# ilpoviertola/V-AURA

Measured on AMD Instinct MI355X. Metric: audio codec tokens/sec (whole node), 2.56 s clips, higher is better.
Workload: dtype f16x2-split(22b)/f32-acc

## Files before the change

include/vaura_hip.h:

```cpp
#ifndef VAURA_HIP_H
#define VAURA_HIP_H

#include <stddef.h>
#include <stdint.h>

#ifdef __cplusplus
extern "C" {
#endif

typedef void* vaura_stream_t;

typedef enum vaura_status {
  VAURA_OK = 0,
  VAURA_ERR_ARG = -1,
  VAURA_ERR_SHAPE = -2,
  VAURA_ERR_DTYPE = -3,
  VAURA_ERR_STATE = -4
} vaura_status;

typedef enum vaura_wdtype { VAURA_W_F32 = 0, VAURA_W_BF16 = 1, VAURA_W_FP8 = 2, VAURA_W_H1 = 3, VAURA_W_H2 = 4, VAURA_W_FP8H = 5 } vaura_wdtype;

typedef struct vaura_dims {
  int32_t n_layer;
  int32_t d_model;
// ... 135 lines not shown

int vaura_pattern_build(const int32_t* codes, int32_t* seq, int B, int K, int T, int special, vaura_stream_t s);
int vaura_pattern_revert(const int32_t* seq, int32_t* codes, int B, int K, int T, int S, int fill, vaura_stream_t s);
int vaura_pattern_build_delays(const int32_t* codes, int32_t* seq, int B, int K, int T, int S, int special,
                               const int32_t* delays_host, vaura_stream_t s);
int vaura_pattern_revert_delays(const int32_t* seq, int32_t* codes, int B, int K, int T, int S, int fill,
                                const int32_t* delays_host, vaura_stream_t s);

int vaura_sample(const float* logits, int B, int K, int vocab, const vaura_sampling* sp, const float* noise,
                 int64_t step, int32_t* tokens_out, vaura_stream_t s);

int vaura_sample_clips(const float* logits, int B, int K, int vocab, const vaura_sampling* sp, const vaura_clip_sampling* clips,
                       const float* noise, int64_t step, int32_t* tokens_out, int32_t* seq, int T, int S, int32_t* state,
                       vaura_stream_t s);

int vaura_sample_logprobs(const float* logits, int B, int K, int vocab, const vaura_sampling* sp, const vaura_clip_sampling* clips,
                          const float* noise, int64_t step, int32_t* tokens_out, int32_t* seq, int T, int S, int32_t* state,
                          float* logprobs_out, vaura_stream_t s);
int vaura_sample_relevance(const float* logits, int B, int K, int vocab, const vaura_sampling* sp, const vaura_clip_sampling* clips,
                           const float* noise, int64_t step, int32_t* tokens_out, int32_t* seq, int T, int S, int32_t* state,
                           float* logprobs_out, float* cond_out, float* null_out, vaura_stream_t s);
int vaura_pattern_revert_delays_f32(const float* seq, float* out, int B, int K, int T, int S, float fill, const int32_t* delays_host,
                                    vaura_stream_t s);
int vaura_sequence_logprob(const float* logprobs, int seq_len, const int32_t* delays_host, int B, int K, int T, int t0,
                           float* per_codebook, float* per_clip, vaura_stream_t s);
int vaura_select_candidates(const float* scores, const int32_t* codes, int B, int N, int K, int T, int32_t* codes_out, int32_t* winner,
                            vaura_stream_t s);

int vaura_pattern_build_clips(const int32_t* codes, int32_t* seq, int B, int K, int T, int S, int special, const int32_t* delays_host,
                              const int32_t* clip_timesteps, vaura_stream_t s);
int vaura_pattern_revert_clips(const int32_t* seq, int32_t* codes, int B, int K, int T, int S, int fill, int pad,
                               const int32_t* delays_host, const int32_t* clip_timesteps, vaura_stream_t s);
int vaura_pattern_revert_clips_f32(const float* seq, float* out, int B, int K, int T, int S, float fill, float pad,
                                   const int32_t* delays_host, const int32_t* clip_timesteps, vaura_stream_t s);
int vaura_sequence_logprob_clips(const float* logprobs, int seq_len, const int32_t* delays_host, int B, int K, int T, int t0,
                                 const int32_t* clip_timesteps, float* per_codebook, float* per_clip, vaura_stream_t s);
int vaura_sample_seq(const float* logits, int B, int K, int vocab, const vaura_sampling* sp, const vaura_clip_sampling* clips,
                     const float* noise, int32_t* seq, int T, int S, int32_t* state, const int32_t* delays_host,
                     const int32_t* clip_timesteps, float* lp_seq, float* cond_seq, float* null_seq, vaura_stream_t s);
int vaura_sample_seq_starts(const float* logits, int B, int K, int vocab, const vaura_sampling* sp, const vaura_clip_sampling* clips,
                            const float* noise, int32_t* seq, int T, int S, int32_t* state, const int32_t* delays_host,
                            const int32_t* clip_timesteps, const int32_t* clip_first_steps, float* lp_seq, float* cond_seq,
                            float* null_seq, vaura_stream_t s);
int vaura_sequence_logprob_starts(const float* logprobs, int seq_len, const int32_t* delays_host, int B, int K, int T,
                                  const int32_t* clip_t0, const int32_t* clip_timesteps, float* per_codebook, float* per_clip,
                                  vaura_stream_t s);
int vaura_embed(const vaura_decoder* dec, int pos_host, int n_pos, vaura_stream_t s);

int vaura_decode_step(const vaura_decoder* dec, const vaura_sampling* sp, int sample, vaura_stream_t s);

typedef void* vaura_step_graph_t;
int vaura_generate_loop(const vaura_decoder* dec, const vaura_sampling* sp, int n_prefill, int n_steps,
                        vaura_step_graph_t graph, vaura_stream_t s);
int vaura_step_graph_build(const vaura_decoder* dec, const vaura_sampling* sp, vaura_stream_t s, vaura_step_graph_t* out);
int vaura_prefill_rows(const vaura_decoder* dec, int n_prefill, int n_sel, vaura_stream_t s);
void vaura_step_graph_free(vaura_step_graph_t graph);

typedef enum vaura_kernel_kind {
  VAURA_K_EMBED = 0, VAURA_K_QKV = 1, VAURA_K_ATTN = 2, VAURA_K_WO = 3, VAURA_K_W13 = 4, VAURA_K_W2 = 5,
  VAURA_K_HEADS = 6, VAURA_K_SAMPLE = 7, VAURA_K_COUNT = 8
} vaura_kernel_kind;
int vaura_profile_loop(const vaura_decoder* dec, const vaura_sampling* sp, int n_steps, unsigned kind_mask,
                       double* total_ms_host, int64_t* launches_host, vaura_stream_t s);
void vaura_profile_outliers(int64_t* per_kind);

int vaura_score(const vaura_decoder* dec, int n_pos, const int32_t* targets, float* ws_chunk_logits, float* logits_out, float* nll,
                uint8_t* mask_out, float* loss_per_cb, float* loss, vaura_stream_t s);
int vaura_score_relevance(const vaura_decoder* dec, int n_pos, const int32_t* targets, float* ws_chunk_logits, float* logits_out, float* nll,
                          uint8_t* mask_out, float* loss_per_cb, float* loss, float* nll_null, float* loss_per_cb_null, float* loss_null,
                          vaura_stream_t s);
int vaura_score_logits(const float* logits, const int32_t* targets, const uint8_t* mask, int B, int K, int V, int Ta, float* nll,
                       float* loss_per_cb, float* loss, vaura_stream_t s);

int vaura_gemv(const void* w, int wdtype, const float* x, const float* gain, const float* residual, float* out,
               int64_t rows, int64_t N, int64_t K, int epilogue, float eps, vaura_stream_t s);
int vaura_gemv_pair(const void* w, int wdtype , const uint16_t* x_split, const float* ss_in, int n_ss_in, const float* residual, float* out,
                    float* out_khalf2 ,
                    uint16_t* out_split, const float* gain_out, float* ss_out, int64_t rows, int64_t N, int64_t K, int epilogue,
                    float eps, vaura_stream_t s);
int vaura_split_rows(const float* src, uint16_t* dst, const float* gain, float* ss, int64_t rows, int64_t C, vaura_stream_t s);

int vaura_attention_step(const float* qkv, const float* rope, float* kcache, float* vcache, float* out,
                         int rows, int n_head, int head_dim, int max_len, int pos, vaura_stream_t s);

int vaura_attention_step_split(const float* qkv, const float* rope, float* kcache, float* vcache, float* out, float* part,
                               int rows, int n_head, int head_dim, int max_len, int pos, int n_split, vaura_stream_t s);
int vaura_attention_splits(int rows, int n_head, int max_len);
int vaura_attention_step_ex(const float* qkv, const float* qkv2, const float* rope, float* kcache, float* vcache, float* out,
                            uint16_t* out_split, float* part, uint32_t* arrivals, int rows, int n_head, int head_dim, int max_len,
                            int pos, int n_split, int plane_shift, int kv_dtype, vaura_stream_t s);
int vaura_attention_step_kv(const float* qkv, const float* qkv2, const float* rope, float* kcache, float* vcache, uint8_t* kscale,
                            uint8_t* vscale, float* out, uint16_t* out_split, float* part, uint32_t* arrivals, int rows, int n_head,
                            int head_dim, int max_len, int pos, int n_split, int plane_shift, int kv_dtype, vaura_stream_t s);
int vaura_attention_step_probs(const float* qkv, const float* qkv2, const float* rope, float* kcache, float* vcache, uint8_t* kscale,
                               uint8_t* vscale, float* out, uint16_t* out_split, float* part, uint32_t* arrivals, int rows, int n_head,
                               int head_dim, int max_len, int pos, int n_split, int plane_shift, int kv_dtype, float* probs, int pos0,
                               int n_steps, int rows_out, vaura_stream_t s);
int vaura_attention_map(const float* probs, float* out, int n_steps, int n_rows, int n_head, int max_len, int W, int all_heads,
                        vaura_stream_t s);
int vaura_attention_prefill(const vaura_decoder* d, int layer, int p0, int n_pos, vaura_stream_t s);
int vaura_rope_append_rows(const vaura_decoder* d, int layer, int p0, int n_pos, const int32_t* row_n, int n_sel, vaura_stream_t s);

typedef struct vaura_conv {
  const float* w;
  const float* bias;
  const float* wscale;
  int32_t cin, cout, taps, dilation, stride, _pad;
} vaura_conv;

typedef struct vaura_codec {
  int32_t n_codebooks, codebook_size, codebook_dim, latent_dim;
  int32_t n_blocks, n_units;
  int32_t rates[4];
  const float* codebooks;
  const float* out_proj_w;
  const float* out_proj_b;
  vaura_conv conv_in;
  const float* alpha_up[4];
  vaura_conv up[4];
  const float* alpha_res[4][3][2];
  vaura_conv res[4][3][2];
  const float* alpha_out;
  vaura_conv conv_out;
  float* ws[4];
  size_t ws_elems;
  int32_t precision;
  int32_t _pad1;
} vaura_codec;

int vaura_dac_decode(const vaura_codec* c, const int32_t* codes, int B, int T, float* wav, vaura_stream_t s);
size_t vaura_dac_workspace_elems(const vaura_codec* c, int B, int T);
int vaura_dac_decode_clips(const vaura_codec* c, const int32_t* codes, int B, int T_max, const int32_t* lengths, float* wav,
                           vaura_stream_t s);
size_t vaura_dac_decode_clips_workspace_elems(const vaura_codec* c, int B, const int32_t* lengths);
int vaura_dac_clips_gap(const vaura_codec* c);
int vaura_dac_decode_window(const vaura_codec* c, const int32_t* codes, int B, int T_max, const int32_t* lengths, const int32_t* starts,
                            const int32_t* counts, float* wav, int N_max, vaura_stream_t s);
size_t vaura_dac_decode_window_workspace_elems(const vaura_codec* c, int B, const int32_t* lengths, const int32_t* starts,
                                               const int32_t* counts);
int vaura_dac_decode_halo(const vaura_codec* c);
int vaura_dac_decode_window_seq(const vaura_codec* c, const int32_t* seq, int B, int K, int S, const int32_t* delays_host,
                                const int32_t* lengths, const int32_t* starts, const int32_t* counts, float* wav, int N_max,
                                vaura_stream_t s);
size_t vaura_dac_decode_window_seq_workspace_elems(const vaura_codec* c, int B, int K, int S, const int32_t* delays_host,
                                                   const int32_t* lengths, const int32_t* starts, const int32_t* counts);
int vaura_dac_conv(const vaura_conv* cv, int precision, const float* in, float* out, float* scratch, int B, int Lin,
                   vaura_stream_t s);
int vaura_dac_conv_ex(const vaura_conv* cv, int precision, const float* in, const float* res, const float* alpha, float* out_raw,
                      void* out_act, float* scratch, int B, int Lin, vaura_stream_t s);
#define VAURA_DAC_UNIT_TWO_LAUNCHES (-100)
int vaura_dac_unit(const vaura_conv* c7, const vaura_conv* c1, int precision, const float* in, const float* res,
                   const float* alpha_mid, const float* alpha_next, float* out_raw, void* out_act, float* scratch, float* mid, int B,
                   int L, vaura_stream_t s);
int vaura_dac_from_codes(const int32_t* codes, const float* codebooks, const float* out_proj_w, const float* out_proj_b, void* z,
                         int B, int K, int T, int size, int dim, int latent, int pairs, vaura_stream_t s);
int vaura_dac_conv_out(const vaura_conv* cv, int precision, const float* in, float* wav, float* scratch, int B, int L,
                       vaura_stream_t s);
int vaura_snake(const float* x, const float* alpha, float* y, int64_t rows, int C, vaura_stream_t s);

typedef struct vaura_codec_encoder {
  int32_t n_codebooks, codebook_size, codebook_dim, latent_dim;
  int32_t n_blocks, n_units;
  int32_t rates[4];
  int32_t enc_dim;
  int32_t _pad0;
  const float* conv_in_w;
  const float* conv_in_b;
  const float* alpha_res[4][3][2];
  vaura_conv res[4][3][2];
  const float* alpha_down[4];
  vaura_conv down[4];
  const float* alpha_out;
  vaura_conv conv_out;
  const float* in_proj_w;
  const float* in_proj_b;
  const float* codebooks;
  const float* out_proj_w;
  const float* out_proj_b;
  float* ws[4];
  size_t ws_elems;
} vaura_codec_encoder;
int vaura_dac_encode(const vaura_codec_encoder* c, const float* wav, int B, int64_t n_samples, int32_t* codes, vaura_stream_t s);
int vaura_dac_enc_conv_in(const float* wav, const float* w, const float* bias, const float* alpha, float* out_raw, void* out_act,
                          int B, int64_t L, int C, vaura_stream_t s);
int vaura_dac_rvq_stage(float* residual, const float* in_w, const float* in_b, const float* codebook, const float* out_w,
                        const float* out_b, int32_t* codes, int B, int T, int latent, int dim, int size, int K, int k,
                        vaura_stream_t s);
size_t vaura_dac_encode_workspace_elems(const vaura_codec_encoder* c, int B, int64_t n_samples);
int vaura_dac_encode_clips(const vaura_codec_encoder* c, const float* wav, int B, int64_t n_max, const int64_t* sample_lengths,
                           int32_t* codes, vaura_stream_t s);
size_t vaura_dac_encode_clips_workspace_elems(const vaura_codec_encoder* c, int B, const int64_t* sample_lengths);
int vaura_dac_encode_clips_gap(const vaura_codec_encoder* c);

typedef enum vaura_audio_strategy { VAURA_AUDIO_CLIP = 0, VAURA_AUDIO_PEAK = 1, VAURA_AUDIO_RMS = 2, VAURA_AUDIO_NONE = 3 } vaura_audio_strategy;
int vaura_audio_normalize(const float* wav, float* out, int n_clips, int64_t n_samples, int strategy, int normalize,
                          float peak_clip_headroom_db, float rms_headroom_db, float* scratch, vaura_stream_t s);
size_t vaura_audio_scratch_elems(int n_clips);
int vaura_audio_loudness(const float* wav, float* out, int n_clips, int64_t n_samples, int sample_rate, float loudness_headroom_db,
                         int compressor, float energy_floor, float* scratch, vaura_stream_t s);
size_t vaura_audio_loudness_scratch_elems(int n_clips);
int vaura_audio_normalize_clips(const float* wav, float* out, int n_clips, int64_t n_stride, const int32_t* lengths, int strategy,
                                int normalize, float peak_clip_headroom_db, float rms_headroom_db, float* scratch, vaura_stream_t s);
int vaura_audio_loudness_clips(const float* wav, float* out, int n_clips, int64_t n_stride, const int32_t* lengths, int sample_rate,
                               float loudness_headroom_db, int compressor, float energy_floor, float* scratch, vaura_stream_t s);

typedef struct vaura_vit_attn {
  const void* qkv_w; const float* qkv_b;
  const void* proj_w; const float* proj_b;
} vaura_vit_attn;
typedef struct vaura_vit_block {
  const float *ln1_w, *ln1_b, *ln2_w, *ln2_b, *ln3_w, *ln3_b;
  vaura_vit_attn space, time;
  const void* fc1_w; const float* fc1_b; const void* fc2_w; const float* fc2_b;
} vaura_vit_block;
typedef struct vaura_vit {
  int32_t depth, dim, heads, hidden;
  int32_t n_patches, n_frames;
  int32_t in_chans, frames, img, patch, patch_t, patch_k;
  float eps; int32_t _pad;
  const void* pe_w; const float* pe_b;
  const float *cls_token, *pos_embed, *temp_embed;
  const vaura_vit_block* blocks_host;
  const float *norm_w, *norm_b;
  const float* agg_cls;
  const float *agg_ln1_w, *agg_ln1_b, *agg_ln2_w, *agg_ln2_b;
  const void* agg_in_w; const float* agg_in_b;
  const void* agg_out_w; const float* agg_out_b;
  const void* agg_l1_w; const float* agg_l1_b;
  const void* agg_l2_w; const float* agg_l2_b;
  float* ws_x; float* ws_qkv; uint16_t* ws_a; uint16_t* ws_h; uint16_t* ws_p; float* ws_z; float* ws_s;
} vaura_vit;
int vaura_avclip_forward(const vaura_vit* v, const float* frames, int n_seg, float* feats, vaura_stream_t s);
size_t vaura_avclip_workspace_bytes(const vaura_vit* v, int n_seg, int which);

int vaura_vit_patchify(const float* frames, void* patches, int n_seg, int in_chans, int frames_per_seg, int img, int patch_t, int patch,
                       vaura_stream_t s);
int vaura_vit_embed(const vaura_vit* v, float* x, int n_seg, vaura_stream_t s);
int vaura_vit_layernorm(const vaura_vit* v, const float* x, const float* w, const float* b, float* out_f32, void* out_pair, int64_t rows,
                        int map, vaura_stream_t s);
int vaura_vit_fill_rows(const vaura_vit* v, float* dst, const float* vec, int64_t n, int64_t stride, vaura_stream_t s);
int vaura_vit_cls_attention(const vaura_vit* v, const float* qkv, void* out_pair, float* part, int n_seq, int Lseq, int64_t out_stride,
                            vaura_stream_t s);
int vaura_vit_time_attention(const vaura_vit* v, const float* qkv, void* out_pair, int n_seg, vaura_stream_t s);
int vaura_vit_space_attention(const vaura_vit* v, const float* qkv, void* out_pair, int n_seg, vaura_stream_t s);
int vaura_linear_pair(const void* in, const void* w, const float* bias, const float* res, float* out_raw, void* out_act, int act, int B,
                      int Lin, int Lout, int oshift, int Cin, int Cout, vaura_stream_t s);

#define VAURA_PREPROC_MAX_TAPS 32
int vaura_video_preprocess(const uint8_t* video, int channels_last, int n_clips, int T, int C, int H, int W, int resize, int crop_h,
                           int crop_w, int F, int S, int seg_start, int seg_stride, const int32_t* h_rel, const int16_t* h_w, int h_taps,
                           int h_prec, const int32_t* v_start, const int16_t* v_w, int v_taps, int v_prec, int x0, int span,
                           int tile_rows, int tile_src_rows, const float* lut, float* out, vaura_stream_t s);
size_t vaura_video_preprocess_lds_bytes(int channels_last, int crop_w, int h_taps, int span, int tile_src_rows);

enum { VAURA_YUV_NV12 = 0, VAURA_YUV_I420 = 1 };
int vaura_video_preprocess_yuv420(const uint8_t* video, int64_t video_bytes, int layout, int64_t pitch, int64_t chroma_offset,
                                  int64_t frame_stride, int n_clips, int T, int H, int W, int y_off, int cy, int crv, int cgu, int cgv,
                                  int cbu, int resize, int crop_h, int crop_w, int F, int S, int seg_start, int seg_stride,
                                  const int32_t* h_rel, const int16_t* h_w, int h_taps, int h_prec, const int32_t* v_start,
                                  const int16_t* v_w, int v_taps, int v_prec, int x0, int span, int tile_rows, int tile_src_rows,
                                  const float* lut, float* out, vaura_stream_t s);
size_t vaura_video_preprocess_yuv420_lds_bytes(int layout, int crop_w, int h_taps, int span, int tile_src_rows);

int vaura_video_preprocess_frames(const uint8_t* video, int channels_last, int n_clips, int T, int C, int H, int W, int resize,
                                  int crop_h, int crop_w, int F, int S, const int32_t* h_rel, const int16_t* h_w, int h_taps, int h_prec,
                                  const int32_t* v_start, const int16_t* v_w, int v_taps, int v_prec, int x0, int span, int tile_rows,
                                  int tile_src_rows, const float* lut, float* out, const int32_t* frame_map, const uint8_t* carry,
                                  int carry_used, vaura_stream_t s);
int vaura_video_preprocess_yuv420_frames(const uint8_t* video, int64_t video_bytes, int layout, int64_t pitch, int64_t chroma_offset,
                                         int64_t frame_stride, int n_clips, int T, int H, int W, int y_off, int cy, int crv, int cgu,
                                         int cgv, int cbu, int resize, int crop_h, int crop_w, int F, int S, const int32_t* h_rel,
                                         const int16_t* h_w, int h_taps, int h_prec, const int32_t* v_start, const int16_t* v_w,
                                         int v_taps, int v_prec, int x0, int span, int tile_rows, int tile_src_rows, const float* lut,
                                         float* out, const int32_t* frame_map, const uint8_t* carry, int carry_used, vaura_stream_t s);

#define VAURA_AUDIO_PRE_TILE 1024
#define VAURA_AUDIO_PRE_MAX_TAPS 64
enum { VAURA_PCM_S16 = 0, VAURA_PCM_S32 = 1, VAURA_PCM_F32 = 2 };
int vaura_audio_preprocess(const void* pcm, int format, int interleaved, int B, int C, int64_t in_stride, const int32_t* n_in, int o, int n,
                           int w, const int32_t* first, const float* taps, int phases, int taps_per_phase, float* out, int64_t out_stride,
                           const int32_t* n_out, vaura_stream_t s);
size_t vaura_audio_preprocess_lds_bytes(int o, int n, int w, int taps_per_phase);
int vaura_audio_preprocess_tile(void);

#define VAURA_AUDIO_OUT_TILE 1024
#define VAURA_AUDIO_OUT_RECORD 5
int vaura_audio_output(const float* x, int B, int64_t in_stride, const int64_t* records, const float* carry_in, float* carry_out,
                       int history, int o, int n, int w, const int32_t* first, const float* taps, int phases, int taps_per_phase,
                       const float* gain, int format, int interleaved, int C_out, void* out, int64_t out_stride, int32_t* clipped,
                       vaura_stream_t s);
size_t vaura_audio_output_lds_bytes(int o, int n, int w, int taps_per_phase);
int vaura_audio_output_tile(void);

#define VAURA_SPECTROGRAM_RECORD 5
#define VAURA_SPECTROGRAM_MAX_MELS 256
enum { VAURA_SPEC_POWER = 0, VAURA_SPEC_DB = 1, VAURA_SPEC_LOG = 2, VAURA_SPEC_COMPLEX = 3 };
int vaura_spectrogram(const float* x, int B, int64_t in_stride, const int64_t* records, const float* carry_in, float* carry_out,
                      int history, int n_fft, int hop, const float* window, const float* twiddles, const int32_t* mel_bins,
                      const float* mel_weights, int mel_total, int F, int scale, float amin, float* out, int64_t out_stride,
                      vaura_stream_t s);
size_t vaura_spectrogram_lds_bytes(int n_fft, int F);

void vaura_set_debug_flags(unsigned flags);
void vaura_set_debug_flags2(unsigned flags);
long long vaura_debug_counter(int which);

const char* vaura_version(void);
size_t vaura_struct_size(int which);

#ifdef __cplusplus
}
#endif
#endif
```

vaura_amd/_lib.py:

```python
from __future__ import annotations

import ctypes as C
import os
from typing import Optional

_HERE = os.path.dirname(os.path.abspath(__file__))
LIB_PATH = os.path.join(_HERE, "csrc", "libvaura_hip.so")

W_F32, W_BF16, W_FP8, W_H1, W_H2, W_FP8H = 0, 1, 2, 3, 4, 5
EPI_STORE, EPI_RESID, EPI_SWIGLU, EPI_GELU, EPI_LOGITS = 0, 1, 2, 3, 4
DAC_UNIT_TWO_LAUNCHES = -100
KERNEL_KINDS = ("embed", "qkv", "attn", "wo", "w13", "w2", "heads", "sample")

c_float_p = C.c_void_p


class Dims(C.Structure):
    _fields_ = [("n_layer", C.c_int32), ("d_model", C.c_int32), ("n_head", C.c_int32), ("ffn_dim", C.c_int32),
                ("n_codebooks", C.c_int32), ("vocab", C.c_int32), ("cond_dim", C.c_int32), ("tok_dim", C.c_int32),
                ("cond_in", C.c_int32), ("codebook_dim", C.c_int32), ("tokens_per_frame", C.c_int32),
                ("eps", C.c_float)]


class LayerWeights(C.Structure):
# ... 5 lines not shown
    _fields_ = [("use_sampling", C.c_int32), ("temp", C.c_float), ("top_k", C.c_int32), ("top_p", C.c_float),
                ("cfg_scale", C.c_float), ("seed", C.c_uint64), ("clip_base", C.c_uint64), ("input_is_probs", C.c_int32),
                ("tie_eps", C.c_float)]


class ClipSampling(C.Structure):
    _fields_ = [("use_sampling", C.c_int32), ("temp", C.c_float), ("top_k", C.c_int32), ("top_p", C.c_float),
                ("cfg_scale", C.c_float), ("reserved", C.c_int32 * 3)]


class Decoder(C.Structure):
    _fields_ = [("dims", Dims), ("wdtype", C.c_int32), ("batch", C.c_int32), ("rows", C.c_int32),
                ("max_len", C.c_int32), ("timesteps", C.c_int32), ("seq_len", C.c_int32),
                ("n_cond_tokens", C.c_int32), ("prefill_positions", C.c_int32),
                ("plane_shift", C.c_int32), ("kv_dtype", C.c_int32),
                ("layers_host", C.POINTER(LayerWeights)), ("heads", C.c_void_p), ("final_norm", C.c_void_p),
                ("tok_emb", C.c_void_p), ("tok_proj_w", C.c_void_p), ("tok_proj_b", C.c_void_p), ("tok_table", C.c_void_p),
                ("empty_video", C.c_void_p), ("rope", C.c_void_p), ("cond_proj", C.c_void_p),
                ("kcache", C.c_void_p), ("vcache", C.c_void_p), ("seq", C.c_void_p), ("state", C.c_void_p),
                ("noise", C.c_void_p),
                ("ws_h", C.c_void_p), ("ws_qkv", C.c_void_p), ("ws_qkv2", C.c_void_p), ("ws_attn", C.c_void_p), ("ws_ffn", C.c_void_p),
                ("ws_logits", C.c_void_p),
                ("ws_h_split", C.c_void_p), ("ws_attn_split", C.c_void_p), ("ws_ffn_split", C.c_void_p),
                ("ws_ss", C.c_void_p), ("first_norm", C.c_void_p), ("ws_attn_part", C.c_void_p), ("ws_sync", C.c_void_p),
                ("has_pattern_delays", C.c_int32), ("pattern_delays", C.c_int32 * 16), ("ext_bytes", C.c_int32),
                ("kscale", C.c_void_p), ("vscale", C.c_void_p), ("clip_sampling", C.c_void_p), ("logprobs", C.c_void_p)]


class DecoderExt(C.Structure):
    _fields_ = [("dec", Decoder), ("logprobs_cond", C.c_void_p), ("logprobs_null", C.c_void_p)]


class DecoderExt2(C.Structure):
    _fields_ = [("ext", DecoderExt), ("clip_timesteps", C.c_void_p), ("clip_cond_tokens", C.c_void_p)]


class DecoderExt3(C.Structure):
    _fields_ = [("ext2", DecoderExt2), ("row_prompt_steps", C.c_void_p)]


class DecoderExt4(C.Structure):
    _fields_ = [("ext3", DecoderExt3), ("attn_probs", C.c_void_p), ("attn_layer", C.c_int32), ("attn_pos0", C.c_int32),
                ("attn_steps", C.c_int32), ("attn_rows", C.c_int32)]


class Conv(C.Structure):
    _fields_ = [("w", C.c_void_p), ("bias", C.c_void_p), ("wscale", C.c_void_p), ("cin", C.c_int32), ("cout", C.c_int32),
                ("taps", C.c_int32), ("dilation", C.c_int32), ("stride", C.c_int32), ("_pad", C.c_int32)]


class Codec(C.Structure):
    _fields_ = [("n_codebooks", C.c_int32), ("codebook_size", C.c_int32), ("codebook_dim", C.c_int32),
                ("latent_dim", C.c_int32), ("n_blocks", C.c_int32), ("n_units", C.c_int32),
                ("rates", C.c_int32 * 4),
                ("codebooks", C.c_void_p), ("out_proj_w", C.c_void_p), ("out_proj_b", C.c_void_p),
                ("conv_in", Conv), ("alpha_up", C.c_void_p * 4), ("up", Conv * 4),
                ("alpha_res", ((C.c_void_p * 2) * 3) * 4), ("res", ((Conv * 2) * 3) * 4),
                ("alpha_out", C.c_void_p), ("conv_out", Conv),
                ("ws", C.c_void_p * 4), ("ws_elems", C.c_size_t), ("precision", C.c_int32), ("_pad1", C.c_int32)]


class CodecEncoder(C.Structure):
    _fields_ = [("n_codebooks", C.c_int32), ("codebook_size", C.c_int32), ("codebook_dim", C.c_int32),
                ("latent_dim", C.c_int32), ("n_blocks", C.c_int32), ("n_units", C.c_int32),
                ("rates", C.c_int32 * 4), ("enc_dim", C.c_int32), ("_pad0", C.c_int32),
                ("conv_in_w", C.c_void_p), ("conv_in_b", C.c_void_p),
                ("alpha_res", ((C.c_void_p * 2) * 3) * 4), ("res", ((Conv * 2) * 3) * 4),
                ("alpha_down", C.c_void_p * 4), ("down", Conv * 4),
                ("alpha_out", C.c_void_p), ("conv_out", Conv),
                ("in_proj_w", C.c_void_p), ("in_proj_b", C.c_void_p), ("codebooks", C.c_void_p),
                ("out_proj_w", C.c_void_p), ("out_proj_b", C.c_void_p),
                ("ws", C.c_void_p * 4), ("ws_elems", C.c_size_t)]


class VitAttn(C.Structure):
    _fields_ = [("qkv_w", C.c_void_p), ("qkv_b", C.c_void_p), ("proj_w", C.c_void_p), ("proj_b", C.c_void_p)]


class VitBlock(C.Structure):
    _fields_ = [("ln1_w", C.c_void_p), ("ln1_b", C.c_void_p), ("ln2_w", C.c_void_p), ("ln2_b", C.c_void_p),
                ("ln3_w", C.c_void_p), ("ln3_b", C.c_void_p), ("space", VitAttn), ("time", VitAttn),
                ("fc1_w", C.c_void_p), ("fc1_b", C.c_void_p), ("fc2_w", C.c_void_p), ("fc2_b", C.c_void_p)]


class Vit(C.Structure):
    _fields_ = [("depth", C.c_int32), ("dim", C.c_int32), ("heads", C.c_int32), ("hidden", C.c_int32),
                ("n_patches", C.c_int32), ("n_frames", C.c_int32),
                ("in_chans", C.c_int32), ("frames", C.c_int32), ("img", C.c_int32), ("patch", C.c_int32), ("patch_t", C.c_int32),
                ("patch_k", C.c_int32), ("eps", C.c_float), ("_pad", C.c_int32),
                ("pe_w", C.c_void_p), ("pe_b", C.c_void_p), ("cls_token", C.c_void_p), ("pos_embed", C.c_void_p),
                ("temp_embed", C.c_void_p), ("blocks_host", C.POINTER(VitBlock)), ("norm_w", C.c_void_p), ("norm_b", C.c_void_p),
                ("agg_cls", C.c_void_p), ("agg_ln1_w", C.c_void_p), ("agg_ln1_b", C.c_void_p), ("agg_ln2_w", C.c_void_p),
                ("agg_ln2_b", C.c_void_p), ("agg_in_w", C.c_void_p), ("agg_in_b", C.c_void_p), ("agg_out_w", C.c_void_p),
                ("agg_out_b", C.c_void_p), ("agg_l1_w", C.c_void_p), ("agg_l1_b", C.c_void_p), ("agg_l2_w", C.c_void_p),
                ("agg_l2_b", C.c_void_p),
                ("ws_x", C.c_void_p), ("ws_qkv", C.c_void_p), ("ws_a", C.c_void_p), ("ws_h", C.c_void_p), ("ws_p", C.c_void_p),
                ("ws_z", C.c_void_p), ("ws_s", C.c_void_p)]


SIGNATURES = {
    "vaura_audio_normalize": (C.c_int, [C.c_void_p, C.c_void_p, C.c_int, C.c_int64, C.c_int, C.c_int, C.c_float, C.c_float,
                                        C.c_void_p, C.c_void_p]),
    "vaura_audio_scratch_elems": (C.c_size_t, [C.c_int]),
    "vaura_audio_loudness": (C.c_int, [C.c_void_p, C.c_void_p, C.c_int, C.c_int64, C.c_int, C.c_float, C.c_int, C.c_float, C.c_void_p,
                                       C.c_void_p]),
    "vaura_audio_loudness_scratch_elems": (C.c_size_t, [C.c_int]),
    "vaura_audio_normalize_clips": (C.c_int, [C.c_void_p, C.c_void_p, C.c_int, C.c_int64, C.c_void_p, C.c_int, C.c_int, C.c_float,
                                              C.c_float, C.c_void_p, C.c_void_p]),
    "vaura_audio_loudness_clips": (C.c_int, [C.c_void_p, C.c_void_p, C.c_int, C.c_int64, C.c_void_p, C.c_int, C.c_float, C.c_int,
                                             C.c_float, C.c_void_p, C.c_void_p]),
    "vaura_dac_encode": (C.c_int, [C.POINTER(CodecEncoder), C.c_void_p, C.c_int, C.c_int64, C.c_void_p, C.c_void_p]),
    "vaura_dac_encode_workspace_elems": (C.c_size_t, [C.POINTER(CodecEncoder), C.c_int, C.c_int64]),
    "vaura_avclip_forward": (C.c_int, [C.POINTER(Vit), C.c_void_p, C.c_int, C.c_void_p, C.c_void_p]),
    "vaura_avclip_workspace_bytes": (C.c_size_t, [C.POINTER(Vit), C.c_int, C.c_int]),
    "vaura_vit_patchify": (C.c_int, [C.c_void_p, C.c_void_p, C.c_int, C.c_int, C.c_int, C.c_int, C.c_int, C.c_int, C.c_void_p]),
    "vaura_vit_embed": (C.c_int, [C.POINTER(Vit), C.c_void_p, C.c_int, C.c_void_p]),
    "vaura_vit_layernorm": (C.c_int, [C.POINTER(Vit), C.c_void_p, C.c_void_p, C.c_void_p, C.c_void_p, C.c_void_p, C.c_int64, C.c_int,
                                      C.c_void_p]),
    "vaura_vit_fill_rows": (C.c_int, [C.POINTER(Vit), C.c_void_p, C.c_void_p, C.c_int64, C.c_int64, C.c_void_p]),
    "vaura_vit_cls_attention": (C.c_int, [C.POINTER(Vit), C.c_void_p, C.c_void_p, C.c_void_p, C.c_int, C.c_int, C.c_int64, C.c_void_p]),
    "vaura_vit_time_attention": (C.c_int, [C.POINTER(Vit), C.c_void_p, C.c_void_p, C.c_int, C.c_void_p]),
    "vaura_vit_space_attention": (C.c_int, [C.POINTER(Vit), C.c_void_p, C.c_void_p, C.c_int, C.c_void_p]),
    "vaura_linear_pair": (C.c_int, [C.c_void_p, C.c_void_p, C.c_void_p, C.c_void_p, C.c_void_p, C.c_void_p, C.c_int, C.c_int, C.c_int,
                                    C.c_int, C.c_int, C.c_int, C.c_int, C.c_void_p]),
    "vaura_video_preprocess": (C.c_int, [C.c_void_p, C.c_int, C.c_int, C.c_int, C.c_int, C.c_int, C.c_int, C.c_int, C.c_int, C.c_int, C.c_int,
                                         C.c_int, C.c_int, C.c_int, C.c_void_p, C.c_void_p, C.c_int, C.c_int, C.c_void_p, C.c_void_p,
                                         C.c_int, C.c_int, C.c_int, C.c_int, C.c_int, C.c_int, C.c_void_p, C.c_void_p, C.c_void_p]),
    "vaura_video_preprocess_lds_bytes": (C.c_size_t, [C.c_int, C.c_int, C.c_int, C.c_int, C.c_int]),
    "vaura_video_preprocess_yuv420": (C.c_int, [C.c_void_p, C.c_int64, C.c_int, C.c_int64, C.c_int64, C.c_int64, *[C.c_int] * 10,
                                                *[C.c_int] * 7, C.c_void_p, C.c_void_p, C.c_int, C.c_int, C.c_void_p, C.c_void_p,
                                                *[C.c_int] * 6, C.c_void_p, C.c_void_p, C.c_void_p]),
    "vaura_video_preprocess_yuv420_lds_bytes": (C.c_size_t, [C.c_int, C.c_int, C.c_int, C.c_int, C.c_int]),
    "vaura_video_preprocess_frames": (C.c_int, [C.c_void_p, *[C.c_int] * 11, C.c_void_p, C.c_void_p, C.c_int, C.c_int, C.c_void_p, C.c_void_p,
                                                *[C.c_int] * 6, C.c_void_p, C.c_void_p, C.c_void_p, C.c_void_p, C.c_int, C.c_void_p]),
    "vaura_video_preprocess_yuv420_frames": (C.c_int, [C.c_void_p, C.c_int64, C.c_int, C.c_int64, C.c_int64, C.c_int64, *[C.c_int] * 10,
                                                       *[C.c_int] * 5, C.c_void_p, C.c_void_p, C.c_int, C.c_int, C.c_void_p, C.c_void_p,
                                                       *[C.c_int] * 6, C.c_void_p, C.c_void_p, C.c_void_p, C.c_void_p, C.c_int, C.c_void_p]),
    "vaura_audio_preprocess": (C.c_int, [C.c_void_p, C.c_int, C.c_int, C.c_int, C.c_int, C.c_int64, C.c_void_p, C.c_int, C.c_int, C.c_int,
                                         C.c_void_p, C.c_void_p, C.c_int, C.c_int, C.c_void_p, C.c_int64, C.c_void_p, C.c_void_p]),
    "vaura_audio_preprocess_lds_bytes": (C.c_size_t, [C.c_int, C.c_int, C.c_int, C.c_int]),
    "vaura_audio_preprocess_tile": (C.c_int, []),
    "vaura_audio_output": (C.c_int, [C.c_void_p, C.c_int, C.c_int64, C.c_void_p, C.c_void_p, C.c_void_p, C.c_int, C.c_int, C.c_int, C.c_int,
                                     C.c_void_p, C.c_void_p, C.c_int, C.c_int, C.c_void_p, C.c_int, C.c_int, C.c_int, C.c_void_p, C.c_int64,
                                     C.c_void_p, C.c_void_p]),
    "vaura_audio_output_lds_bytes": (C.c_size_t, [C.c_int, C.c_int, C.c_int, C.c_int]),
    "vaura_audio_output_tile": (C.c_int, []),
    "vaura_spectrogram": (C.c_int, [C.c_void_p, C.c_int, C.c_int64, C.c_void_p, C.c_void_p, C.c_void_p, C.c_int, C.c_int, C.c_int,
                                    C.c_void_p, C.c_void_p, C.c_void_p, C.c_void_p, C.c_int, C.c_int, C.c_int, C.c_float, C.c_void_p,
                                    C.c_int64, C.c_void_p]),
    "vaura_spectrogram_lds_bytes": (C.c_size_t, [C.c_int, C.c_int]),
    "vaura_version": (C.c_char_p, []),
    "vaura_set_debug_flags": (None, [C.c_uint]),
    "vaura_set_debug_flags2": (None, [C.c_uint]),
    "vaura_debug_counter": (C.c_longlong, [C.c_int]),
    "vaura_struct_size": (C.c_size_t, [C.c_int]),
    "vaura_packed_weight_bytes": (C.c_size_t, [C.c_int64, C.c_int64, C.c_int]),
    "vaura_pack_weight": (C.c_int, [C.c_void_p, C.c_void_p, C.c_int64, C.c_int64, C.c_int, C.c_void_p]),
    "vaura_build_token_table": (C.c_int, [C.c_void_p, C.c_void_p, C.c_void_p, C.c_void_p, C.c_int, C.c_int, C.c_int,
                                          C.c_int, C.c_void_p]),
    "vaura_pack_rows": (C.c_int, [C.c_void_p, C.c_void_p, C.c_int64, C.c_int64, C.c_void_p]),
    "vaura_unpack_rows": (C.c_int, [C.c_void_p, C.c_void_p, C.c_int64, C.c_int64, C.c_void_p]),
    "vaura_prefill_cond": (C.c_int, [C.POINTER(Dims), C.c_void_p, C.c_void_p, C.c_void_p, C.c_int, C.c_void_p,
                                     C.c_void_p, C.c_int64, C.c_void_p]),
    "vaura_cond_window": (C.c_int, [C.POINTER(Decoder), C.c_void_p, C.c_void_p, C.c_int, C.c_int, C.c_int, C.c_void_p]),
    "vaura_pattern_build": (C.c_int, [C.c_void_p, C.c_void_p, C.c_int, C.c_int, C.c_int, C.c_int, C.c_void_p]),
    "vaura_pattern_revert": (C.c_int, [C.c_void_p, C.c_void_p, C.c_int, C.c_int, C.c_int, C.c_int, C.c_int, C.c_void_p]),
    "vaura_pattern_build_delays": (C.c_int, [C.c_void_p, C.c_void_p, C.c_int, C.c_int, C.c_int, C.c_int, C.c_int,
                                             C.POINTER(C.c_int32), C.c_void_p]),
    "vaura_pattern_revert_delays": (C.c_int, [C.c_void_p, C.c_void_p, C.c_int, C.c_int, C.c_int, C.c_int, C.c_int,
                                              C.POINTER(C.c_int32), C.c_void_p]),
    "vaura_sample": (C.c_int, [C.c_void_p, C.c_int, C.c_int, C.c_int, C.POINTER(Sampling), C.c_void_p, C.c_int64,
                               C.c_void_p, C.c_void_p]),
    "vaura_sample_clips": (C.c_int, [C.c_void_p, C.c_int, C.c_int, C.c_int, C.POINTER(Sampling), C.c_void_p, C.c_void_p, C.c_int64,
                                     C.c_void_p, C.c_void_p, C.c_int, C.c_int, C.c_void_p, C.c_void_p]),
    "vaura_sample_logprobs": (C.c_int, [C.c_void_p, C.c_int, C.c_int, C.c_int, C.POINTER(Sampling), C.c_void_p, C.c_void_p, C.c_int64,
                                        C.c_void_p, C.c_void_p, C.c_int, C.c_int, C.c_void_p, C.c_void_p, C.c_void_p]),
    "vaura_sample_relevance": (C.c_int, [C.c_void_p, C.c_int, C.c_int, C.c_int, C.POINTER(Sampling), C.c_void_p, C.c_void_p, C.c_int64,
                                         C.c_void_p, C.c_void_p, C.c_int, C.c_int, C.c_void_p, C.c_void_p, C.c_void_p, C.c_void_p,
                                         C.c_void_p]),
    "vaura_pattern_revert_delays_f32": (C.c_int, [C.c_void_p, C.c_void_p, C.c_int, C.c_int, C.c_int, C.c_int, C.c_float,
                                                  C.POINTER(C.c_int32), C.c_void_p]),
    "vaura_sequence_logprob": (C.c_int, [C.c_void_p, C.c_int, C.POINTER(C.c_int32), C.c_int, C.c_int, C.c_int, C.c_int, C.c_void_p,
                                         C.c_void_p, C.c_void_p]),
    "vaura_select_candidates": (C.c_int, [C.c_void_p, C.c_void_p, C.c_int, C.c_int, C.c_int, C.c_int, C.c_void_p, C.c_void_p,
                                          C.c_void_p]),
    "vaura_pattern_build_clips": (C.c_int, [C.c_void_p, C.c_void_p, C.c_int, C.c_int, C.c_int, C.c_int, C.c_int, C.POINTER(C.c_int32),
                                            C.c_void_p, C.c_void_p]),
    "vaura_pattern_revert_clips": (C.c_int, [C.c_void_p, C.c_void_p, C.c_int, C.c_int, C.c_int, C.c_int, C.c_int, C.c_int,
                                             C.POINTER(C.c_int32), C.c_void_p, C.c_void_p]),
    "vaura_pattern_revert_clips_f32": (C.c_int, [C.c_void_p, C.c_void_p, C.c_int, C.c_int, C.c_int, C.c_int, C.c_float, C.c_float,
                                                 C.POINTER(C.c_int32), C.c_void_p, C.c_void_p]),
    "vaura_sequence_logprob_clips": (C.c_int, [C.c_void_p, C.c_int, C.POINTER(C.c_int32), C.c_int, C.c_int, C.c_int, C.c_int, C.c_void_p,
                                               C.c_void_p, C.c_void_p, C.c_void_p]),
    "vaura_sample_seq": (C.c_int, [C.c_void_p, C.c_int, C.c_int, C.c_int, C.POINTER(Sampling), C.c_void_p, C.c_void_p, C.c_void_p, C.c_int,
                                   C.c_int, C.c_void_p, C.POINTER(C.c_int32), C.c_void_p, C.c_void_p, C.c_void_p, C.c_void_p, C.c_void_p]),
    "vaura_sample_seq_starts": (C.c_int, [C.c_void_p, C.c_int, C.c_int, C.c_int, C.POINTER(Sampling), C.c_void_p, C.c_void_p, C.c_void_p, C.c_int,
                                          C.c_int, C.c_void_p, C.POINTER(C.c_int32), C.c_void_p, C.c_void_p, C.c_void_p, C.c_void_p, C.c_void_p,
                                          C.c_void_p]),
    "vaura_sequence_logprob_starts": (C.c_int, [C.c_void_p, C.c_int, C.POINTER(C.c_int32), C.c_int, C.c_int, C.c_int, C.c_void_p, C.c_void_p,
                                                C.c_void_p, C.c_void_p, C.c_void_p]),
    "vaura_prefill_rows": (C.c_int, [C.POINTER(Decoder), C.c_int, C.c_int, C.c_void_p]),
    "vaura_rope_append_rows": (C.c_int, [C.POINTER(Decoder), C.c_int, C.c_int, C.c_int, C.c_void_p, C.c_int, C.c_void_p]),
    "vaura_embed": (C.c_int, [C.POINTER(Decoder), C.c_int, C.c_int, C.c_void_p]),
    "vaura_decode_step": (C.c_int, [C.POINTER(Decoder), C.POINTER(Sampling), C.c_int, C.c_void_p]),
    "vaura_generate_loop": (C.c_int, [C.POINTER(Decoder), C.POINTER(Sampling), C.c_int, C.c_int, C.c_void_p, C.c_void_p]),
    "vaura_step_graph_build": (C.c_int, [C.POINTER(Decoder), C.POINTER(Sampling), C.c_void_p, C.POINTER(C.c_void_p)]),
    "vaura_step_graph_free": (None, [C.c_void_p]),
    "vaura_profile_loop": (C.c_int, [C.POINTER(Decoder), C.POINTER(Sampling), C.c_int, C.c_uint, C.POINTER(C.c_double),
                                     C.POINTER(C.c_int64), C.c_void_p]),
    "vaura_profile_outliers": (None, [C.POINTER(C.c_int64)]),
    "vaura_score": (C.c_int, [C.POINTER(Decoder), C.c_int, C.c_void_p, C.c_void_p, C.c_void_p, C.c_void_p, C.c_void_p, C.c_void_p,
                              C.c_void_p, C.c_void_p]),
    "vaura_score_relevance": (C.c_int, [C.POINTER(Decoder), C.c_int, C.c_void_p, C.c_void_p, C.c_void_p, C.c_void_p, C.c_void_p,
                                        C.c_void_p, C.c_void_p, C.c_void_p, C.c_void_p, C.c_void_p, C.c_void_p]),
    "vaura_score_logits": (C.c_int, [C.c_void_p, C.c_void_p, C.c_void_p, C.c_int, C.c_int, C.c_int, C.c_int, C.c_void_p, C.c_void_p,
                                     C.c_void_p, C.c_void_p]),
    "vaura_gemv": (C.c_int, [C.c_void_p, C.c_int, C.c_void_p, C.c_void_p, C.c_void_p, C.c_void_p, C.c_int64,
                             C.c_int64, C.c_int64, C.c_int, C.c_float, C.c_void_p]),
    "vaura_gemv_pair": (C.c_int, [C.c_void_p, C.c_int, C.c_void_p, C.c_void_p, C.c_int, C.c_void_p, C.c_void_p, C.c_void_p, C.c_void_p, C.c_void_p,
                                  C.c_void_p, C.c_int64, C.c_int64, C.c_int64, C.c_int, C.c_float, C.c_void_p]),
    "vaura_split_rows": (C.c_int, [C.c_void_p, C.c_void_p, C.c_void_p, C.c_void_p, C.c_int64, C.c_int64, C.c_void_p]),
    "vaura_attention_step_split": (C.c_int, [C.c_void_p, C.c_void_p, C.c_void_p, C.c_void_p, C.c_void_p, C.c_void_p, C.c_int,
                                             C.c_int, C.c_int, C.c_int, C.c_int, C.c_int, C.c_void_p]),
    "vaura_attention_splits": (C.c_int, [C.c_int, C.c_int, C.c_int]),
    "vaura_attention_step": (C.c_int, [C.c_void_p, C.c_void_p, C.c_void_p, C.c_void_p, C.c_void_p, C.c_int, C.c_int,
                                       C.c_int, C.c_int, C.c_int, C.c_void_p]),
    "vaura_attention_step_ex": (C.c_int, [C.c_void_p, C.c_void_p, C.c_void_p, C.c_void_p, C.c_void_p, C.c_void_p, C.c_void_p, C.c_void_p,
                                          C.c_void_p, C.c_int, C.c_int, C.c_int, C.c_int, C.c_int, C.c_int, C.c_int, C.c_int, C.c_void_p]),
    "vaura_attention_step_kv": (C.c_int, [C.c_void_p, C.c_void_p, C.c_void_p, C.c_void_p, C.c_void_p, C.c_void_p, C.c_void_p, C.c_void_p,
                                          C.c_void_p, C.c_void_p, C.c_void_p, C.c_int, C.c_int, C.c_int, C.c_int, C.c_int, C.c_int, C.c_int,
                                          C.c_int, C.c_void_p]),
    "vaura_attention_step_probs": (C.c_int, [C.c_void_p, C.c_void_p, C.c_void_p, C.c_void_p, C.c_void_p, C.c_void_p, C.c_void_p, C.c_void_p,
                                             C.c_void_p, C.c_void_p, C.c_void_p, C.c_int, C.c_int, C.c_int, C.c_int, C.c_int, C.c_int, C.c_int,
                                             C.c_int, C.c_void_p, C.c_int, C.c_int, C.c_int, C.c_void_p]),
    "vaura_attention_map": (C.c_int, [C.c_void_p, C.c_void_p, C.c_int, C.c_int, C.c_int, C.c_int, C.c_int, C.c_int, C.c_void_p]),
    "vaura_attention_prefill": (C.c_int, [C.POINTER(Decoder), C.c_int, C.c_int, C.c_int, C.c_void_p]),
    "vaura_dac_decode": (C.c_int, [C.POINTER(Codec), C.c_void_p, C.c_int, C.c_int, C.c_void_p, C.c_void_p]),
    "vaura_dac_workspace_elems": (C.c_size_t, [C.POINTER(Codec), C.c_int, C.c_int]),
    "vaura_dac_conv": (C.c_int, [C.POINTER(Conv), C.c_int, C.c_void_p, C.c_void_p, C.c_void_p, C.c_int, C.c_int, C.c_void_p]),
    "vaura_dac_conv_ex": (C.c_int, [C.POINTER(Conv), C.c_int, C.c_void_p, C.c_void_p, C.c_void_p, C.c_void_p, C.c_void_p, C.c_void_p,
                                    C.c_int, C.c_int, C.c_void_p]),
    "vaura_dac_unit": (C.c_int, [C.POINTER(Conv), C.POINTER(Conv), C.c_int, C.c_void_p, C.c_void_p, C.c_void_p, C.c_void_p, C.c_void_p,
                                 C.c_void_p, C.c_void_p, C.c_void_p, C.c_int, C.c_int, C.c_void_p]),
    "vaura_dac_from_codes": (C.c_int, [C.c_void_p, C.c_void_p, C.c_void_p, C.c_void_p, C.c_void_p, C.c_int, C.c_int, C.c_int, C.c_int,
                                       C.c_int, C.c_int, C.c_int, C.c_void_p]),
    "vaura_dac_conv_out": (C.c_int, [C.POINTER(Conv), C.c_int, C.c_void_p, C.c_void_p, C.c_void_p, C.c_int, C.c_int, C.c_void_p]),
    "vaura_dac_enc_conv_in": (C.c_int, [C.c_void_p, C.c_void_p, C.c_void_p, C.c_void_p, C.c_void_p, C.c_void_p, C.c_int, C.c_int64,
                                        C.c_int, C.c_void_p]),
    "vaura_dac_rvq_stage": (C.c_int, [C.c_void_p, C.c_void_p, C.c_void_p, C.c_void_p, C.c_void_p, C.c_void_p, C.c_void_p, C.c_int,
                                      C.c_int, C.c_int, C.c_int, C.c_int, C.c_int, C.c_int, C.c_void_p]),
    "vaura_snake": (C.c_int, [C.c_void_p, C.c_void_p, C.c_void_p, C.c_int64, C.c_int, C.c_void_p]),
    "vaura_dac_decode_clips": (C.c_int, [C.POINTER(Codec), C.c_void_p, C.c_int, C.c_int, C.POINTER(C.c_int32), C.c_void_p, C.c_void_p]),
    "vaura_dac_decode_clips_workspace_elems": (C.c_size_t, [C.POINTER(Codec), C.c_int, C.POINTER(C.c_int32)]),
    "vaura_dac_clips_gap": (C.c_int, [C.POINTER(Codec)]),
    "vaura_dac_decode_window": (C.c_int, [C.POINTER(Codec), C.c_void_p, C.c_int, C.c_int, C.POINTER(C.c_int32), C.POINTER(C.c_int32),
                                          C.POINTER(C.c_int32), C.c_void_p, C.c_int, C.c_void_p]),
    "vaura_dac_decode_window_workspace_elems": (C.c_size_t, [C.POINTER(Codec), C.c_int, C.POINTER(C.c_int32), C.POINTER(C.c_int32),
                                                             C.POINTER(C.c_int32)]),
    "vaura_dac_decode_halo": (C.c_int, [C.POINTER(Codec)]),
    "vaura_dac_decode_window_seq": (C.c_int, [C.POINTER(Codec), C.c_void_p, C.c_int, C.c_int, C.c_int, C.POINTER(C.c_int32),
                                              C.POINTER(C.c_int32), C.POINTER(C.c_int32), C.POINTER(C.c_int32), C.c_void_p, C.c_int,
                                              C.c_void_p]),
    "vaura_dac_decode_window_seq_workspace_elems": (C.c_size_t, [C.POINTER(Codec), C.c_int, C.c_int, C.c_int, C.POINTER(C.c_int32),
                                                                 C.POINTER(C.c_int32), C.POINTER(C.c_int32), C.POINTER(C.c_int32)]),
    "vaura_dac_encode_clips": (C.c_int, [C.POINTER(CodecEncoder), C.c_void_p, C.c_int, C.c_int64, C.POINTER(C.c_int64), C.c_void_p,
                                         C.c_void_p]),
    "vaura_dac_encode_clips_workspace_elems": (C.c_size_t, [C.POINTER(CodecEncoder), C.c_int, C.POINTER(C.c_int64)]),
    "vaura_dac_encode_clips_gap": (C.c_int, [C.POINTER(CodecEncoder)]),
}

_lib: Optional[C.CDLL] = None


class VauraHipError(RuntimeError):
    pass


def lib() -> C.CDLL:
    global _lib
    if _lib is None:
        if not os.path.exists(LIB_PATH):
            raise VauraHipError(
                f"{LIB_PATH} is missing: the HIP hot path is not built (run `python -m vaura_amd.csrc.build`). "
                "There is no CPU fallback.")
        import torch
        handle = C.CDLL(LIB_PATH)
        for name, (res, args) in SIGNATURES.items():
            fn = getattr(handle, name)
            fn.restype = res
            fn.argtypes = args
        structs = dict(enumerate([Dims, LayerWeights, Sampling, Decoder, Conv, Codec, CodecEncoder, Vit, VitBlock, ClipSampling, DecoderExt, DecoderExt2]))
        structs[13] = DecoderExt3
        structs[14] = DecoderExt4
        for which, cls in structs.items():
            if C.sizeof(cls) != handle.vaura_struct_size(which):
                raise VauraHipError(f"{LIB_PATH} was built from a different include/vaura_hip.h: sizeof({cls.__name__}) is "
                                    f"{handle.vaura_struct_size(which)} there, {C.sizeof(cls)} here (rebuild the library)")
        _lib = handle
    return _lib


def check(rc: int, what: str) -> None:
    if rc == 0:
        return
    if rc < 0:
        names = {-1: "VAURA_ERR_ARG", -2: "VAURA_ERR_SHAPE", -3: "VAURA_ERR_DTYPE", -4: "VAURA_ERR_STATE"}
        raise VauraHipError(f"{what}: {names.get(rc, rc)}")
    raise VauraHipError(f"{what}: hipError_t {rc}")


def check_delays(delays, n_codebooks: int) -> tuple:
    d = tuple(int(x) for x in delays)
    if len(d) != n_codebooks:
        raise VauraHipError(f"pattern delays {list(d)}: {len(d)} values for {n_codebooks} codebooks")
    if n_codebooks > 16:
        raise VauraHipError(f"delay patterns are implemented for at most 16 codebooks, got {n_codebooks}")
    if any(x < 0 for x in d) or list(d) != sorted(d):
        raise VauraHipError(f"pattern delays must be sorted and non-negative, got {list(d)}")
    return d


def delays_host(delays) -> "C.Array":
    return (C.c_int32 * len(delays))(*delays)


def ptr(t) -> int:
    return 0 if t is None else int(t.data_ptr())


def current_stream(device=None) -> int:
    import torch
    return int(torch.cuda.current_stream(device).cuda_stream)
```

vaura_amd/csrc/dac.hip:

```cpp
#include "conv_kernels.h"
#include "dac_clips.h"

__global__ __launch_bounds__(256) void conv_mfma_kernel(ConvArgs a) {
  __shared__ f32x4 Ws[2][BK / 4][BN + 1];
  __shared__ f32x4 Xs[2][BK / 4][BM + 1];
  const int tid = threadIdx.x, lane = tid & 63, wv = tid >> 6;
  const int wn = wv & 1, wm = wv >> 1;
  const int j0 = blockIdx.x * BM;
  const int n0 = blockIdx.y * BN;
  const int tiles_m = gridDim.x;
  (void)tiles_m;
  const int phases = a.ostride;
  const int b = blockIdx.z / phases, ph = blockIdx.z % phases;
  const float* in = a.in + (size_t)b * a.Lin * a.Cin;
  const float* wbase = a.w + (size_t)ph * a.NT * a.Cout * a.Cin;
  const int kc = a.Cin / BK;
  const int nk = a.NT * kc;

  f32x4 wreg[3], xreg[4];
  auto load_tile = [&](int kt) {
    const int t = kt / kc, ci0 = (kt % kc) * BK;
    const float* wt = wbase + (size_t)t * a.Cout * a.Cin;
    const int off = a.off_base + t * a.off_step;
#pragma unroll
    for (int i = 0; i < 3; ++i) {
      const int qd = tid + 256 * i, row = qd >> 3, kq = qd & 7;
      wreg[i] = *reinterpret_cast<const f32x4*>(wt + (size_t)(n0 + row) * a.Cin + ci0 + 4 * kq);
    }
#pragma unroll
    for (int i = 0; i < 4; ++i) {
      const int qd = tid + 256 * i, row = qd >> 3, kq = qd & 7;
      const int jr = j0 + row + off;
      xreg[i] = (jr >= 0 && jr < a.Lin) ? *reinterpret_cast<const f32x4*>(in + (size_t)jr * a.Cin + ci0 + 4 * kq)
                                        : f32x4{0.f, 0.f, 0.f, 0.f};
    }
  };
  auto store_tile = [&](int buf) {
#pragma unroll
    for (int i = 0; i < 3; ++i) { const int qd = tid + 256 * i; Ws[buf][qd & 7][qd >> 3] = wreg[i]; }
#pragma unroll
    for (int i = 0; i < 4; ++i) { const int qd = tid + 256 * i; Xs[buf][qd & 7][qd >> 3] = xreg[i]; }
  };

  f32x4 acc[3][4];
#pragma unroll
  for (int i = 0; i < 3; ++i)
#pragma unroll
    for (int j = 0; j < 4; ++j) acc[i][j] = f32x4{0.f, 0.f, 0.f, 0.f};

  load_tile(0);
  store_tile(0);
  __syncthreads();
  for (int kt = 0; kt < nk; ++kt) {
    const int buf = kt & 1;
    if (kt + 1 < nk) load_tile(kt + 1);
#pragma unroll
    for (int c = 0; c < 2; ++c) {
      f32x4 af[3], bf[4];
#pragma unroll
      for (int i = 0; i < 3; ++i) af[i] = Ws[buf][4 * c + (lane >> 4)][wn * 48 + i * 16 + (lane & 15)];
#pragma unroll
      for (int j = 0; j < 4; ++j) bf[j] = Xs[buf][4 * c + (lane >> 4)][wm * 64 + j * 16 + (lane & 15)];
#pragma unroll
      for (int s = 0; s < 4; ++s)
#pragma unroll
        for (int i = 0; i < 3; ++i)
#pragma unroll
          for (int j = 0; j < 4; ++j)
            acc[i][j] = __builtin_amdgcn_mfma_f32_16x16x4f32(af[i][s], bf[j][s], acc[i][j], 0, 0, 0);
    }
    if (kt + 1 < nk) store_tile(buf ^ 1);
    __syncthreads();
  }

  const size_t obase = (size_t)b * a.Lout * a.Cout;
#pragma unroll
  for (int j = 0; j < 4; ++j) {
    const int jr = j0 + wm * 64 + j * 16 + (lane & 15);
    if (jr >= a.jcount) continue;
    const int orow = jr * a.ostride + a.oshift0 + ph;
    if (orow < 0 || orow >= a.Lout) continue;
#pragma unroll
    for (int i = 0; i < 3; ++i) {
      const int co = n0 + wn * 48 + i * 16 + 4 * (lane >> 4);
      const size_t o = obase + (size_t)orow * a.Cout + co;
      f32x4 v = acc[i][j] + *reinterpret_cast<const f32x4*>(a.bias + co);
      if (a.res) v = *reinterpret_cast<const f32x4*>(a.res + o) + v;
      if (a.out_raw) *reinterpret_cast<f32x4*>(a.out_raw + o) = v;
      if (a.out_act) {
        const f32x4 al = *reinterpret_cast<const f32x4*>(a.alpha + co);
        f32x4 s;
#pragma unroll
        for (int r = 0; r < 4; ++r) s[r] = snake_f(v[r], al[r]);
        *reinterpret_cast<f32x4*>(a.out_act + o) = s;
      }
    }
  }
}

#define XHALO 56
#define XROWS (BM + XHALO)
template <int NI, bool WS, bool XS = false, int MJ = 4, bool FUSE = false>
__global__ __launch_bounds__(256, 2) void conv_pair_kernel(ConvPArgs a) {
  constexpr int BN_ = 32 * NI;
  constexpr int BMT = 32 * MJ;
  constexpr int XROWS_T = BMT + XHALO;
  constexpr int NXB = MJ == 4 ? 2 : 1;
  static_assert(MJ == 4 || MJ == 8, "128 or 256 rows");
  constexpr int WSTR = (BN_ + 3 + 15) / 16 * 16, XSTR = (XROWS_T + 3 + 15) / 16 * 16;
  constexpr int WS_ELEMS = 2 * (BK / 4) * WSTR, XS_ELEMS = NXB * (BK / 4) * XSTR;
  constexpr int SP = BN_ + 4;
  static_assert((WS_ELEMS + XS_ELEMS) * 16 >= BM * SP * 4, "the output tile must fit in the main loop's LDS");
  static_assert(!FUSE || (NI == 3 && MJ == 8), "the fused residual unit: all 96 channels in one 256-row workgroup");
  constexpr int W1STR = 112, YSTR = 80;
  constexpr int W1_ELEMS = FUSE ? 3 * (BK / 4) * W1STR : 0, Y_ELEMS = FUSE ? 3 * (BK / 4) * YSTR : 0;
  static_assert(!FUSE || Y_ELEMS * 16 >= 64 * SP * 4, "the 64-row output tile is staged over the activated tile");
  constexpr int SMEM_ELEMS = (WS_ELEMS + XS_ELEMS) > (W1_ELEMS + Y_ELEMS) ? (WS_ELEMS + XS_ELEMS) : (W1_ELEMS + Y_ELEMS);
  constexpr int TAB_ELEMS = FUSE ? 2 * BN_ / 4 : 0;
  __shared__ u32x4 smem[SMEM_ELEMS + TAB_ELEMS];
  auto coff = [](int kq) { return (kq & 1) + ((kq >> 2) << 1); };
  auto Ws = [&](int buf, int kq, int row) -> u32x4& { return smem[(buf * (BK / 4) + kq) * WSTR + row + coff(kq)]; };
  auto Xs = [&](int buf, int kq, int row) -> u32x4& { return smem[WS_ELEMS + (buf * (BK / 4) + kq) * XSTR + row + coff(kq)]; };
  const int tid = threadIdx.x, lane = tid & 63, wv = tid >> 6;
  const int wn = wv & 1, wm = wv >> 1;
  const int j0 = blockIdx.x * BMT;
  const int n0 = blockIdx.y * BN_;
  const int phases = a.ostride;
  const int b = blockIdx.z / phases, ph = blockIdx.z % phases;
  const int cq = a.Cin / 4;
  const u32x4* in = reinterpret_cast<const u32x4*>(a.in) + (size_t)b * a.Lin * cq;
  const u32x4* wbase = reinterpret_cast<const u32x4*>(a.w) + (size_t)ph * a.NT * a.Cout * cq;
  const int kc = a.Cin / BK;
  const int NT = a.NT;
  const int nk = NT * kc;
  const int span = (NT - 1) * (a.off_step < 0 ? -a.off_step : a.off_step);
  const int lo_off = a.off_base + (a.off_step < 0 ? (NT - 1) * a.off_step : 0);
  const int xrows = BMT + span;
  constexpr int XL = (XROWS_T * (BK / 4) + 255) / 256;

  u32x4 wreg[NI], xreg[XL];
  auto load_w = [&](int kt) {
    const int c = kt / NT, t = kt - c * NT;
    const u32x4* wt = wbase + (size_t)t * a.Cout * cq;
    const int q0 = c * (BK / 4);
#pragma unroll
    for (int i = 0; i < NI; ++i) {
      const int qd = tid + 256 * i, row = qd >> 3, kq = qd & 7;
      wreg[i] = wt[(size_t)(n0 + row) * cq + q0 + kq];
    }
  };
  auto store_w = [&](int buf) {
#pragma unroll
    for (int i = 0; i < NI; ++i) { const int qd = tid + 256 * i; Ws(buf, qd & 7, qd >> 3) = wreg[i]; }
  };
  auto load_x = [&](int c) {
    const int q0 = c * (BK / 4);
#pragma unroll
    for (int i = 0; i < XL; ++i) {
      const int qd = tid + 256 * i, row = qd >> 3, kq = qd & 7;
      const int jr = j0 + lo_off + row;
      xreg[i] = (row < xrows && jr >= 0 && jr < a.Lin) ? in[(size_t)jr * cq + q0 + kq] : u32x4{0u, 0u, 0u, 0u};
    }
  };
  auto store_x = [&](int buf) {
#pragma unroll
    for (int i = 0; i < XL; ++i) {
      const int qd = tid + 256 * i;
      if ((qd >> 3) < XROWS_T) Xs(buf, qd & 7, qd >> 3) = xreg[i];
    }
  };

  f32x4 acc[NI][MJ];
#pragma unroll
  for (int i = 0; i < NI; ++i)
#pragma unroll
    for (int j = 0; j < MJ; ++j) acc[i][j] = f32x4{0.f, 0.f, 0.f, 0.f};

  VA_STAMP_DECL(stamps);
  VA_STAMP(stamps, 0);
  load_w(0);
  load_x(0);
  store_w(0);
  store_x(0);
  if constexpr (FUSE) {
    if (tid < BN_) {
      float* tab = reinterpret_cast<float*>(smem + SMEM_ELEMS);
      const float al = a.alpha_mid[tid];
      tab[tid] = al;
      tab[BN_ + tid] = 1.0f / (al + 1e-9f);
    }
  }
  __syncthreads();
  VA_STAMP(stamps, 1);
  const int g = lane >> 4, r16 = lane & 15;
  int kt = 0;
  for (int c = 0; c < kc; ++c) {
    const int xb = NXB == 2 ? (c & 1) : 0;
    for (int t = 0; t < NT; ++t, ++kt) {
      const int buf = kt & 1;
      if (kt + 1 < nk) load_w(kt + 1);
      if (t == (NXB == 2 ? 0 : NT - 1) && c + 1 < kc) load_x(c + 1);
      const int shift = a.off_base + t * a.off_step - lo_off;
      f16x8 wh[NI], wl[NI];
#pragma unroll
      for (int i = 0; i < NI; ++i) {
        wh[i] = __builtin_bit_cast(f16x8, Ws(buf, 2 * g, wn * (NI * 16) + i * 16 + r16));
        if constexpr (!WS && !XS) wl[i] = __builtin_bit_cast(f16x8, Ws(buf, 2 * g + 1, wn * (NI * 16) + i * 16 + r16));
      }
      constexpr int JG = MJ == 4 ? 4 : 2;
#pragma unroll
      for (int jh = 0; jh < MJ; jh += JG) {
        f16x8 xh[JG], xl[JG];
#pragma unroll
        for (int j = 0; j < JG; ++j) {
          xh[j] = __builtin_bit_cast(f16x8, Xs(xb, 2 * g, shift + wm * (16 * MJ) + (jh + j) * 16 + r16));
          if constexpr (!XS) xl[j] = __builtin_bit_cast(f16x8, Xs(xb, 2 * g + 1, shift + wm * (16 * MJ) + (jh + j) * 16 + r16));
        }
#pragma unroll
        for (int i = 0; i < NI; ++i)
#pragma unroll
          for (int j = 0; j < JG; ++j) {
            if constexpr (!WS && !XS) acc[i][jh + j] = __builtin_amdgcn_mfma_f32_16x16x32_f16(wl[i], xh[j], acc[i][jh + j], 0, 0, 0);
            if constexpr (!XS) acc[i][jh + j] = __builtin_amdgcn_mfma_f32_16x16x32_f16(wh[i], xl[j], acc[i][jh + j], 0, 0, 0);
            acc[i][jh + j] = __builtin_amdgcn_mfma_f32_16x16x32_f16(wh[i], xh[j], acc[i][jh + j], 0, 0, 0);
          }
      }
      if (kt + 1 < nk) store_w(buf ^ 1);
      if (t == NT - 1 && c + 1 < kc) {
        if constexpr (NXB == 1) __syncthreads();
        store_x(NXB == 2 ? (xb ^ 1) : 0);
      }
      __syncthreads();
    }
  }

  VA_STAMP(stamps, 2);
  if constexpr (FUSE) {
    u32x4* W1 = smem;
    u32x4* Yi = smem + W1_ELEMS;
    auto W1s = [&](int c2, int kq, int row) -> u32x4& { return W1[(c2 * (BK / 4) + kq) * W1STR + row + coff(kq)]; };
    auto Ys = [&](int c2, int kq, int row) -> u32x4& { return Yi[(c2 * (BK / 4) + kq) * YSTR + row + coff(kq)]; };
    u32x4 w1reg[9];
#pragma unroll
    for (int i = 0; i < 9; ++i) w1reg[i] = reinterpret_cast<const u32x4*>(a.w2)[tid + 256 * i];
    float* stage = reinterpret_cast<float*>(Yi);
    const float* tab = reinterpret_cast<const float*>(smem + SMEM_ELEMS);
    typedef _Float16 f16x4 __attribute__((ext_vector_type(4)));
    auto pass = [&](auto pc) {
      constexpr int p = decltype(pc)::value;
      if (p > 0) __syncthreads();
      if (wm == (p >> 1)) {
#pragma unroll
        for (int jj = 0; jj < 4; ++jj)
#pragma unroll
          for (int i = 0; i < NI; ++i) {
            const int col = wn * (NI * 16) + i * 16 + 4 * g;
            const f32x4 v = acc[i][4 * (p & 1) + jj] + *reinterpret_cast<const f32x4*>(a.bias + col);
            const f32x4 al = *reinterpret_cast<const f32x4*>(tab + col), iv = *reinterpret_cast<const f32x4*>(tab + BN_ + col);
            f16x4 h4, l4;
#pragma unroll
            for (int e = 0; e < 4; ++e) {
              const float sv = snake_fi(v[e], al[e], iv[e]);
              h4[e] = (_Float16)sv;
              l4[e] = (_Float16)(sv - (float)h4[e]);
            }
            const int c2 = col >> 5, o = (col & 31) >> 3, half = (col & 7) >> 2, row = jj * 16 + r16;
            reinterpret_cast<f16x4*>(&Ys(c2, 2 * o, row))[half] = h4;
            reinterpret_cast<f16x4*>(&Ys(c2, 2 * o + 1, row))[half] = l4;
          }
      }
      if (p == 0) {
#pragma unroll
        for (int i = 0; i < 9; ++i) {
          const int qd = tid + 256 * i, n = qd / 24, q = qd - n * 24;
          W1s(q >> 3, q & 7, n) = w1reg[i];
        }
      }
      __syncthreads();
      if (p == 0) VA_STAMP(stamps, 3);
      f32x4 acc2[NI][2];
#pragma unroll
      for (int i = 0; i < NI; ++i)
#pragma unroll
        for (int j = 0; j < 2; ++j) acc2[i][j] = f32x4{0.f, 0.f, 0.f, 0.f};
#pragma unroll
      for (int c2 = 0; c2 < 3; ++c2) {
        f16x8 wh[NI], wl[NI], xh[2], xl[2];
#pragma unroll
        for (int i = 0; i < NI; ++i) {
          wh[i] = __builtin_bit_cast(f16x8, W1s(c2, 2 * g, wn * (NI * 16) + i * 16 + r16));
          if constexpr (!WS && !XS) wl[i] = __builtin_bit_cast(f16x8, W1s(c2, 2 * g + 1, wn * (NI * 16) + i * 16 + r16));
        }
#pragma unroll
        for (int j = 0; j < 2; ++j) {
          xh[j] = __builtin_bit_cast(f16x8, Ys(c2, 2 * g, (wm * 2 + j) * 16 + r16));
          if constexpr (!XS) xl[j] = __builtin_bit_cast(f16x8, Ys(c2, 2 * g + 1, (wm * 2 + j) * 16 + r16));
        }
#pragma unroll
        for (int i = 0; i < NI; ++i)
#pragma unroll
          for (int j = 0; j < 2; ++j) {
            if constexpr (!WS && !XS) acc2[i][j] = __builtin_amdgcn_mfma_f32_16x16x32_f16(wl[i], xh[j], acc2[i][j], 0, 0, 0);
            if constexpr (!XS) acc2[i][j] = __builtin_amdgcn_mfma_f32_16x16x32_f16(wh[i], xl[j], acc2[i][j], 0, 0, 0);
            acc2[i][j] = __builtin_amdgcn_mfma_f32_16x16x32_f16(wh[i], xh[j], acc2[i][j], 0, 0, 0);
          }
      }
      __syncthreads();
      if (p == 0) VA_STAMP(stamps, 4);
#pragma unroll
      for (int i = 0; i < NI; ++i)
#pragma unroll
        for (int j = 0; j < 2; ++j) {
          const int row = (wm * 2 + j) * 16 + r16, col = wn * (NI * 16) + i * 16 + 4 * g;
          *reinterpret_cast<f32x4*>(stage + row * SP + col) = acc2[i][j] + *reinterpret_cast<const f32x4*>(a.bias2 + col);
        }
      __syncthreads();
      conv_tile_store<BN_, SP, false, 64>(a, stage, b, ph, j0 + p * 64, n0, tid);
      if (p == 0) VA_STAMP(stamps, 5);
    };
    pass(std::integral_constant<int, 0>{});
    pass(std::integral_constant<int, 1>{});
    pass(std::integral_constant<int, 2>{});
    pass(std::integral_constant<int, 3>{});
    VA_STAMP(stamps, 6);
    VA_STAMP_FLUSH(stamps, 21);
    return;
  }
  float* stage = reinterpret_cast<float*>(smem);
#pragma unroll
  for (int h = 0; h < MJ / 4; ++h) {
    if (h > 0) __syncthreads();
#pragma unroll
    for (int j = 0; j < MJ; ++j) {
      const int rbk = wm * MJ + j;
      if (rbk / 8 != h) continue;
#pragma unroll
      for (int i = 0; i < NI; ++i) {
        const int row = (rbk % 8) * 16 + r16, col = wn * (NI * 16) + i * 16 + 4 * g;
        *reinterpret_cast<f32x4*>(stage + row * SP + col) = acc[i][j] + *reinterpret_cast<const f32x4*>(a.bias + n0 + col);
      }
    }
    __syncthreads();
    if (h == 0) VA_STAMP(stamps, 4);
    conv_tile_store<BN_, SP>(a, stage, b, ph, j0 + h * BM, n0, tid);
    if (h == 0) VA_STAMP(stamps, 5);
  }
  VA_STAMP(stamps, 6);
  VA_STAMP_FLUSH(stamps, 20);
}

template <int N, typename F>
__device__ __forceinline__ void va_static_for(F&& f) {
  if constexpr (N > 0) {
    va_static_for<N - 1>(f);
    f(std::integral_constant<int, N - 1>{});
  }
}

template <int NCT, int RB, bool WS, bool XS>
__global__ __launch_bounds__(256, 2) void conv_unit_kernel(ConvPArgs a) {
  constexpr int C_ = 16 * NCT;
  constexpr int BMT = 64 * RB;
  constexpr int KC = C_ / BK;
  constexpr int XROWS_T = BMT + XHALO;
  constexpr int WSTR = (C_ + 3 + 15) / 16 * 16, XSTR = (XROWS_T + 3 + 15) / 16 * 16, W2STR = (BN + 3 + 15) / 16 * 16;
  constexpr int WS_ELEMS = 2 * (BK / 4) * WSTR, XS_ELEMS = (BK / 4) * XSTR;
  constexpr int SP = BN + 4;
  constexpr int W2_ELEMS = 2 * (BK / 4) * W2STR, ST_ELEMS = 64 * SP / 4;
  constexpr int MAIN_ELEMS = WS_ELEMS + XS_ELEMS > W2_ELEMS + ST_ELEMS ? WS_ELEMS + XS_ELEMS : W2_ELEMS + ST_ELEMS;
  constexpr int TAB_ELEMS = 2 * C_ / 4;
  static_assert(NCT % 6 == 0 && (RB == 2 || RB == 4) && NCT * RB == 24, "96 channels x 256 rows or 192 x 128: 96 accumulator registers");
  __shared__ u32x4 smem[MAIN_ELEMS + TAB_ELEMS];
  auto coff = [](int kq) { return (kq & 1) + ((kq >> 2) << 1); };
  auto Ws = [&](int buf, int kq, int row) -> u32x4& { return smem[(buf * (BK / 4) + kq) * WSTR + row + coff(kq)]; };
  auto Xs = [&](int kq, int row) -> u32x4& { return smem[WS_ELEMS + kq * XSTR + row + coff(kq)]; };
  auto W2s = [&](int buf, int kq, int row) -> u32x4& { return smem[(buf * (BK / 4) + kq) * W2STR + row + coff(kq)]; };
  float* tab = reinterpret_cast<float*>(smem + MAIN_ELEMS);
  const int tid = threadIdx.x, lane = tid & 63;
  const int wv = __builtin_amdgcn_readfirstlane(tid >> 6);
  const int g = lane >> 4, r16 = lane & 15;
  const int j0 = blockIdx.x * BMT, b = blockIdx.z;
  constexpr int cq = C_ / 4;
  const u32x4* in = reinterpret_cast<const u32x4*>(a.in) + (size_t)b * a.Lin * cq;
  const u32x4* wbase = reinterpret_cast<const u32x4*>(a.w);
  const int NT = a.NT, nk = NT * KC;
  const int span = (NT - 1) * (a.off_step < 0 ? -a.off_step : a.off_step);
  const int lo_off = a.off_base + (a.off_step < 0 ? (NT - 1) * a.off_step : 0);
  const int xrows = BMT + span;
  constexpr int WL = C_ * (BK / 4) / 256;
  constexpr int XL = (XROWS_T * (BK / 4) + 255) / 256;

  u32x4 wreg[WL], xreg[XL];
  auto load_w = [&](int kt) {
    const int c = kt / NT, t = kt - c * NT;
    const u32x4* wt = wbase + (size_t)t * C_ * cq + c * (BK / 4);
#pragma unroll
    for (int i = 0; i < WL; ++i) { const int qd = tid + 256 * i; wreg[i] = wt[(size_t)(qd >> 3) * cq + (qd & 7)]; }
  };
  auto store_w = [&](int buf) {
#pragma unroll
    for (int i = 0; i < WL; ++i) {
      const int qd = tid + 256 * i, ch = qd >> 3, w5 = ch & 31;
      Ws(buf, qd & 7, (ch & ~31) + (((w5 >> 2) & 1) << 4) + ((w5 >> 3) << 2) + (w5 & 3)) = wreg[i];
    }
  };
  auto load_x = [&](int c) {
#pragma unroll
    for (int i = 0; i < XL; ++i) {
      const int qd = tid + 256 * i, row = qd >> 3, kq = qd & 7;
      const int jr = j0 + lo_off + row;
      xreg[i] = (row < xrows && jr >= 0 && jr < a.Lin) ? in[(size_t)jr * cq + c * (BK / 4) + kq] : u32x4{0u, 0u, 0u, 0u};
    }
  };
  auto store_x = [&]() {
#pragma unroll
    for (int i = 0; i < XL; ++i) { const int qd = tid + 256 * i; if ((qd >> 3) < XROWS_T) Xs(qd & 7, qd >> 3) = xreg[i]; }
  };

  f32x4 acc[NCT][RB];
#pragma unroll
  for (int i = 0; i < NCT; ++i)
#pragma unroll
    for (int j = 0; j < RB; ++j) acc[i][j] = f32x4{0.f, 0.f, 0.f, 0.f};

  VA_STAMP_DECL(stamps);
  VA_STAMP(stamps, 0);
  load_w(0);
  load_x(0);
  store_w(0);
  store_x();
  for (int ch = tid; ch < C_; ch += 256) {
    const float al = a.alpha_mid[ch];
    tab[ch] = al;
    tab[C_ + ch] = 1.0f / (al + 1e-9f);
  }
  __syncthreads();
  VA_STAMP(stamps, 1);
  int kt = 0;
  for (int c = 0; c < KC; ++c) {
    for (int t = 0; t < NT; ++t, ++kt) {
      const int buf = kt & 1;
      if (kt + 1 < nk) load_w(kt + 1);
      if (t == NT - 1 && c + 1 < KC) load_x(c + 1);
      const int shift = a.off_base + t * a.off_step - lo_off;
      f16x8 xh[RB], xl[RB];
#pragma unroll
      for (int j = 0; j < RB; ++j) {
        xh[j] = __builtin_bit_cast(f16x8, Xs(2 * g, shift + (wv * RB + j) * 16 + r16));
        if constexpr (!XS) xl[j] = __builtin_bit_cast(f16x8, Xs(2 * g + 1, shift + (wv * RB + j) * 16 + r16));
      }
#pragma unroll
      for (int ig = 0; ig < NCT; ig += 3) {
        f16x8 wh[3], wl[3];
#pragma unroll
        for (int i = 0; i < 3; ++i) {
          wh[i] = __builtin_bit_cast(f16x8, Ws(buf, 2 * g, (ig + i) * 16 + r16));
          if constexpr (!WS && !XS) wl[i] = __builtin_bit_cast(f16x8, Ws(buf, 2 * g + 1, (ig + i) * 16 + r16));
        }
#pragma unroll
        for (int i = 0; i < 3; ++i)
#pragma unroll
          for (int j = 0; j < RB; ++j) {
            if constexpr (!WS && !XS) acc[ig + i][j] = __builtin_amdgcn_mfma_f32_16x16x32_f16(wl[i], xh[j], acc[ig + i][j], 0, 0, 0);
            if constexpr (!XS) acc[ig + i][j] = __builtin_amdgcn_mfma_f32_16x16x32_f16(wh[i], xl[j], acc[ig + i][j], 0, 0, 0);
            acc[ig + i][j] = __builtin_amdgcn_mfma_f32_16x16x32_f16(wh[i], xh[j], acc[ig + i][j], 0, 0, 0);
          }
      }
      if (kt + 1 < nk) store_w(buf ^ 1);
      if (t == NT - 1 && c + 1 < KC) {
        __syncthreads();
        store_x();
      }
      __syncthreads();
    }
  }

  const u32x4* w2q = reinterpret_cast<const u32x4*>(a.w2);
  u32x4 w2reg[3];
  auto load_w2 = [&](int nt, int c2) {
#pragma unroll
    for (int i = 0; i < 3; ++i) { const int qd = tid + 256 * i; w2reg[i] = w2q[(size_t)(nt * BN + (qd >> 3)) * cq + c2 * (BK / 4) + (qd & 7)]; }
  };
  auto store_w2 = [&](int buf) {
#pragma unroll
    for (int i = 0; i < 3; ++i) { const int qd = tid + 256 * i; W2s(buf, qd & 7, qd >> 3) = w2reg[i]; }
  };
  VA_STAMP(stamps, 2);
  load_w2(0, 0);

  f16x8 yh[KC][RB], yl[KC][RB];
  va_static_for<KC>([&](auto cc) {
    constexpr int c2 = decltype(cc)::value;
    const int ch = 32 * c2 + 8 * g;
    const f32x4 b0 = *reinterpret_cast<const f32x4*>(a.bias + ch), b1 = *reinterpret_cast<const f32x4*>(a.bias + ch + 4);
    const f32x4 al0 = *reinterpret_cast<const f32x4*>(tab + ch), al1 = *reinterpret_cast<const f32x4*>(tab + ch + 4);
    const f32x4 iv0 = *reinterpret_cast<const f32x4*>(tab + C_ + ch), iv1 = *reinterpret_cast<const f32x4*>(tab + C_ + ch + 4);
#pragma unroll
    for (int j = 0; j < RB; ++j) {
      const f32x4 v0 = acc[2 * c2][j] + b0, v1 = acc[2 * c2 + 1][j] + b1;
      f16x8 h, l;
#pragma unroll
      for (int e = 0; e < 4; ++e) {
        const float s0 = snake_fi(v0[e], al0[e], iv0[e]), s1 = snake_fi(v1[e], al1[e], iv1[e]);
        h[e] = (_Float16)s0; l[e] = (_Float16)(s0 - (float)h[e]);
        h[e + 4] = (_Float16)s1; l[e + 4] = (_Float16)(s1 - (float)h[e + 4]);
      }
      yh[c2][j] = h;
      yl[c2][j] = l;
    }
  });

  VA_STAMP(stamps, 3);
  float* stage = reinterpret_cast<float*>(smem + W2_ELEMS);
  constexpr int WPP = 4 / RB;
#pragma unroll 1
  for (int nt = 0; nt < C_ / BN; ++nt) {
    f32x4 acc2[BN / 16][RB];
#pragma unroll
    for (int i = 0; i < BN / 16; ++i)
#pragma unroll
      for (int j = 0; j < RB; ++j) acc2[i][j] = f32x4{0.f, 0.f, 0.f, 0.f};
    if (nt > 0) load_w2(nt, 0);
    store_w2(0);
    __syncthreads();
    va_static_for<KC>([&](auto cc) {
      constexpr int c2 = decltype(cc)::value;
      constexpr int buf = c2 & 1;
      if (c2 + 1 < KC) load_w2(nt, c2 + 1);
#pragma unroll
      for (int ig = 0; ig < BN / 16; ig += 3) {
        f16x8 wh[3], wl[3];
#pragma unroll
        for (int i = 0; i < 3; ++i) {
          wh[i] = __builtin_bit_cast(f16x8, W2s(buf, 2 * g, (ig + i) * 16 + r16));
          if constexpr (!WS && !XS) wl[i] = __builtin_bit_cast(f16x8, W2s(buf, 2 * g + 1, (ig + i) * 16 + r16));
        }
#pragma unroll
        for (int i = 0; i < 3; ++i)
#pragma unroll
          for (int j = 0; j < RB; ++j) {
            if constexpr (!WS && !XS) acc2[ig + i][j] = __builtin_amdgcn_mfma_f32_16x16x32_f16(wl[i], yh[c2][j], acc2[ig + i][j], 0, 0, 0);
            if constexpr (!XS) acc2[ig + i][j] = __builtin_amdgcn_mfma_f32_16x16x32_f16(wh[i], yl[c2][j], acc2[ig + i][j], 0, 0, 0);
            acc2[ig + i][j] = __builtin_amdgcn_mfma_f32_16x16x32_f16(wh[i], yh[c2][j], acc2[ig + i][j], 0, 0, 0);
          }
      }
      if (c2 + 1 < KC) store_w2(buf ^ 1);
      __syncthreads();
    });
    if (nt == 0) VA_STAMP(stamps, 4);
#pragma unroll
    for (int p = 0; p < BMT / 64; ++p) {
      if (p > 0) __syncthreads();
      if (wv / WPP == p) {
#pragma unroll
        for (int i = 0; i < BN / 16; ++i)
#pragma unroll
          for (int j = 0; j < RB; ++j) {
            const int row = ((wv % WPP) * RB + j) * 16 + r16, col = i * 16 + 4 * g;
            *reinterpret_cast<f32x4*>(stage + row * SP + col) = acc2[i][j] + *reinterpret_cast<const f32x4*>(a.bias2 + nt * BN + col);
          }
      }
      __syncthreads();
      conv_tile_store<BN, SP, false, 64>(a, stage, b, 0, j0 + p * 64, nt * BN, tid);
    }
    if (nt == 0) VA_STAMP(stamps, 5);
    if (nt + 1 < C_ / BN) __syncthreads();
  }
  VA_STAMP(stamps, 6);
  VA_STAMP_FLUSH(stamps, 22);
}

typedef int i32x8 __attribute__((ext_vector_type(8)));

template <int NI>
__global__ __launch_bounds__(256, 2) void conv_mx8_kernel(ConvPArgs a) {
  constexpr int BN_ = 32 * NI;
  constexpr int WS_ELEMS = 2 * 8 * (BN_ + 1), XS_ELEMS = 2 * 8 * (XROWS + 1);
  constexpr int SP = BN_ + 4;
  static_assert((WS_ELEMS + XS_ELEMS) * 16 >= BM * SP * 4, "the output tile must fit in the main loop's LDS");
  __shared__ u32x4 smem[WS_ELEMS + XS_ELEMS];
  __shared__ uint32_t xsc[2][XROWS];
  auto Ws = [&](int buf, int kq, int row) -> u32x4& { return smem[(buf * 8 + kq) * (BN_ + 1) + row]; };
  auto Xs = [&](int buf, int kq, int row) -> u32x4& { return smem[WS_ELEMS + (buf * 8 + kq) * (XROWS + 1) + row]; };
  const int tid = threadIdx.x, lane = tid & 63, wv = tid >> 6;
  const int wn = wv & 1, wm = wv >> 1;
  const int j0 = blockIdx.x * BM;
  const int n0 = blockIdx.y * BN_;
  const int phases = a.ostride;
  const int b = blockIdx.z / phases, ph = blockIdx.z % phases;
  const int cq = a.Cin / 16;
  const int NT = a.NT;
  const int nsc = (a.Cin + 127) >> 7;
  const int nch_last = (a.Cin - 128 * (nsc - 1)) >> 5;
  const int steps_last = (nch_last * NT + 3) >> 2;
  const int nk = (nsc - 1) * NT + steps_last;
  const u32x4* in = reinterpret_cast<const u32x4*>(a.in) + (size_t)b * a.Lin * cq;
  const uint32_t* insc = a.in_scale + (size_t)b * a.Lin * nsc;
  const u32x4* wbase = reinterpret_cast<const u32x4*>(a.w) + (size_t)ph * nk * a.Cout * 8;
  const int span = (NT - 1) * (a.off_step < 0 ? -a.off_step : a.off_step);
  const int lo_off = a.off_base + (a.off_step < 0 ? (NT - 1) * a.off_step : 0);
  const int xrows = BM + span;
  constexpr int XL = (XROWS * 8 + 255) / 256;

  u32x4 wreg[NI], xreg[XL];
  uint32_t screg = 0;
  auto load_w = [&](int kt) {
    const u32x4* wt = wbase + (size_t)kt * a.Cout * 8;
#pragma unroll
    for (int i = 0; i < NI; ++i) {
      const int qd = tid + 256 * i;
      wreg[i] = wt[(size_t)(n0 + (qd >> 3)) * 8 + (qd & 7)];
    }
  };
  auto store_w = [&](int buf) {
#pragma unroll
    for (int i = 0; i < NI; ++i) { const int qd = tid + 256 * i; Ws(buf, qd & 7, qd >> 3) = wreg[i]; }
  };
  auto load_x = [&](int sc) {
    const int q0 = sc * 8, nq = (sc == nsc - 1 ? nch_last : 4) * 2;
#pragma unroll
    for (int i = 0; i < XL; ++i) {
      const int qd = tid + 256 * i, row = qd >> 3, kq = qd & 7;
      const int jr = j0 + lo_off + row;
      xreg[i] = (row < xrows && kq < nq && jr >= 0 && jr < a.Lin) ? in[(size_t)jr * cq + q0 + kq] : u32x4{0u, 0u, 0u, 0u};
    }
    const int jr = j0 + lo_off + tid;
    screg = (tid < xrows && jr >= 0 && jr < a.Lin) ? insc[(size_t)jr * nsc + sc] : 0u;
  };
  auto store_x = [&](int buf) {
#pragma unroll
    for (int i = 0; i < XL; ++i) {
      const int qd = tid + 256 * i;
      if ((qd >> 3) < XROWS) Xs(buf, qd & 7, qd >> 3) = xreg[i];
    }
    if (tid < XROWS) xsc[buf][tid] = screg;
  };

  f32x4 acc[NI][4];
#pragma unroll
  for (int i = 0; i < NI; ++i)
#pragma unroll
    for (int j = 0; j < 4; ++j) acc[i][j] = f32x4{0.f, 0.f, 0.f, 0.f};

  load_w(0);
  load_x(0);
  store_w(0);
  store_x(0);
  __syncthreads();
  const int g = lane >> 4, r16 = lane & 15;
  int kt = 0;
  for (int sc = 0; sc < nsc; ++sc) {
    const int xb = sc & 1;
    const int nch = sc == nsc - 1 ? nch_last : 4;
    const int nsteps = sc == nsc - 1 ? steps_last : NT;
    const int nkb = nch * NT;
    const float rnch = 1.0f / (float)nch;
    for (int st = 0; st < nsteps; ++st, ++kt) {
      const int buf = kt & 1;
      if (kt + 1 < nk) load_w(kt + 1);
      if (st == 0 && sc + 1 < nsc) load_x(sc + 1);
      const int h = g & 1;
      int chA = g >> 1, chB = 2 + (g >> 1), chS = g;
      int shA = a.off_base + st * a.off_step - lo_off, shB = shA, shS = shA;
      if (nch != 4) {
        auto split = [&](int kb, int& ch) {
          kb = kb < nkb ? kb : nkb - 1;
          const int t = (int)(((float)kb + 0.5f) * rnch);
          ch = kb - t * nch;
          return a.off_base + t * a.off_step - lo_off;
        };
        shA = split(4 * st + (g >> 1), chA);
        shB = split(4 * st + 2 + (g >> 1), chB);
        shS = split(4 * st + g, chS);
      }
      i32x8 wf[NI], xf[4];
      int xs[4];
#pragma unroll
      for (int i = 0; i < NI; ++i) {
        const u32x4 q0 = Ws(buf, 2 * g, wn * (NI * 16) + i * 16 + r16), q1 = Ws(buf, 2 * g + 1, wn * (NI * 16) + i * 16 + r16);
        wf[i] = i32x8{(int)q0.x, (int)q0.y, (int)q0.z, (int)q0.w, (int)q1.x, (int)q1.y, (int)q1.z, (int)q1.w};
      }
#pragma unroll
      for (int j = 0; j < 4; ++j) {
        const int row = wm * 64 + j * 16 + r16;
        const u32x4 q0 = Xs(xb, 2 * chA + h, shA + row), q1 = Xs(xb, 2 * chB + h, shB + row);
        xf[j] = i32x8{(int)q0.x, (int)q0.y, (int)q0.z, (int)q0.w, (int)q1.x, (int)q1.y, (int)q1.z, (int)q1.w};
        xs[j] = (int)((xsc[xb][shS + row] >> (8 * chS)) & 0xffu);
      }
#pragma unroll
      for (int i = 0; i < NI; ++i)
#pragma unroll
        for (int j = 0; j < 4; ++j)
          acc[i][j] = __builtin_amdgcn_mfma_scale_f32_16x16x128_f8f6f4(wf[i], xf[j], acc[i][j], 0, 0, 0, 127, 0, xs[j]);
      if (kt + 1 < nk) store_w(buf ^ 1);
      if (st == nsteps - 1 && sc + 1 < nsc) store_x(xb ^ 1);
      __syncthreads();
    }
  }

  float* stage = reinterpret_cast<float*>(smem);
#pragma unroll
  for (int j = 0; j < 4; ++j)
#pragma unroll
    for (int i = 0; i < NI; ++i) {
      const int row = wm * 64 + j * 16 + r16, col = wn * (NI * 16) + i * 16 + 4 * g;
      *reinterpret_cast<f32x4*>(stage + row * SP + col) =
          acc[i][j] * *reinterpret_cast<const f32x4*>(a.wscale + n0 + col) + *reinterpret_cast<const f32x4*>(a.bias + n0 + col);
    }
  __syncthreads();
  conv_tile_store<BN_, SP, true>(a, stage, b, ph, j0, n0, tid);
}

#define FC_NT 8
__global__ __launch_bounds__(256) void from_codes_kernel(const int32_t* __restrict__ codes, const float* __restrict__ cb,
                                                          const float* __restrict__ pw, const float* __restrict__ pb,
                                                          float* __restrict__ z, int K, int T, int size, int dim, int latent,
                                                          int pairs) {
  __shared__ float e[FC_NT][16][8];
  const int t0 = blockIdx.x * FC_NT, b = blockIdx.y;
  if (dim < 8) {
    for (int u = threadIdx.x; u < FC_NT * 16 * 8; u += blockDim.x) (&e[0][0][0])[u] = 0.f;
    __syncthreads();
  }
// ... 73 lines not shown
      const f32x4 ww = *reinterpret_cast<const f32x4*>(w + (size_t)t * C + 4 * cq);
      d = fmaf(x[0], ww[0], d); d = fmaf(x[1], ww[1], d); d = fmaf(x[2], ww[2], d); d = fmaf(x[3], ww[3], d);
    }
  }
  d += __shfl_xor(d, 1, 64);
  d += __shfl_xor(d, 2, 64);
  d += __shfl_xor(d, 4, 64);
  if (sub == 0 && l < L) wav[(size_t)b * L + l] = tanhf(d + bias[0]);
}

#define CO_TL 128
__global__ __launch_bounds__(256) void conv_out_tiled_kernel(const float* __restrict__ act, const float* __restrict__ w,
                                                              const float* __restrict__ bias, float* __restrict__ wav, int L, int C,
                                                              int pairs) {
  extern __shared__ __attribute__((aligned(16))) float rows[];
  const int b = blockIdx.y, l0 = blockIdx.x * CO_TL, tid = threadIdx.x;
  const int SR = C + 4, oct = C >> 3;
  for (int u = tid; u < (CO_TL + 6) * oct; u += 256) {
    const int rr = u / oct, oc = u - rr * oct;
    const int r = l0 - 3 + rr;
    float x[8];
    if (r < 0 || r >= L) {
#pragma unroll
      for (int e = 0; e < 8; ++e) x[e] = 0.f;
    } else if (pairs == 3) {
      const uint8_t* q = reinterpret_cast<const uint8_t*>(act) + (size_t)b * L * C;
      const int nsc = (C + 127) >> 7;
      const uint8_t* sc = reinterpret_cast<const uint8_t*>(act) + mx8_scale_offset((size_t)gridDim.y * L * C) + (size_t)b * L * nsc * 4;
      typedef int i32x2 __attribute__((ext_vector_type(2)));
      typedef float f32x2 __attribute__((ext_vector_type(2)));
      const i32x2 w8 = *reinterpret_cast<const i32x2*>(q + (size_t)r * C + 8 * oc);
      const int e8 = sc[((size_t)r * nsc + (oc >> 4)) * 4 + ((oc >> 2) & 3)];
      const float scl = __builtin_bit_cast(float, (uint32_t)e8 << 23);
      const f32x2 a0 = __builtin_amdgcn_cvt_pk_f32_fp8(w8.x, false), a1 = __builtin_amdgcn_cvt_pk_f32_fp8(w8.x, true);
      const f32x2 a2 = __builtin_amdgcn_cvt_pk_f32_fp8(w8.y, false), a3 = __builtin_amdgcn_cvt_pk_f32_fp8(w8.y, true);
      x[0] = a0.x * scl; x[1] = a0.y * scl; x[2] = a1.x * scl; x[3] = a1.y * scl;
      x[4] = a2.x * scl; x[5] = a2.y * scl; x[6] = a3.x * scl; x[7] = a3.y * scl;
    } else if (pairs) {
      const f16x8* pp = reinterpret_cast<const f16x8*>(reinterpret_cast<const _Float16*>(act) + (((size_t)b * L + r) * oct + oc) * 16);
      const f16x8 h = pp[0], lo = pp[1];
#pragma unroll
      for (int e = 0; e < 8; ++e) x[e] = (float)h[e] + (float)lo[e];
    } else {
      const f32x4* pp = reinterpret_cast<const f32x4*>(act + ((size_t)b * L + r) * C + 8 * oc);
      const f32x4 a0 = pp[0], a1 = pp[1];
      x[0] = a0[0]; x[1] = a0[1]; x[2] = a0[2]; x[3] = a0[3]; x[4] = a1[0]; x[5] = a1[1]; x[6] = a1[2]; x[7] = a1[3];
    }
    *reinterpret_cast<f32x4*>(rows + rr * SR + 8 * oc) = f32x4{x[0], x[1], x[2], x[3]};
    *reinterpret_cast<f32x4*>(rows + rr * SR + 8 * oc + 4) = f32x4{x[4], x[5], x[6], x[7]};
  }
  __syncthreads();
  const int half = __builtin_amdgcn_readfirstlane(tid >> 7), lo_ = tid & 127;
  const int c0 = half * (C >> 1), c1 = c0 + (C >> 1);
  f32x4 d4 = f32x4{0.f, 0.f, 0.f, 0.f};
#pragma unroll
  for (int t = 0; t < 7; ++t) {
    const f32x4* xr = reinterpret_cast<const f32x4*>(rows + (lo_ + t) * SR + c0);
    const f32x4* wr = reinterpret_cast<const f32x4*>(w + (size_t)t * C + c0);
#pragma unroll 4
    for (int c = 0; c < (c1 - c0) / 4; ++c) {
      const f32x4 x = xr[c], ww = wr[c];
      d4[0] = fmaf(x[0], ww[0], d4[0]); d4[1] = fmaf(x[1], ww[1], d4[1]); d4[2] = fmaf(x[2], ww[2], d4[2]); d4[3] = fmaf(x[3], ww[3], d4[3]);
    }
  }
  const float d = (d4[0] + d4[1]) + (d4[2] + d4[3]);
  float* part = rows + (CO_TL + 6) * SR;
  if (half) part[lo_] = d;
  __syncthreads();
  if (!half && l0 + lo_ < L) wav[(size_t)b * L + l0 + lo_] = tanhf((d + part[lo_]) + bias[0]);
}

__global__ __launch_bounds__(256) void act_convert_kernel(const float* __restrict__ in, void* out, uint8_t* out_scale, size_t rows,
                                                          int C, int fmt) {
  const size_t u = (size_t)blockIdx.x * 256 + threadIdx.x;
  const int oct = C >> 3;
  const size_t row = u / oct;
  if (row >= rows) return;
  const int co = (int)(u - row * oct) * 8;
  const f32x4 v0 = *reinterpret_cast<const f32x4*>(in + row * C + co), v1 = *reinterpret_cast<const f32x4*>(in + row * C + co + 4);
  const float sv[8] = {v0[0], v0[1], v0[2], v0[3], v1[0], v1[1], v1[2], v1[3]};
  store_act_octet(out, out_scale, fmt, row, co, C, sv);
}

static long long va_conv256_launches = 0;

typedef void (*ConvPairKernel)(ConvPArgs);
static ConvPairKernel conv_pair_instance(int ni, bool ws, bool xs, bool big) {
  if (ni == 3) {
    if (xs) return big ? conv_pair_kernel<3, true, true, 8> : conv_pair_kernel<3, true, true>;
    if (ws) return big ? conv_pair_kernel<3, true, false, 8> : conv_pair_kernel<3, true>;
    return big ? conv_pair_kernel<3, false, false, 8> : conv_pair_kernel<3, false>;
  }
  if (xs) return conv_pair_kernel<2, true, true>;
  if (ws) return big ? conv_pair_kernel<2, true, false, 8> : conv_pair_kernel<2, true>;
  return big ? conv_pair_kernel<2, false, false, 8> : conv_pair_kernel<2, false>;
}

static int launch_conv(const vaura_conv& cv, const float* in, const float* res, const float* alpha, float* out_raw,
                       float* out_act, int B, int Lin, int pairs, hipStream_t s) {
  if (!cv.w || !cv.bias || (cv.cin % BK)) return VAURA_ERR_SHAPE;
  if (out_act && !alpha) return VAURA_ERR_ARG;
  if (pairs) {
    if ((cv.cout % BN) && (cv.cout % 64)) return VAURA_ERR_SHAPE;
    ConvPArgs p;
    p.in = reinterpret_cast<const uint16_t*>(in); p.w = reinterpret_cast<const uint16_t*>(cv.w); p.bias = cv.bias; p.res = res;
    p.alpha = alpha; p.out_raw = out_raw; p.out_act = reinterpret_cast<uint16_t*>(out_act);
    p.Lin = Lin; p.Cin = cv.cin; p.Cout = cv.cout; p.act = 0;
    p.act_fmt = 0; p.out_scale = nullptr; p.in_scale = nullptr; p.wscale = nullptr;
    p.w2 = nullptr; p.bias2 = nullptr; p.alpha_mid = nullptr;
    if (cv.stride > 1 && (cv.stride % 2)) return VAURA_ERR_SHAPE;
    if (cv.stride <= 1 && (cv.taps - 1) * cv.dilation > XHALO) return VAURA_ERR_SHAPE;
    const int ph = va_conv_geometry(p, cv.taps, cv.dilation, cv.stride, Lin);
    if (pairs == 3) {
      if (out_act) {
        p.act_fmt = 1;
        p.out_scale = reinterpret_cast<uint8_t*>(out_act) + mx8_scale_offset((size_t)B * p.Lout * cv.cout);
      }
      if (cv.wscale) {
        if (cv.cout % BN) return VAURA_ERR_SHAPE;
        p.wscale = cv.wscale;
        p.in_scale = reinterpret_cast<const uint32_t*>(reinterpret_cast<const uint8_t*>(in) + mx8_scale_offset((size_t)B * Lin * cv.cin));
        VA_LAUNCH((conv_mx8_kernel<3>), dim3((p.jcount + BM - 1) / BM, cv.cout / BN, B * ph), dim3(256), 0, s, p);
        return 0;
      }
      pairs = 2;
    }
    const bool xs = pairs == 4, ws = xs || pairs == 2;
    const int ni = cv.cout % BN == 0 ? 3 : 2, tiles = cv.cout / (32 * ni);
    const int g256 = (p.jcount + 2 * BM - 1) / (2 * BM);
    const bool big = (ni == 3 || !xs) && !va_variant(VV_CODEC_128_ROWS) && (int64_t)g256 * tiles * B * ph >= 384;
    if (big) ++va_conv256_launches;
    VA_LAUNCH(conv_pair_instance(ni, ws, xs, big), dim3(big ? g256 : (p.jcount + BM - 1) / BM, tiles, B * ph), dim3(256), 0, s, p);
    return 0;
  }
  if (cv.cout % BN) return VAURA_ERR_SHAPE;
  ConvArgs a;
  a.in = in; a.w = cv.w; a.bias = cv.bias; a.res = res; a.alpha = alpha; a.out_raw = out_raw; a.out_act = out_act;
  a.Lin = Lin; a.Cin = cv.cin; a.Cout = cv.cout;
  if (cv.stride > 1 && (cv.stride % 2)) return VAURA_ERR_SHAPE;
  const int phases = va_conv_geometry(a, cv.taps, cv.dilation, cv.stride, Lin);
  dim3 grid((a.jcount + BM - 1) / BM, cv.cout / BN, B * phases);
  VA_LAUNCH(conv_mfma_kernel, grid, dim3(256), 0, s, a);
  return 0;
}

int va_launch_conv_pair_tile(const ConvPArgs& p, int B, hipStream_t s) {
  VA_LAUNCH((conv_pair_kernel<3, false>), dim3((p.jcount + BM - 1) / BM, p.Cout / BN, B), dim3(256), 0, s, p);
  return 0;
}


#define VA_UNIT_NOT_ELIGIBLE (-0x7fffff00)
static long long va_conv_units_fused = 0;
static int launch_conv_unit(const vaura_conv& c7, const vaura_conv& c1, const float* in, const float* res, const float* alpha_mid,
                            const float* alpha_next, float* out_raw, float* out_act, int B, int L, int pairs, hipStream_t s) {
  if (pairs != 1 && pairs != 2 && pairs != 4) return VA_UNIT_NOT_ELIGIBLE;
  if (va_variant(VV_CODEC_UNIT_TWO_LAUNCHES) || va_variant(VV_CODEC_128_ROWS)) return VA_UNIT_NOT_ELIGIBLE;
  const int C = c7.cin;
  if ((C != BN && C != 2 * BN) || c7.cout != C || c1.cin != C || c1.cout != C || c7.stride != 1 || c1.stride != 1 || c1.taps != 1 || c7.taps < 1 ||
      (c7.taps - 1) * c7.dilation > XHALO || !c7.w || !c7.bias || !c1.w || !c1.bias || !alpha_mid || !alpha_next || !res || !out_act || (const float*)out_act == in)
    return VA_UNIT_NOT_ELIGIBLE;
  const int rows = C == BN ? 256 : 128;
  const int gx = (L + rows - 1) / rows;
  if ((int64_t)gx * B < 384) return VA_UNIT_NOT_ELIGIBLE;
  ConvPArgs p;
  p.in = reinterpret_cast<const uint16_t*>(in); p.w = reinterpret_cast<const uint16_t*>(c7.w); p.bias = c7.bias; p.res = res;
  p.alpha = alpha_next; p.out_raw = out_raw; p.out_act = reinterpret_cast<uint16_t*>(out_act);
  p.Lin = L; p.Cin = C; p.Cout = C; p.act = 0;
  p.act_fmt = 0; p.out_scale = nullptr; p.in_scale = nullptr; p.wscale = nullptr;
  va_conv_geometry(p, c7.taps, c7.dilation, 1, L);
  p.w2 = reinterpret_cast<const uint16_t*>(c1.w); p.bias2 = c1.bias; p.alpha_mid = alpha_mid;
  ++va_conv_units_fused;
  const dim3 grid(gx, 1, B);
  if (C == BN) {
    if (pairs == 4) VA_LAUNCH((conv_pair_kernel<3, true, true, 8, true>), grid, dim3(256), 0, s, p);
    else if (pairs == 2) VA_LAUNCH((conv_pair_kernel<3, true, false, 8, true>), grid, dim3(256), 0, s, p);
    else VA_LAUNCH((conv_pair_kernel<3, false, false, 8, true>), grid, dim3(256), 0, s, p);
  } else {
    if (pairs == 4) VA_LAUNCH((conv_unit_kernel<12, 2, true, true>), grid, dim3(256), 0, s, p);
    else if (pairs == 2) VA_LAUNCH((conv_unit_kernel<12, 2, true, false>), grid, dim3(256), 0, s, p);
    else VA_LAUNCH((conv_unit_kernel<12, 2, false, false>), grid, dim3(256), 0, s, p);
  }
  return 0;
}


VA_STAMP_SETTER(vaura_stamps_set_dac)

__global__ __launch_bounds__(256) void enc_conv_in_kernel(const float* __restrict__ wav, const float* __restrict__ w ,
                                                          const float* __restrict__ bias, const float* __restrict__ alpha,
                                                          float* __restrict__ out_raw, uint16_t* __restrict__ out_act, int64_t L,
                                                          int C) {
  const int b = blockIdx.y;
  const int qpr = C / 4;
  const int64_t gid = (int64_t)blockIdx.x * 256 + threadIdx.x;
  const int64_t l = gid / qpr;
  const int cq = (int)(gid % qpr);
  if (l >= L) return;
  const float* x = wav + (size_t)b * L;
  f32x4 v = *reinterpret_cast<const f32x4*>(bias + cq * 4);
#pragma unroll
  for (int t = 0; t < 7; ++t) {
    const int64_t r = l + t - 3;
    const float xv = (r >= 0 && r < L) ? x[r] : 0.f;
    v += *reinterpret_cast<const f32x4*>(w + t * C + cq * 4) * xv;
  }
  const size_t row = (size_t)b * L + (size_t)l;
  *reinterpret_cast<f32x4*>(out_raw + row * C + cq * 4) = v;
  const f32x4 al = *reinterpret_cast<const f32x4*>(alpha + cq * 4);
  f32x4 sn;
#pragma unroll
  for (int r = 0; r < 4; ++r) sn[r] = snake_f(v[r], al[r]);
  store_pair4(out_act, row, cq * 4, C, sn);
}

__global__ __launch_bounds__(256) void rvq_stage_kernel(float* __restrict__ residual ,
                                                        const float* __restrict__ in_w ,
                                                        const float* __restrict__ in_b, const float* __restrict__ cb ,
                                                        const float* __restrict__ out_w ,
                                                        const float* __restrict__ out_b, int32_t* __restrict__ codes, int latent,
                                                        int dim, int size, int T, int K, int k) {
  __shared__ float part[4][8];
  __shared__ float ze[8];
  __shared__ float bestv[4];
  __shared__ int besti[4];
  const int row = blockIdx.x, tid = threadIdx.x, lane = tid & 63, wv = tid >> 6;
  float* res = residual + (size_t)row * latent;
  float acc[8];
#pragma unroll
  for (int d = 0; d < 8; ++d) acc[d] = 0.f;
  for (int c = tid; c < latent; c += 256) {
    const float x = res[c];
#pragma unroll
    for (int d = 0; d < 8; ++d)
      if (d < dim) acc[d] = fmaf(in_w[(size_t)d * latent + c], x, acc[d]);
  }
#pragma unroll
  for (int d = 0; d < 8; ++d) {
    const float s = wave_sum(acc[d]);
    if (lane == 0) part[wv][d] = s;
  }
  __syncthreads();
  if (tid < 8) ze[tid] = tid < dim ? ((part[0][tid] + part[1][tid]) + (part[2][tid] + part[3][tid])) + in_b[tid] : 0.f;
  __syncthreads();
  float e[8], en2 = 0.f;
#pragma unroll
  for (int d = 0; d < 8; ++d) en2 = fmaf(ze[d], ze[d], en2);
  const float einv = 1.0f / fmaxf(sqrtf(en2), 1e-12f);
  float e2 = 0.f;
#pragma unroll
  for (int d = 0; d < 8; ++d) { e[d] = ze[d] * einv; e2 = fmaf(e[d], e[d], e2); }
  float bv = -INFINITY;
  int bi = 0x7fffffff;
  for (int j = tid; j < size; j += 256) {
    float c[8], cn2 = 0.f;
#pragma unroll
    for (int d = 0; d < 8; ++d) { c[d] = d < dim ? cb[(size_t)j * dim + d] : 0.f; cn2 = fmaf(c[d], c[d], cn2); }
    const float cinv = 1.0f / fmaxf(sqrtf(cn2), 1e-12f);
    float dot = 0.f, c2 = 0.f;
#pragma unroll
    for (int d = 0; d < 8; ++d) { const float cn = c[d] * cinv; dot = fmaf(e[d], cn, dot); c2 = fmaf(cn, cn, c2); }
    const float score = -((e2 - 2.0f * dot) + c2);
    if (score > bv) { bv = score; bi = j; }
  }
#pragma unroll
  for (int off = 32; off > 0; off >>= 1) {
    const float ov = __shfl_xor(bv, off, 64);
    const int oi = __shfl_xor(bi, off, 64);
    if (ov > bv || (ov == bv && oi < bi)) { bv = ov; bi = oi; }
  }
  if (lane == 0) { bestv[wv] = bv; besti[wv] = bi; }
  __syncthreads();
  float fv = bestv[0];
  int fi = besti[0];
#pragma unroll
  for (int w = 1; w < 4; ++w)
    if (bestv[w] > fv || (bestv[w] == fv && besti[w] < fi)) { fv = bestv[w]; fi = besti[w]; }
  float zq[8];
#pragma unroll
  for (int d = 0; d < 8; ++d) zq[d] = d < dim ? ze[d] + (cb[(size_t)fi * dim + d] - ze[d]) : 0.f;
  for (int c = tid; c < latent; c += 256) {
    float o = 0.f;
#pragma unroll
    for (int d = 0; d < 8; ++d)
      if (d < dim) o = fmaf(out_w[(size_t)c * dim + d], zq[d], o);
    res[c] -= o + out_b[c];
  }
  if (tid == 0) codes[((size_t)(row / T) * K + k) * T + (row % T)] = fi;
}

__global__ __launch_bounds__(256) void snake_kernel(const float* __restrict__ x, const float* __restrict__ alpha, float* __restrict__ y,
                                                    int64_t n, int C) {
  const int64_t i = (int64_t)blockIdx.x * 256 + threadIdx.x;
  if (i < n) y[i] = snake_f(x[i], alpha[i % C]);
}

static int launch_conv_out(const vaura_conv& co, const float* A, float* wav, int B, int L, int pr, hipStream_t s) {
  const int C = co.cin;
  if (co.cout != 1 || co.taps != 7 || (C % 4)) return VAURA_ERR_SHAPE;
  if (C <= 128 && C % 8 == 0 && !va_variant(VV_CODEC_LAST_CONV_UNTILED)) {
    const size_t sm = sizeof(float) * ((size_t)(CO_TL + 6) * (C + 4) + CO_TL);
    static unsigned long long big = 0;
    if (va_big_lds_once(reinterpret_cast<const void*>(conv_out_tiled_kernel), 80 * 1024, &big)) return VAURA_ERR_STATE;
    VA_LAUNCH(conv_out_tiled_kernel, dim3((L + CO_TL - 1) / CO_TL, B), dim3(256), sm, s, A, co.w, co.bias, wav, L, C, pr);
  } else {
    VA_LAUNCH(conv_out_kernel, dim3((L + 31) / 32, B), dim3(256), 0, s, A, co.w, co.bias, wav, L, C, pr);
  }
  return 0;
}

static unsigned va_clip_gx(int64_t items) {
  const int64_t g = (items + 255) / 256;
  return (unsigned)(g < 1 ? 1 : (g > 256 ? 256 : g));
}
static int va_clips_zero(const ClipLayout& l, void* buf, int64_t rate, size_t row_bytes, hipStream_t s) {
  const size_t unit = (size_t)rate * row_bytes;
  if (unit % 16) return VAURA_ERR_SHAPE;
  for (int b0 = 0; b0 < l.B - 1; b0 += VA_CLIP_CHUNK) {
    const ClipChunk k = va_clip_chunk(l, b0, l.B - 1);
    VA_LAUNCH(clips_zero_gaps_kernel, dim3(va_clip_gx((int64_t)((size_t)l.gap * unit / 16)), k.n), dim3(256), 0, s,
              reinterpret_cast<unsigned char*>(buf), k, unit, l.gap);
  }
  return 0;
}
extern "C" {

long long vaura_debug_counter(int which) {
  if (which == 1) {
    const long long v = va_conv_units_fused;
    va_conv_units_fused = 0;
    return v;
  }
  if (which != 0) return -1;
  const long long v = va_conv256_launches;
  va_conv256_launches = 0;
  return v;
}

size_t vaura_dac_workspace_elems(const vaura_codec* c, int B, int T) {
  if (!c || B <= 0 || T <= 0) return 0;
  size_t L = (size_t)T, best = (size_t)T * (size_t)c->latent_dim;
  int ch = c->conv_in.cout;
  if ((size_t)T * ch > best) best = (size_t)T * ch;
  for (int b = 0; b < c->n_blocks; ++b) {
    L *= (size_t)c->rates[b];
    ch = c->up[b].cout;
    if (L * ch > best) best = L * ch;
  }
  return best * (size_t)B;
}

static int va_dac_decode_pass(const vaura_codec* c, const int32_t* codes, int B, int T, float* wav, const ClipLayout* lay, hipStream_t s) {
  const int pr = c->precision;
  float* R = c->ws[0]; float* A = c->ws[1]; float* Y = c->ws[2]; float* Z = c->ws[3];
  const int Bc = B, Tc = T;
  int rc = 0;
  if (lay) {
    int32_t* packed = reinterpret_cast<int32_t*>(Z);
    for (int w0 = 0; lay->win && w0 < lay->B; w0 += VA_CLIP_CHUNK) {
      const WindowChunk k = va_window_pack_chunk(*lay, w0);
      int widest = 0;
      for (int i = 0; i < k.n; ++i) widest = std::max(widest, k.len[i]);
      if (lay->win->seq_S > 0) {
        SeqDelays dl;
        for (int q = 0; q < 16; ++q) dl.d[q] = lay->win->seq_delays[q];
        VA_LAUNCH(window_pack_seq_kernel, dim3(va_clip_gx(widest), k.n, c->n_codebooks), dim3(256), 0, s, codes, packed, k, dl,
                  lay->win->seq_K, lay->win->seq_S, lay->total, c->codebook_size);
        continue;
      }
      VA_LAUNCH(window_pack_codes_kernel, dim3(va_clip_gx(widest), k.n, c->n_codebooks), dim3(256), 0, s, codes, packed, k,
                c->n_codebooks, Tc, lay->total);
    }
    for (int b0 = 0; !lay->win && b0 < Bc; b0 += VA_CLIP_CHUNK) {
      const ClipChunk k = va_clip_chunk(*lay, b0, Bc);
      VA_LAUNCH(clips_pack_codes_kernel, dim3(va_clip_gx(Tc + lay->gap), k.n, c->n_codebooks), dim3(256), 0, s, codes, packed, k,
                c->n_codebooks, Tc, lay->total, lay->gap, Bc);
    }
    codes = packed; B = 1; T = (int)lay->total;
  }
  const size_t act_b = pr == 3 ? 1 : 4;

  VA_LAUNCH(from_codes_kernel, dim3((T + FC_NT - 1) / FC_NT, B), dim3(256), 0, s, codes, c->codebooks, c->out_proj_w, c->out_proj_b, Y,
                     c->n_codebooks, T, c->codebook_size, c->codebook_dim, c->latent_dim, pr ? 1 : 0);
  if (lay && (rc = va_clips_zero(*lay, Y, 1, (size_t)c->latent_dim * 4, s))) return rc;
  rc = launch_conv(c->conv_in, Y, nullptr, c->alpha_up[0], nullptr, A, B, T, pr, s);
  if (rc) return rc;
  if (lay && (rc = va_clips_zero(*lay, A, 1, c->conv_in.cout * act_b, s))) return rc;
  int L = T;
  for (int b = 0; b < c->n_blocks; ++b) {
    rc = launch_conv(c->up[b], A, nullptr, c->alpha_res[b][0][0], Y, Z, B, L, pr, s);
    if (rc) return rc;
    L *= c->rates[b];
    if (lay && (rc = va_clips_zero(*lay, Z, L / T, c->up[b].cout * act_b, s))) return rc;
    { float* t = R; R = Y; Y = t; t = A; A = Z; Z = t; }
    for (int u = 0; u < 3; ++u) {
      const float* next_alpha = (u < 2) ? c->alpha_res[b][u + 1][0] : (b + 1 < c->n_blocks ? c->alpha_up[b + 1] : c->alpha_out);
      rc = launch_conv_unit(c->res[b][u][0], c->res[b][u][1], A, R, c->alpha_res[b][u][1], next_alpha, (u < 2) ? R : nullptr, Y, B, L, pr, s);
      if (rc == 0) {
        float* t = A; A = Y; Y = t;
        if (lay && (rc = va_clips_zero(*lay, A, L / T, c->up[b].cout * act_b, s))) return rc;
        continue;
      }
      if (rc != VA_UNIT_NOT_ELIGIBLE) return rc;
      rc = launch_conv(c->res[b][u][0], A, nullptr, c->alpha_res[b][u][1], nullptr, Y, B, L, pr, s);
      if (rc) return rc;
      rc = launch_conv(c->res[b][u][1], Y, R, next_alpha, (u < 2) ? R : nullptr, A, B, L, pr, s);
      if (rc) return rc;
      if (lay && (rc = va_clips_zero(*lay, A, L / T, c->up[b].cout * act_b, s))) return rc;
    }
  }
  if (!lay) return launch_conv_out(c->conv_out, A, wav, B, L, pr, s);
  const int hop = L / T;
  rc = launch_conv_out(c->conv_out, A, R, B, L, pr, s);
  if (rc) return rc;
  for (int b0 = 0; lay->win && b0 < Bc; b0 += VA_CLIP_CHUNK) {
    const WindowChunk k = va_window_unpack_chunk(*lay, b0);
    const int64_t n_out = (int64_t)lay->win->n_max * hop;
    VA_LAUNCH(window_unpack_wav_kernel, dim3(va_clip_gx(n_out), k.n), dim3(256), 0, s, R, wav, k, n_out, hop);
  }
  for (int b0 = 0; !lay->win && b0 < Bc; b0 += VA_CLIP_CHUNK) {
    const ClipChunk k = va_clip_chunk(*lay, b0, Bc);
    VA_LAUNCH(clips_unpack_wav_kernel, dim3(va_clip_gx((int64_t)Tc * hop), k.n), dim3(256), 0, s, R, wav, k, (int64_t)Tc * hop, hop);
  }
  return 0;
}

int vaura_dac_decode(const vaura_codec* c, const int32_t* codes, int B, int T, float* wav, vaura_stream_t s_) {
  if (!c || !codes || !wav || B <= 0 || T <= 0) return VAURA_ERR_ARG;
  if (c->n_blocks < 1 || c->n_blocks > 4 || c->n_units != 3 || c->n_codebooks > 16 || c->codebook_dim > 8)
    return VAURA_ERR_SHAPE;
  if (c->ws_elems < vaura_dac_workspace_elems(c, B, T)) return VAURA_ERR_ARG;
  for (int i = 0; i < 4; ++i) if (!c->ws[i]) return VAURA_ERR_ARG;
  const int pr = c->precision;
  if (pr < 0 || pr > 4) return VAURA_ERR_DTYPE;
  return va_dac_decode_pass(c, codes, B, T, wav, nullptr, as_stream(s_));
}

int vaura_dac_clips_gap(const vaura_codec* c) { return c ? va_clips_gap_decode(c) : -1; }

static int64_t va_decode_clips_total(const vaura_codec* c, int B, int T_max, const int32_t* lengths, int* off, int* gap_out) {
  const int gap = va_clips_gap_decode(c);
  if (gap < 0) return 0;
  for (int b = 0; b < B; ++b)
    if (lengths[b] < 1 || (T_max > 0 && lengths[b] > T_max)) return 0;
  int64_t total = 0;
  if (!va_clips_offsets(lengths, B, gap, off, &total)) return -1;
  if (gap_out) *gap_out = gap;
  return total;
}
static size_t va_decode_clips_elems(const vaura_codec* c, int64_t total) {
  size_t need = vaura_dac_workspace_elems(c, 1, (int)total);
  const size_t kc = (size_t)c->n_codebooks * (size_t)total;
  return need > kc ? need : kc;
}

size_t vaura_dac_decode_clips_workspace_elems(const vaura_codec* c, int B, const int32_t* lengths) {
  if (!c || !lengths || B <= 0) return 0;
  std::vector<int> off((size_t)B);
  const int64_t total = va_decode_clips_total(c, B, 0, lengths, off.data(), nullptr);
  return total > 0 ? va_decode_clips_elems(c, total) : 0;
}

int vaura_dac_decode_clips(const vaura_codec* c, const int32_t* codes, int B, int T_max, const int32_t* lengths, float* wav,
                           vaura_stream_t s_) {
  if (!c || !codes || !wav || !lengths || B <= 0 || T_max <= 0) return VAURA_ERR_ARG;
  if (c->n_blocks < 1 || c->n_blocks > 4 || c->n_units != 3 || c->n_codebooks > 16 || c->codebook_dim > 8)
    return VAURA_ERR_SHAPE;
  std::vector<int> off((size_t)B), len(lengths, lengths + B);
  ClipLayout lay;
  lay.B = B; lay.off = off.data(); lay.len = len.data(); lay.aux = nullptr;
  lay.total = va_decode_clips_total(c, B, T_max, lengths, off.data(), &lay.gap);
  if (lay.total == 0) return VAURA_ERR_ARG;
  if (lay.total < 0 || va_decode_clips_elems(c, lay.total) > (size_t)0x7fffffff || (int64_t)B * T_max > 0x7fffffff) return VAURA_ERR_SHAPE;
  if (c->ws_elems < va_decode_clips_elems(c, lay.total)) return VAURA_ERR_ARG;
  for (int i = 0; i < 4; ++i) if (!c->ws[i]) return VAURA_ERR_ARG;
  const int pr = c->precision;
  if (pr < 0 || pr > 4) return VAURA_ERR_DTYPE;
  return va_dac_decode_pass(c, codes, B, T_max, wav, &lay, as_stream(s_));
}

int vaura_dac_decode_halo(const vaura_codec* c) { return c ? va_decode_halo(c) : -1; }

size_t vaura_dac_decode_window_workspace_elems(const vaura_codec* c, int B, const int32_t* lengths, const int32_t* starts,
                                               const int32_t* counts) {
  if (!c || !starts || !counts || B <= 0) return 0;
  const WindowPlan p = va_window_plan(c, B, 0, lengths, starts, counts, 0);
  return p.total > 0 ? va_decode_clips_elems(c, p.total) : 0;
}

static int va_dac_decode_window_any(const vaura_codec* c, const int32_t* codes, int B, int T_max, const int32_t* lengths, const int32_t* starts,
                                    const int32_t* counts, float* wav, int N_max, const SeqSource* sq, vaura_stream_t s_) {
  if (!c || !codes || !wav || !starts || !counts || B <= 0 || T_max <= 0 || N_max <= 0) return VAURA_ERR_ARG;
  if (c->n_blocks < 1 || c->n_blocks > 4 || c->n_units != 3 || c->n_codebooks > 16 || c->codebook_dim > 8)
    return VAURA_ERR_SHAPE;
  if (va_decode_halo(c) < 0) return VAURA_ERR_SHAPE;
  const WindowPlan p = va_window_plan(c, B, T_max, lengths, starts, counts, N_max);
  if (p.total == 0) return VAURA_ERR_ARG;
  if (sq)
    for (size_t w = 0; w < p.clip.size(); ++w)
      if ((int64_t)p.lo[w] + p.len[w] + sq->d_max > (int64_t)sq->S - 1) return VAURA_ERR_ARG;
  int64_t hop = 1;
  for (int b = 0; b < c->n_blocks; ++b) hop *= c->rates[b];
  const int64_t src_elems = sq ? (int64_t)B * sq->K * sq->S : (int64_t)B * T_max;
  if (p.total < 0 || va_decode_clips_elems(c, p.total) > (size_t)0x7fffffff || src_elems > 0x7fffffff ||
      (int64_t)N_max * hop > 0x7fffffff) return VAURA_ERR_SHAPE;
  if (c->ws_elems < va_decode_clips_elems(c, p.total)) return VAURA_ERR_ARG;
  for (int i = 0; i < 4; ++i) if (!c->ws[i]) return VAURA_ERR_ARG;
  const int pr = c->precision;
  if (pr < 0 || pr > 4) return VAURA_ERR_DTYPE;
  WindowLayout win;
  win.B = B; win.n_max = N_max; win.clip = p.clip.data(); win.lo = p.lo.data(); win.skip = p.skip.data();
  win.window = p.window.data(); win.count = p.count.data();
  if (sq) {
    win.seq_K = sq->K; win.seq_S = sq->S;
    for (int q = 0; q < 16; ++q) win.seq_delays[q] = sq->delays[q];
  }
  ClipLayout lay;
  lay.B = (int)p.clip.size(); lay.gap = p.gap; lay.total = p.total; lay.off = p.off.data(); lay.len = p.len.data(); lay.aux = nullptr;
  lay.win = &win;
  return va_dac_decode_pass(c, codes, B, T_max, wav, &lay, as_stream(s_));
}

int vaura_dac_decode_window(const vaura_codec* c, const int32_t* codes, int B, int T_max, const int32_t* lengths, const int32_t* starts,
                            const int32_t* counts, float* wav, int N_max, vaura_stream_t s_) {
  return va_dac_decode_window_any(c, codes, B, T_max, lengths, starts, counts, wav, N_max, nullptr, s_);
}

size_t vaura_dac_decode_window_seq_workspace_elems(const vaura_codec* c, int B, int K, int S, const int32_t* delays_host,
                                                   const int32_t* lengths, const int32_t* starts, const int32_t* counts) {
  SeqSource sq;
  if (!c || !starts || !counts || B <= 0 || !va_seq_source(c, K, S, delays_host, &sq)) return 0;
  const WindowPlan p = va_window_plan(c, B, S - 1 - sq.d_max, lengths, starts, counts, 0);
  return p.total > 0 ? va_decode_clips_elems(c, p.total) : 0;
}

int vaura_dac_decode_window_seq(const vaura_codec* c, const int32_t* seq, int B, int K, int S, const int32_t* delays_host,
                                const int32_t* lengths, const int32_t* starts, const int32_t* counts, float* wav, int N_max,
                                vaura_stream_t s_) {
  SeqSource sq;
  if (!c || !seq || B <= 0 || !va_seq_source(c, K, S, delays_host, &sq)) return VAURA_ERR_ARG;
  return va_dac_decode_window_any(c, seq, B, S - 1 - sq.d_max, lengths, starts, counts, wav, N_max, &sq, s_);
}

int vaura_snake(const float* x, const float* alpha, float* y, int64_t rows, int C, vaura_stream_t s_) {
  if (!x || !alpha || !y || rows <= 0 || C <= 0) return VAURA_ERR_ARG;
  const int64_t n = rows * C;
  VA_LAUNCH(snake_kernel, dim3((unsigned)((n + 255) / 256)), dim3(256), 0, as_stream(s_), x, alpha, y, n, C);
  return 0;
}

static int va_conv_input(const vaura_conv& cv, int precision, const float* in, float* scratch, int B, int L, hipStream_t s,
                         const float** x) {
  *x = in;
  if (!precision) return 0;
  if (!scratch) return VAURA_ERR_ARG;
  const bool mx = precision == 3 && cv.wscale;
  const size_t rows = (size_t)B * L, n = rows * (cv.cin / 8);
  uint8_t* sc = reinterpret_cast<uint8_t*>(scratch) + mx8_scale_offset(rows * cv.cin);
  VA_LAUNCH(act_convert_kernel, dim3((unsigned)((n + 255) / 256)), dim3(256), 0, s, in, scratch, sc, rows, cv.cin, mx ? 1 : 0);
  *x = scratch;
  return 0;
}

int vaura_dac_conv(const vaura_conv* cv, int precision, const float* in, float* out, float* scratch, int B, int Lin,
                   vaura_stream_t s_) {
  if (!cv || !in || !out || !scratch || B <= 0 || Lin <= 0 || precision < 0 || precision > 4) return VAURA_ERR_ARG;
  if (cv->cin % 32) return VAURA_ERR_SHAPE;
  hipStream_t s = as_stream(s_);
  const float* x = in;
  const int rc = va_conv_input(*cv, precision, in, scratch, B, Lin, s, &x);
  if (rc) return rc;
  return launch_conv(*cv, x, nullptr, nullptr, out, nullptr, B, Lin, precision, s);
}

int vaura_dac_conv_ex(const vaura_conv* cv, int precision, const float* in, const float* res, const float* alpha, float* out_raw,
                      void* out_act, float* scratch, int B, int Lin, vaura_stream_t s_) {
  if (!cv || !in || (!out_raw && !out_act) || (precision && !scratch) || B <= 0 || Lin <= 0 || precision < 0 || precision > 4)
    return VAURA_ERR_ARG;
  if (cv->cin % 32) return VAURA_ERR_SHAPE;
  hipStream_t s = as_stream(s_);
  const float* x = in;
  const int rc = va_conv_input(*cv, precision, in, scratch, B, Lin, s, &x);
  if (rc) return rc;
  return launch_conv(*cv, x, res, alpha, out_raw, reinterpret_cast<float*>(out_act), B, Lin, precision, s);
}

int vaura_dac_unit(const vaura_conv* c7, const vaura_conv* c1, int precision, const float* in, const float* res,
                   const float* alpha_mid, const float* alpha_next, float* out_raw, void* out_act, float* scratch, float* mid, int B,
                   int L, vaura_stream_t s_) {
  if (!c7 || !c1 || !in || !res || !alpha_mid || !alpha_next || !out_act || (precision && !scratch) || B <= 0 || L <= 0 ||
      precision < 0 || precision > 4)
    return VAURA_ERR_ARG;
  if (c7->cin % 32) return VAURA_ERR_SHAPE;
  hipStream_t s = as_stream(s_);
  const float* x = in;
  int rc = va_conv_input(*c7, precision, in, scratch, B, L, s, &x);
  if (rc) return rc;
  rc = launch_conv_unit(*c7, *c1, x, res, alpha_mid, alpha_next, out_raw, reinterpret_cast<float*>(out_act), B, L, precision, s);
  if (rc != VA_UNIT_NOT_ELIGIBLE) return rc;
  if (!mid) return VAURA_DAC_UNIT_TWO_LAUNCHES;
  rc = launch_conv(*c7, x, nullptr, alpha_mid, nullptr, mid, B, L, precision, s);
  if (rc) return rc;
  rc = launch_conv(*c1, mid, res, alpha_next, out_raw, reinterpret_cast<float*>(out_act), B, L, precision, s);
  return rc ? rc : VAURA_DAC_UNIT_TWO_LAUNCHES;
}

int vaura_dac_from_codes(const int32_t* codes, const float* codebooks, const float* out_proj_w, const float* out_proj_b, void* z,
                         int B, int K, int T, int size, int dim, int latent, int pairs, vaura_stream_t s_) {
  if (!codes || !codebooks || !out_proj_w || !out_proj_b || !z || B <= 0 || T <= 0) return VAURA_ERR_ARG;
  if (K < 1 || K > 16 || dim < 1 || dim > 8 || size < 1 || latent < 8 || (latent % 8)) return VAURA_ERR_SHAPE;
  VA_LAUNCH(from_codes_kernel, dim3((T + FC_NT - 1) / FC_NT, B), dim3(256), 0, as_stream(s_), codes, codebooks, out_proj_w, out_proj_b,
            reinterpret_cast<float*>(z), K, T, size, dim, latent, pairs ? 1 : 0);
  return 0;
}

int vaura_dac_conv_out(const vaura_conv* cv, int precision, const float* in, float* wav, float* scratch, int B, int L,
                       vaura_stream_t s_) {
  if (!cv || !cv->w || !cv->bias || !in || !wav || (precision && !scratch) || B <= 0 || L <= 0 || precision < 0 || precision > 4)
    return VAURA_ERR_ARG;
  if (precision && (cv->cin % 32)) return VAURA_ERR_SHAPE;
  hipStream_t s = as_stream(s_);
  const float* x = in;
  if (precision) {
    const size_t rows = (size_t)B * L, n = rows * (cv->cin / 8);
    uint8_t* sc = reinterpret_cast<uint8_t*>(scratch) + mx8_scale_offset(rows * cv->cin);
    VA_LAUNCH(act_convert_kernel, dim3((unsigned)((n + 255) / 256)), dim3(256), 0, s, in, scratch, sc, rows, cv->cin, precision == 3 ? 1 : 0);
    x = scratch;
  }
  return launch_conv_out(*cv, x, wav, B, L, precision, s);
}

size_t vaura_dac_encode_workspace_elems(const vaura_codec_encoder* c, int B, int64_t n_samples) {
  if (!c || B <= 0 || n_samples <= 0) return 0;
  size_t L = (size_t)n_samples, best = L * (size_t)c->enc_dim;
  int ch = c->enc_dim;
  for (int b = 0; b < c->n_blocks; ++b) {
    L /= (size_t)c->rates[b];
    ch *= 2;
    if (L * ch > best) best = L * ch;
  }
  if (L * (size_t)c->latent_dim > best) best = L * (size_t)c->latent_dim;
  return best * (size_t)B;
}

static int va_dac_encode_pass(const vaura_codec_encoder* c, const float* wav, int B, int64_t n_samples, int32_t* codes, const ClipLayout* lay,
                              int64_t hop, hipStream_t s) {
  float* R = c->ws[0]; float* A = c->ws[1]; float* Y = c->ws[2]; float* Z = c->ws[3];
  const int Bc = B;
  const int64_t n_in = n_samples;
  int rc = 0;
  if (lay) {
    for (int b0 = 0; b0 < Bc; b0 += VA_CLIP_CHUNK) {
      const ClipChunk k = va_clip_chunk(*lay, b0, Bc);
      VA_LAUNCH(clips_pack_wav_kernel, dim3(va_clip_gx(n_in + lay->gap * hop), k.n), dim3(256), 0, s, wav, Z, k, n_in, (int)hop, lay->gap, Bc);
    }
    wav = Z; B = 1; n_samples = lay->total * hop;
  }

  int64_t L = n_samples;
  int C = c->enc_dim;
  {
    const int64_t total = L * (C / 4);
    VA_LAUNCH(enc_conv_in_kernel, dim3((unsigned)((total + 255) / 256), B), dim3(256), 0, s, wav, c->conv_in_w, c->conv_in_b,
              c->alpha_res[0][0][0], R, reinterpret_cast<uint16_t*>(A), L, C);
  }
  if (lay && (rc = va_clips_zero(*lay, A, L / lay->total, (size_t)C * 4, s))) return rc;
  for (int b = 0; b < c->n_blocks; ++b) {
    for (int u = 0; u < 3; ++u) {
      rc = launch_conv(c->res[b][u][0], A, nullptr, c->alpha_res[b][u][1], nullptr, Y, B, (int)L, 1, s);
      if (rc) return rc;
      const float* next_alpha = (u < 2) ? c->alpha_res[b][u + 1][0] : c->alpha_down[b];
      rc = launch_conv(c->res[b][u][1], Y, R, next_alpha, (u < 2) ? R : nullptr, A, B, (int)L, 1, s);
      if (rc) return rc;
      if (lay && (rc = va_clips_zero(*lay, A, L / lay->total, (size_t)C * 4, s))) return rc;
    }
    const int r = c->rates[b];
    const bool last = b + 1 == c->n_blocks;
    rc = launch_conv(c->down[b], A, nullptr, last ? c->alpha_out : c->alpha_res[b + 1][0][0], last ? nullptr : Y, Z, B, (int)(L / r), 1, s);
    if (rc) return rc;
    L /= r;
    C *= 2;
    if (lay && (rc = va_clips_zero(*lay, Z, L / lay->total, (size_t)C * 4, s))) return rc;
    { float* t = R; R = Y; Y = t; t = A; A = Z; Z = t; }
  }
  rc = launch_conv(c->conv_out, A, nullptr, nullptr, Y, nullptr, B, (int)L, 1, s);
  if (rc) return rc;
  const int T = (int)L;
  int32_t* codes_out = lay ? reinterpret_cast<int32_t*>(Z) : codes;
  for (int k = 0; k < c->n_codebooks; ++k) {
    VA_LAUNCH(rvq_stage_kernel, dim3((unsigned)(B * T)), dim3(256), 0, s, Y,
              c->in_proj_w + (size_t)k * c->codebook_dim * c->latent_dim, c->in_proj_b + (size_t)k * c->codebook_dim,
              c->codebooks + (size_t)k * c->codebook_size * c->codebook_dim,
              c->out_proj_w + (size_t)k * c->latent_dim * c->codebook_dim, c->out_proj_b + (size_t)k * c->latent_dim, codes_out,
              c->latent_dim, c->codebook_dim, c->codebook_size, T, c->n_codebooks, k);
  }
  if (!lay) return 0;
  const int T_max = (int)((n_in + hop - 1) / hop);
  for (int b0 = 0; b0 < Bc; b0 += VA_CLIP_CHUNK) {
    const ClipChunk k = va_clip_chunk(*lay, b0, Bc);
    VA_LAUNCH(clips_unpack_codes_kernel, dim3(va_clip_gx(T_max), k.n, c->n_codebooks), dim3(256), 0, s, codes_out, codes, k, c->n_codebooks,
              T_max, lay->total);
  }
  return 0;
}

static bool va_encoder_shape_ok(const vaura_codec_encoder* c) {
  return !(c->n_blocks < 1 || c->n_blocks > 4 || c->n_units != 3 || c->n_codebooks > 16 || c->codebook_dim > 8 ||
           c->codebook_size > 1024 || c->latent_dim > 2048 || (c->enc_dim % 32));
}

int vaura_dac_encode(const vaura_codec_encoder* c, const float* wav, int B, int64_t n_samples, int32_t* codes, vaura_stream_t s_) {
  if (!c || !wav || !codes || B <= 0 || n_samples <= 0) return VAURA_ERR_ARG;
  if (!va_encoder_shape_ok(c)) return VAURA_ERR_SHAPE;
  int64_t hop = 1;
  for (int b = 0; b < c->n_blocks; ++b) hop *= c->rates[b];
  if (n_samples % hop) return VAURA_ERR_SHAPE;
  if (c->ws_elems < vaura_dac_encode_workspace_elems(c, B, n_samples)) return VAURA_ERR_ARG;
  for (int i = 0; i < 4; ++i) if (!c->ws[i]) return VAURA_ERR_ARG;
  return va_dac_encode_pass(c, wav, B, n_samples, codes, nullptr, hop, as_stream(s_));
}

int vaura_dac_encode_clips_gap(const vaura_codec_encoder* c) { return c ? va_clips_gap_encode(c, nullptr) : -1; }

static int64_t va_encode_clips_total(const vaura_codec_encoder* c, int B, int64_t n_max, const int64_t* n, int* frames, int* off, int* gap_out,
                                     int64_t* hop_out) {
  int64_t hop = 1;
  const int gap = va_clips_gap_encode(c, &hop);
  if (gap < 0) return 0;
  for (int b = 0; b < B; ++b) {
    if (n[b] < 1 || (n_max > 0 && n[b] > n_max)) return 0;
    const int64_t f = (n[b] + hop - 1) / hop;
    if (f > 0x7fffffff) return -1;
    frames[b] = (int)f;
  }
  int64_t total = 0;
  if (!va_clips_offsets(frames, B, gap, off, &total)) return -1;
  if (gap_out) *gap_out = gap;
  if (hop_out) *hop_out = hop;
  return total;
}
static size_t va_encode_clips_elems(const vaura_codec_encoder* c, int64_t total, int64_t hop) {
  const size_t need = vaura_dac_encode_workspace_elems(c, 1, total * hop);
  const size_t kc = (size_t)c->n_codebooks * (size_t)total;
  return need > kc ? need : kc;
}

size_t vaura_dac_encode_clips_workspace_elems(const vaura_codec_encoder* c, int B, const int64_t* sample_lengths) {
  if (!c || !sample_lengths || B <= 0) return 0;
  std::vector<int> off((size_t)B), frames((size_t)B);
  int64_t hop = 1;
  const int64_t total = va_encode_clips_total(c, B, 0, sample_lengths, frames.data(), off.data(), nullptr, &hop);
  if (total <= 0 || total > 0x7fffffff / hop) return 0;
  return va_encode_clips_elems(c, total, hop);
}

int vaura_dac_encode_clips(const vaura_codec_encoder* c, const float* wav, int B, int64_t n_max, const int64_t* sample_lengths,
                           int32_t* codes, vaura_stream_t s_) {
  if (!c || !wav || !codes || !sample_lengths || B <= 0 || n_max <= 0) return VAURA_ERR_ARG;
  if (!va_encoder_shape_ok(c)) return VAURA_ERR_SHAPE;
// ... 38 lines not shown
```

vaura_amd/csrc/gemv3.hip:

```cpp
#include "gemv3_kernel.h"
#include "mlp_engine.h"
#include <cstdlib>

unsigned va_debug_flags = 0;
unsigned va_debug_flags2 = 0;
unsigned va_debug_flags_get() { return va_debug_flags; }
unsigned va_debug_flags2_get() { return va_debug_flags2; }
extern "C" void vaura_set_debug_flags(unsigned flags) { va_debug_flags = flags; }
extern "C" void vaura_set_debug_flags2(unsigned flags) { va_debug_flags2 = flags; }
VA_STAMP_SETTER(vaura_stamps_set_gemv3)

static bool rb2(const Gemv3Args& a) { return a.R >= 2 && !va_variant(VV_ROW_BLOCKS_WALK); }

template <int WT, int G, int NW, int T, int EPI, bool NORM, int XB = 1, int KS = 1, bool RB2 = false, int XBR = XB>
static int launch3(const Gemv3Args& a, int64_t n_tiles, hipStream_t s) {
  if (n_tiles % T) return VAURA_ERR_SHAPE;
  if constexpr (RB2) {
    if (rb2(a)) {
      VA_LAUNCH((gemv3_kernel<G, NW, T, EPI, NORM, XBR, 0, WT, KS, 2>), dim3((unsigned)(n_tiles / T * KS)), dim3(NW * 64), 0, s, a.W, a.XP, a);
      return 0;
    }
  }
  VA_LAUNCH((gemv3_kernel<G, NW, T, EPI, NORM, XB, 0, WT, KS>), dim3((unsigned)(n_tiles / T * KS)), dim3(NW * 64), 0, s, a.W, a.XP, a);
  return 0;
}


template <int WT, int G2, int EPI, int XB, int NBF = 2, int NW = 8, bool RB2 = false>
static int launch3h(const Gemv3Args& a, int64_t n_tiles, hipStream_t s) {
  const int halves = (a.R == 1 && a.rows <= 8) ? 1 : 2;
  if (halves == 2 && (n_tiles % 8)) return VAURA_ERR_SHAPE;
  if constexpr (RB2) {
    if (rb2(a)) {
      VA_LAUNCH((gemv3h_kernel<G2, NW, EPI, XB, WT, NBF, 2>), dim3((unsigned)(n_tiles * halves)), dim3(NW * 64), 0, s, a.W, a.XP, a, halves);
      return 0;
    }
  }
  VA_LAUNCH((gemv3h_kernel<G2, NW, EPI, XB, WT, NBF>), dim3((unsigned)(n_tiles * halves)), dim3(NW * 64), 0, s, a.W, a.XP, a, halves);
  return 0;
}

template <int WT>
static int dispatch3(const Gemv3Args& a, int64_t tiles, int64_t K, int epilogue, bool norm, hipStream_t s) {
  constexpr int XB2 = WT == 2 ? 3 : 1, XB4 = 4;
  if constexpr (WT == 1 || WT == 3) {
    if (a.R >= 2 && !norm && !va_variant(VV_ROWSPLIT_OFF) && !va_variant(VV_FP8_ROWSPLIT_OFF) && tiles % 8 == 0 && epilogue == E3_RESID) {
      if (K == 1536) return launch3h<WT, 3, E3_RESID, 1, 2, 8, true>(a, tiles, s);
      if (K == 4096) return launch3h<WT, 8, E3_RESID, 1, 2, 8, true>(a, tiles, s);
    }
  }
  if constexpr (WT != 1 && WT != 3) {
    if (!norm && !va_variant(VV_ROWSPLIT_OFF) && tiles % 8 == 0 && (epilogue == E3_RESID || epilogue == E3_STORE)) {
      if (K == 1536 && epilogue == E3_RESID) return launch3h<WT, 3, E3_RESID, 1, 2, 8, true>(a, tiles, s);
      if (K == 1536 && epilogue == E3_STORE) return launch3h<WT, 3, E3_STORE, 1>(a, tiles, s);
      if (K == 4096 && epilogue == E3_RESID) return launch3h<WT, 8, E3_RESID, (WT == 2 ? 4 : 1), 2, 8, true>(a, tiles, s);
      if (K == 4096 && epilogue == E3_STORE) return launch3h<WT, 8, E3_STORE, (WT == 2 ? 4 : 1)>(a, tiles, s);
    }
  }
  if (K == 1536) {
    if (epilogue == E3_STORE && norm) return launch3<WT, 6, 8, 2, E3_STORE, true, XB2>(a, tiles, s);
    if (epilogue == E3_STORE && !norm) return launch3<WT, 6, 8, 1, E3_STORE, false>(a, tiles, s);
    if (epilogue == E3_RESID && !norm) return launch3<WT, 6, 8, 1, E3_RESID, false, 1, 1, true>(a, tiles, s);
    if (epilogue == E3_SWIGLU && norm) return launch3<WT, 6, 8, 2, E3_SWIGLU, true, XB2, 1, true, 3>(a, tiles, s);
    if (epilogue == E3_LOGITS && norm) return launch3<WT, 6, 8, 3, E3_LOGITS, true, XB2, 1, true, 3>(a, tiles, s);
  } else if (K == 4096) {
    if (epilogue == E3_RESID && !norm) return launch3<WT, 16, 8, 1, E3_RESID, false, XB4, 1, true>(a, tiles, s);
    if (epilogue == E3_STORE && !norm) return launch3<WT, 16, 8, 1, E3_STORE, false, XB4>(a, tiles, s);
  }
  return VAURA_ERR_SHAPE;
}

template <int EPI, bool NORM>
static int launch_gemm3(const Gemv3Args& a, int64_t tiles, int64_t K, hipStream_t s) {
  const int gx = (int)(tiles / (G3M_NW * G3M_T)), gy4 = (a.R + G3M_RB - 1) / G3M_RB, gy8 = (a.R + 7) / 8;
  const bool big = !va_variant(VV_PREFILL_GEMM_64_ROWS) && (va_variant(VV_GEMM3_ROUND2_TILE_RULE) ? a.R >= 64 : gx * gy8 >= 320);
  const int remap = va_variant(VV_PREFILL_GEMM_LAUNCH_ORDER) ? 0 : 1;
  const bool pf2 = !va_variant(VV_GEMM3_ONE_KGROUP) && (K / 32) % 2 == 0;
  const int gy = big ? gy8 : gy4;
  const dim3 grid((unsigned)(gx * gy)), block(G3M_NW * 64);
  if (a.wq == 1 || a.wq == 3) {
    if (big) VA_LAUNCH((gemm3_kernel<EPI, NORM, 1, 8>), grid, block, 0, s, a, (int)K, gx, gy, remap);
    else VA_LAUNCH((gemm3_kernel<EPI, NORM, 1>), grid, block, 0, s, a, (int)K, gx, gy, remap);
  } else if (a.wq == 2) {
    if (big && pf2) VA_LAUNCH((gemm3_kernel<EPI, NORM, 2, 8, 2>), grid, block, 0, s, a, (int)K, gx, gy, remap);
    else if (big) VA_LAUNCH((gemm3_kernel<EPI, NORM, 2, 8, 1>), grid, block, 0, s, a, (int)K, gx, gy, remap);
    else if (pf2) VA_LAUNCH((gemm3_kernel<EPI, NORM, 2, G3M_RB, 2>), grid, block, 0, s, a, (int)K, gx, gy, remap);
    else VA_LAUNCH((gemm3_kernel<EPI, NORM, 2>), grid, block, 0, s, a, (int)K, gx, gy, remap);
  } else {
    if (big && pf2) VA_LAUNCH((gemm3_kernel<EPI, NORM, 0, 8, 2>), grid, block, 0, s, a, (int)K, gx, gy, remap);
    else if (big) VA_LAUNCH((gemm3_kernel<EPI, NORM, 0, 8, 1>), grid, block, 0, s, a, (int)K, gx, gy, remap);
    else if (pf2) VA_LAUNCH((gemm3_kernel<EPI, NORM, 0, G3M_RB, 2>), grid, block, 0, s, a, (int)K, gx, gy, remap);
    else VA_LAUNCH((gemm3_kernel<EPI, NORM, 0>), grid, block, 0, s, a, (int)K, gx, gy, remap);
  }
  return 0;
}

template <int EPI, bool NORM, int WT, int RBW, int CT = G4_CT>
static int launch_gemm4_i(const Gemv3Args& a, int64_t K, int gx, int rb_off, int n_rb, hipStream_t s) {
  using SH = G4Shape<WT, RBW, CT>;
  static unsigned long long big = 0;
  if (va_big_lds_once(reinterpret_cast<const void*>(gemm4_kernel<EPI, NORM, WT, RBW, CT>), SH::LDS, &big)) return VAURA_ERR_STATE;
  const int gy = (n_rb + RBW - 1) / RBW;
  VA_LAUNCH((gemm4_kernel<EPI, NORM, WT, RBW, CT>), dim3((unsigned)(gx * gy)), dim3(G4_NW * 64), SH::LDS, s, a, (int)K, gx, gy,
            (va_variant(VV_PREFILL_GEMM_LAUNCH_ORDER) ? 0 : 1) | (va_variant(VV_GEMM4_NO_DMA) ? 2 : 0),
            rb_off);
  return 0;
}
template <int EPI, bool NORM, int WT>
static int launch_gemm4_h(const Gemv3Args& a, int64_t K, int gx, int rbw, int rb_off, int n_rb, hipStream_t s) {
  if (rbw == 8) return launch_gemm4_i<EPI, NORM, WT, 8>(a, K, gx, rb_off, n_rb, s);
  if (rbw == 6) return launch_gemm4_i<EPI, NORM, WT, 6>(a, K, gx, rb_off, n_rb, s);
  return launch_gemm4_i<EPI, NORM, WT, 4>(a, K, gx, rb_off, n_rb, s);
}
template <int EPI, bool NORM>
static int launch_gemm4(const Gemv3Args& a, int64_t tiles, int64_t K, hipStream_t s) {
  const int gx = (int)(tiles / G4_CT);
  const int cand[3] = {8, 6, 4};
  const float eff[3] = {1.0f, 1.03f, a.wq == 2 ? 1.12f : 0.95f};
  auto rounds = [&](int rb, int h) { return (float)((gx * ((rb + h - 1) / h) + 255) / 256); };
  int h1 = 4, h2 = 0, cut = 0;
  if (!va_variant(VV_PREFILL_GEMM_64_ROWS)) {
    float best = 1e30f;
    for (int i = 0; i < 3; ++i) {
      const float c1 = rounds(a.R, cand[i]) * cand[i] * eff[i];
      if (c1 < best) { best = c1; h1 = cand[i]; h2 = 0; cut = 0; }
      if (cand[i] == 4 || a.wq != 2 || va_variant(VV_PREFILL_GEMM_NO_CUT)) continue;
      const int full = gx * ((a.R + cand[i] - 1) / cand[i]) / 256;
      const int gy1 = full * 256 / gx, rb1 = gy1 * cand[i];
      if (full < 1 || gy1 < 1 || rb1 >= a.R) continue;
      for (int k = 0; k < 3; ++k) {
        const float c2 = (float)full * cand[i] * eff[i] + rounds(a.R - rb1, cand[k]) * cand[k] * eff[k] + 0.3f;
        if (c2 < best) { best = c2; h1 = cand[i]; h2 = cand[k]; cut = rb1; }
      }
    }
  }
  int rc;
  if (a.wq == 2 && h1 == 4 && !h2 && !va_variant(VV_PREFILL_GEMM_64x256) && !va_variant(VV_PREFILL_GEMM_64_ROWS))
    return launch_gemm4_i<EPI, NORM, 2, 8, 8>(a, K, 2 * gx, 0, a.R, s);
  if (a.wq == 2) {
    rc = launch_gemm4_h<EPI, NORM, 2>(a, K, gx, h1, 0, h2 ? cut : a.R, s);
    if (!rc && h2) rc = launch_gemm4_h<EPI, NORM, 2>(a, K, gx, h2, cut, a.R - cut, s);
  } else {
    rc = launch_gemm4_h<EPI, NORM, 0>(a, K, gx, h1, 0, h2 ? cut : a.R, s);
    if (!rc && h2) rc = launch_gemm4_h<EPI, NORM, 0>(a, K, gx, h2, cut, a.R - cut, s);
  }
  return rc;
}

static int dispatch_gemm3(const Gemv3Args& a, int64_t tiles, int64_t K, int epilogue, bool norm, hipStream_t s) {
  if (a.wq != 1 && a.wq != 3 && !va_variant(VV_PREFILL_GEMM_REGISTER_STAGED)) {
    if (epilogue == E3_STORE && norm) return launch_gemm4<E3_STORE, true>(a, tiles, K, s);
    if (epilogue == E3_STORE && !norm) return launch_gemm4<E3_STORE, false>(a, tiles, K, s);
    if (epilogue == E3_RESID && !norm) return launch_gemm4<E3_RESID, false>(a, tiles, K, s);
    if (epilogue == E3_SWIGLU && norm) return launch_gemm4<E3_SWIGLU, true>(a, tiles, K, s);
    if (epilogue == E3_LOGITS && norm) return launch_gemm4<E3_LOGITS, true>(a, tiles, K, s);
    return VAURA_ERR_SHAPE;
  }
  if (epilogue == E3_STORE && norm) return launch_gemm3<E3_STORE, true>(a, tiles, K, s);
  if (epilogue == E3_STORE && !norm) return launch_gemm3<E3_STORE, false>(a, tiles, K, s);
  if (epilogue == E3_RESID && !norm) return launch_gemm3<E3_RESID, false>(a, tiles, K, s);
  if (epilogue == E3_SWIGLU && norm) return launch_gemm3<E3_SWIGLU, true>(a, tiles, K, s);
  if (epilogue == E3_LOGITS && norm) return launch_gemm3<E3_LOGITS, true>(a, tiles, K, s);
// ... 230 lines not shown
```

vaura_amd/csrc/variants.h:

```cpp
#pragma once
#include "../../include/vaura_hip.h"

#define VA_VARIANTS(X)                                                                                                                 \
  X(ROWSPLIT_OFF, 1, 0, "wo / w2 on the one-workgroup-per-tile GEMV instead of the row-split pair")                                    \
  X(QKV_OWN_LAUNCH, 1, 1, "the next layer's qkv GEMV stays its own launch (not the MLP launch's third phase)")                         \
  X(MLP_TWO_LAUNCHES, 1, 2, "w1||w3 and w2 as two launches even where the one-launch MLP (mlp_engine.h) is eligible")                  \
  X(PREFILL_ATTN_PER_POSITION, 1, 4, "fp32 cache: per-position prefill attention instead of the MFMA kernel")                          \
  X(PREFILL_GEMM_64_ROWS, 1, 5, "64-row prefill GEMM workgroups only")                                                                 \
  X(VIT_SPACE_THREAD_PER_QUERY, 1, 7, "extractor space attention with one thread per query instead of the MFMA kernels")               \
  X(VIT_CLS_UNSPLIT, 1, 9, "extractor CLS attention on the one-workgroup-per-(sequence, head) kernel")                                 \
  X(VIT_TIME_THREAD_PER_HEAD_FRAME, 1, 10, "extractor time attention with one thread per (head, frame)")                               \
  X(VIT_SPACE_FP32_MFMA, 1, 11, "extractor space attention on the exact-fp32 MFMA instead of fp16 pairs")                              \
  X(CODEC_LAST_CONV_UNTILED, 1, 13, "the codec's last conv (C -> 1) without the LDS-staged window")                                    \
  X(GEMM3_ROUND2_TILE_RULE, 1, 14, "gemm3_kernel only: round 2's tile rule (128-row workgroups from 64 row blocks up)")                \
  X(PREFILL_GEMM_LAUNCH_ORDER, 1, 15, "prefill GEMM workgroups in launch order (no XCD tile order)")                                   \
  X(GEMM3_ONE_KGROUP, 1, 16, "gemm3_kernel only: one k-group of planes and weights in flight")                                         \
  X(PREFILL_GEMM_REGISTER_STAGED, 1, 17, "prefill GEMMs on the register-staged gemm3_kernel for every storage (fp8 always uses it)")   \
  X(GEMM4_NO_DMA, 1, 18, "gemm4_kernel ablation for tools/time_prefill_gemm.py: no DMA in the loop (WRONG RESULTS, timing only)")      \
  X(ATTN_MERGE_OWN_LAUNCH, 1, 19, "range-split attention: the merge of the partials as its own launch, not by the last split to arrive") \
  X(CODEC_128_ROWS, 1, 20, "codec convs in 128-row workgroups only (no 256-row instances, no one-launch residual units)")              \
  X(CODEC_UNIT_TWO_LAUNCHES, 1, 21, "codec residual units as two launches even where one workgroup holds every channel (C = 96, 192)") \
  X(PREFILL_GEMM_NO_CUT, 1, 22, "prefill GEMMs never cut into two launches of different workgroup heights")                            \
  X(PREFILL_GEMM_64x256, 1, 23, "two-plane prefill GEMMs with few column tiles (wo, w2) in 64 x 256 workgroups instead of 128 x 128")  \
  X(ROW_BLOCKS_WALK, 2, 0, "17..32 decoder rows: the GEMVs walk the two row blocks one after the other instead of both per weight pass") \
  X(ENGINE_MAX_16_ROWS, 2, 1, "the one-launch MLP refuses more than 16 rows (the separate two-row-block launches run instead)")        \
  X(FP8_ROWSPLIT_OFF, 2, 3, "fp8 weights, 17..32 rows: wo / w2 on one workgroup per tile instead of the fp8 row-split pair instances") \
  X(FP8_NO_ENGINE, 2, 4, "fp8 weights never take the one-launch MLP")                                                                  \
  X(LINEAR_REGISTER_STAGED, 2, 5, "extractor linear layers on the register-staged linear_pair_kernel, not linear_dma_kernel (bit-identical)") \
  X(LINEAR_DMA_LATE_FRAGMENTS, 2, 6, "extractor linear layers: LDS-DMA kernel with the fragments read beside their matrix instructions")

#define VA_VARIANT_FIELDS(X)                                                                                                           \
  X(GRAPH_STEPS, 1, 24, 4, "decode steps per graph launch (1..15; 0 = the default VA_GRAPH_STEPS), read by vaura_step_graph_build")    \
  X(ENGINE_ABL, 1, 28, 4, "MlpEngineArgs::abl, timing only: 1 = no flag waits (WRONG RESULTS); 4: see the struct; 8 = no run-ahead throttle") \
  X(LINEAR_PANEL, 2, 12, 4, "extractor linear layers: column-tile panel of n tiles where n divides the tile count (15 = the whole width)")

enum VaVariant : unsigned {
#define X(name, word, bit, effect) VV_##name = ((word) - 1) * 32 + (bit),
  VA_VARIANTS(X)
#undef X
};
enum VaVariantField : unsigned {
#define X(name, word, shift, width, effect) VF_##name = ((width) << 8) | (((word) - 1) * 32 + (shift)),
  VA_VARIANT_FIELDS(X)
#undef X
};

constexpr bool va_variants_disjoint() {
  unsigned seen[2] = {0u, 0u};
  bool ok = true;
#define X(name, word, bit, effect) ok = ok && (word) >= 1 && (word) <= 2 && (bit) < 32 && !(seen[(word) - 1] >> (bit) & 1u), seen[(word) - 1] |= 1u << (bit);
  VA_VARIANTS(X)
#undef X
#define X(name, word, shift, width, effect)                                                                                  \
  ok = ok && (word) >= 1 && (word) <= 2 && (width) >= 1 && (shift) + (width) <= 32 &&                                        \
       !(seen[(word) - 1] & (unsigned)(((1ull << (width)) - 1) << (shift))),                                                 \
  seen[(word) - 1] |= (unsigned)(((1ull << (width)) - 1) << (shift));
  VA_VARIANT_FIELDS(X)
#undef X
  return ok;
}
static_assert(va_variants_disjoint(), "two kernel-variant switches overlap within a word (or leave it)");

unsigned va_debug_flags_get();
unsigned va_debug_flags2_get();

inline bool va_variant(VaVariant v) { return ((v < 32 ? va_debug_flags_get() : va_debug_flags2_get()) >> (v & 31u)) & 1u; }
inline unsigned va_variant_field(VaVariantField f) {
  return (((f & 255u) < 32 ? va_debug_flags_get() : va_debug_flags2_get()) >> (f & 31u)) & ((1u << (f >> 8)) - 1u);
}

struct VaVariantWords {
  unsigned w1 = 0, w2 = 0;
  static VaVariantWords current() { return {va_debug_flags_get(), va_debug_flags2_get()}; }
  void set() const { vaura_set_debug_flags(w1); vaura_set_debug_flags2(w2); }
};
class VaVariantScope {
  const VaVariantWords saved = VaVariantWords::current();
 public:
  explicit VaVariantScope(const VaVariantWords& w) { w.set(); }
  ~VaVariantScope() { saved.set(); }
  VaVariantScope(const VaVariantScope&) = delete;
  VaVariantScope& operator=(const VaVariantScope&) = delete;
};
```

vaura_amd/engine.py:

```python
from __future__ import annotations

import contextlib
import ctypes as C
import math
import os
from typing import Dict, Optional, Sequence

import torch

from . import _lib as L
from . import clip_params
from . import ops
from .synth import CodecCfg, SamplerCfg, fold_weight_norm


def rope_table(n_pos: int, head_dim: int, base: int = 10000) -> torch.Tensor:
    inv = 1.0 / (base ** (torch.arange(0, head_dim, 2)[: head_dim // 2].float() / head_dim))
    ang = torch.outer(torch.arange(n_pos), inv)
    z = torch.polar(torch.ones_like(ang), ang)
    return torch.stack([z.real, z.imag], dim=-1).contiguous()


_PRIVATE_STREAMS: Dict[torch.device, "torch.cuda.Stream"] = {}

# ... 1233 lines not shown
        for name, v in (("starts", starts), ("counts", counts)):
            if not clip_params.is_per_clip(v):
                raise L.VauraHipError(f"{name} must be one integer per clip (a list, tuple or 1-D tensor), got {v!r}")
            v = clip_params._int_list(name, v)
            if len(v) != B:
                raise L.VauraHipError(f"{name} has {len(v)} values for a batch of {B} clips")
            out.append(v)
        s, c = out
        if any(a < 0 or k < 0 or a + k > t for a, k, t in zip(s, c, n)):
            raise L.VauraHipError(f"every window must lie inside its clip: lengths {n}, starts {s}, counts {c}")
        if max(c) < 1:
            raise L.VauraHipError(f"decode_window: every count is 0, there is nothing to decode (counts {c})")
        return s, c

    @torch.no_grad()
    def decode_window(self, codes: torch.Tensor, starts, counts, lengths=None) -> torch.Tensor:
        B, K, T = codes.shape
        n = [T] * B if lengths is None else _clip_lengths("lengths", lengths, B, T)
        s, c = self._window_args(B, n, starts, counts)
        with off_null_stream(self.dev) as caller:
            ci = codes.to(self.dev, torch.int32).contiguous()
            wav = self._window_call(ci, n, s, c)
            self._codes_keepalive = ci
        if caller is not None:
            wav.record_stream(caller)
        return wav

    @torch.no_grad()
    def decode_window_seq(self, seq: torch.Tensor, starts, counts, lengths=None, delays: Optional[Sequence[int]] = None) -> torch.Tensor:
        if seq.dim() != 3 or seq.dtype != torch.int32 or not seq.is_cuda or not seq.is_contiguous():
            raise L.VauraHipError(f"seq must be a contiguous (B, K, S) int32 tensor on {self.dev}, got {tuple(seq.shape)} {seq.dtype} on {seq.device}")
        B, K, S = seq.shape
        d = None if delays is None else L.check_delays(delays, K)
        T = S - 1 - (K - 1 if d is None else max(d))
        if K < self.cfg.n_codebooks or T < 1:
            raise L.VauraHipError(f"a pattern sequence of {K} codebooks and {S} steps under the delays {list(d) if d else list(range(K))} holds "
                                  f"no frame of the codec's {self.cfg.n_codebooks} codebooks")
        n = [T] * B if lengths is None else _clip_lengths("lengths", lengths, B, T)
        s, c = self._window_args(B, n, starts, counts)
        with off_null_stream(self.dev) as caller:
            wav = self._window_call(seq, n, s, c, seq_delays=d)
        if caller is not None:
            wav.record_stream(caller)
        return wav

    @torch.no_grad()
    def decode_windowed(self, codes: torch.Tensor, window: int, lengths=None) -> torch.Tensor:
        B, K, T = codes.shape
        if isinstance(window, bool) or not isinstance(window, int) or window < 1:
            raise L.VauraHipError(f"window must be a positive number of frames, got {window!r}")
        n = [T] * B if lengths is None else _clip_lengths("lengths", lengths, B, T)
        if window >= T:
            return self.decode(codes) if lengths is None or min(n) == T else self.decode_clips(codes, n)
        hop = self.cfg.hop
        with off_null_stream(self.dev) as caller:
            ci = codes.to(self.dev, torch.int32).contiguous()
            wav = torch.zeros(B, 1, T * hop, dtype=torch.float32, device=self.dev)
            for s in range(0, max(n), window):
                counts = [max(0, min(window, t - s)) for t in n]
                part = self._window_call(ci, n, [min(s, t) for t in n], counts)
                wav[:, :, s * hop:s * hop + part.shape[-1]] = part
            self._codes_keepalive = ci
        if caller is not None:
            wav.record_stream(caller)
        return wav


class CodecConvOp:

    def __init__(self, weight: torch.Tensor, bias: torch.Tensor, dilation: int = 1, stride: int = 1, precision: str = "f16pair",
                 device="cuda:0", mx8_weights: bool = True):
        _require_cuda(device)
        self.dev, self.lib, self._keep = torch.device(device), L.lib(), []
        self.pairs = CODEC_PRECISIONS[precision]
        self.cv = L.Conv()
        CodecEngine._pack_conv(self, self.cv, weight.float(), bias.float(), dilation, stride, mx8_weights)
        self.stride = stride

    _dev = CodecEngine._dev

    @torch.no_grad()
    def __call__(self, x: torch.Tensor) -> torch.Tensor:
        B, Lin, cin = x.shape
        assert cin == self.cv.cin
        with off_null_stream(self.dev) as caller:
            xi = x.to(self.dev, torch.float32).contiguous()
            out = torch.empty(B, Lin * self.stride, self.cv.cout, dtype=torch.float32, device=self.dev)
            scratch = torch.empty(B * Lin * cin + 64, dtype=torch.float32, device=self.dev)
            L.check(self.lib.vaura_dac_conv(C.byref(self.cv), self.pairs, L.ptr(xi), L.ptr(out), L.ptr(scratch), B, Lin,
                                            L.current_stream(self.dev)), "vaura_dac_conv")
            self._keepalive = (xi, scratch)
        if caller is not None:
            out.record_stream(caller)
        return out


    @torch.no_grad()
    def ex(self, x: torch.Tensor, res: Optional[torch.Tensor] = None, alpha: Optional[torch.Tensor] = None,
           out_raw: Optional[torch.Tensor] = None, out_act: Optional[torch.Tensor] = None) -> None:
        B, Lin, cin = x.shape
        assert cin == self.cv.cin and (out_raw is not None or out_act is not None)
        _cuda_contiguous(res, alpha, out_raw, out_act)
        with off_null_stream(self.dev):
            xi = x.to(self.dev, torch.float32).contiguous()
            scratch = torch.empty(B * Lin * cin + 64, dtype=torch.float32, device=self.dev)
            L.check(self.lib.vaura_dac_conv_ex(C.byref(self.cv), self.pairs, L.ptr(xi), L.ptr(res), L.ptr(alpha), L.ptr(out_raw),
                                               L.ptr(out_act), L.ptr(scratch), B, Lin, L.current_stream(self.dev)), "vaura_dac_conv_ex")
            self._keepalive = (xi, scratch)


def _cuda_contiguous(*ts):
    for t in ts:
        if t is not None and not (t.is_cuda and t.is_contiguous()):
            raise L.VauraHipError("op-level codec entry: contiguous tensors on a HIP device expected")


def codec_act_bytes(precision: str, rows: int, Cc: int) -> int:
    if precision != "mx8":
        return 4 * rows * Cc
    return ((rows * Cc + 15) & ~15) + rows * ((Cc + 127) // 128) * 4


class CodecUnitOp:

    def __init__(self, w7: torch.Tensor, b7: torch.Tensor, dilation: int, w1: torch.Tensor, b1: torch.Tensor,
                 precision: str = "f16pair", device="cuda:0"):
        _require_cuda(device)
        self.dev, self.lib, self._keep = torch.device(device), L.lib(), []
        self.pairs = CODEC_PRECISIONS[precision]
        self.c7, self.c1 = L.Conv(), L.Conv()
        CodecEngine._pack_conv(self, self.c7, w7.float(), b7.float(), dilation, 1)
        CodecEngine._pack_conv(self, self.c1, w1.float(), b1.float(), 1, 1)

    _dev = CodecEngine._dev

    @torch.no_grad()
    def __call__(self, x: torch.Tensor, res: torch.Tensor, alpha_mid: torch.Tensor, alpha_next: torch.Tensor,
                 out_raw: Optional[torch.Tensor], out_act: torch.Tensor, mid: Optional[torch.Tensor] = None) -> bool:
        B, Ln, cin = x.shape
        assert cin == self.c7.cin and res.shape == x.shape
        _cuda_contiguous(res, alpha_mid, alpha_next, out_raw, out_act, mid)
        with off_null_stream(self.dev):
            xi = x.to(self.dev, torch.float32).contiguous()
            scratch = torch.empty(B * Ln * cin + 64, dtype=torch.float32, device=self.dev)
            rc = self.lib.vaura_dac_unit(C.byref(self.c7), C.byref(self.c1), self.pairs, L.ptr(xi), L.ptr(res), L.ptr(alpha_mid),
                                         L.ptr(alpha_next), L.ptr(out_raw), L.ptr(out_act), L.ptr(scratch), L.ptr(mid), B, Ln,
                                         L.current_stream(self.dev))
            self._keepalive = (xi, scratch)
        if rc == L.DAC_UNIT_TWO_LAUNCHES:
            return False
        L.check(rc, "vaura_dac_unit")
        return True


@torch.no_grad()
def codec_from_codes(codes: torch.Tensor, codebooks: torch.Tensor, out_proj_w: torch.Tensor, out_proj_b: torch.Tensor,
                     out: torch.Tensor, pairs: bool) -> None:
    _cuda_contiguous(codes, codebooks, out_proj_w, out_proj_b, out)
    assert codes.dtype == torch.int32
    B, K, T = codes.shape
    _, size, dim = codebooks.shape
    latent = out_proj_w.shape[1]
    with off_null_stream(out.device):
        L.check(L.lib().vaura_dac_from_codes(L.ptr(codes), L.ptr(codebooks), L.ptr(out_proj_w), L.ptr(out_proj_b), L.ptr(out), B, K, T,
                                             size, dim, latent, 1 if pairs else 0, L.current_stream(out.device)), "vaura_dac_from_codes")


@torch.no_grad()
def codec_conv_out(w: torch.Tensor, bias: torch.Tensor, x: torch.Tensor, out: torch.Tensor, precision: str = "f16pair") -> None:
    _cuda_contiguous(x, out)
    dev = x.device
    pairs = CODEC_PRECISIONS[precision]
    B, Ln, Cc = x.shape
    cv = L.Conv()
    wl = w.float()[0].t().contiguous().to(dev)
    bl = bias.float().contiguous().to(dev)
    cv.w, cv.bias, cv.cin, cv.cout, cv.taps, cv.dilation, cv.stride = L.ptr(wl), L.ptr(bl), Cc, 1, 7, 1, 1
    with off_null_stream(dev):
        xi = x.float().contiguous()
        scratch = torch.empty(B * Ln * Cc + 64, dtype=torch.float32, device=dev)
        L.check(L.lib().vaura_dac_conv_out(C.byref(cv), pairs, L.ptr(xi), L.ptr(out), L.ptr(scratch), B, Ln, L.current_stream(dev)),
                "vaura_dac_conv_out")
        torch.cuda.current_stream(dev).synchronize()


@torch.no_grad()
def codec_enc_conv_in(wav: torch.Tensor, w: torch.Tensor, bias: torch.Tensor, alpha: torch.Tensor, out_raw: torch.Tensor,
                      out_act: torch.Tensor) -> None:
    _cuda_contiguous(wav, w, bias, alpha, out_raw, out_act)
    B, Ln = wav.shape
    with off_null_stream(wav.device):
        L.check(L.lib().vaura_dac_enc_conv_in(L.ptr(wav), L.ptr(w), L.ptr(bias), L.ptr(alpha), L.ptr(out_raw), L.ptr(out_act), B, Ln,
                                              w.shape[1], L.current_stream(wav.device)), "vaura_dac_enc_conv_in")


@torch.no_grad()
def codec_rvq_stage(residual: torch.Tensor, in_w: torch.Tensor, in_b: torch.Tensor, codebook: torch.Tensor, out_w: torch.Tensor,
                    out_b: torch.Tensor, codes: torch.Tensor, k: int) -> None:
    _cuda_contiguous(residual, in_w, in_b, codebook, out_w, out_b, codes)
    assert codes.dtype == torch.int32
    B, T, latent = residual.shape
    size, dim = codebook.shape
    with off_null_stream(residual.device):
        L.check(L.lib().vaura_dac_rvq_stage(L.ptr(residual), L.ptr(in_w), L.ptr(in_b), L.ptr(codebook), L.ptr(out_w), L.ptr(out_b),
                                            L.ptr(codes), B, T, latent, dim, size, codes.shape[1], k,
                                            L.current_stream(residual.device)), "vaura_dac_rvq_stage")


def snake(x: torch.Tensor, alpha: torch.Tensor, device="cuda:0") -> torch.Tensor:
    _require_cuda(device)
    dev = torch.device(device)
    with off_null_stream(dev) as caller:
        xi = x.to(dev, torch.float32).contiguous()
        al = alpha.to(dev, torch.float32).contiguous()
        y = torch.empty_like(xi)
        L.check(L.lib().vaura_snake(L.ptr(xi), L.ptr(al), L.ptr(y), xi.numel() // xi.shape[-1], xi.shape[-1], L.current_stream(dev)),
                "vaura_snake")
    if caller is not None:
        y.record_stream(caller)
    return y


class CodecEncoderEngine:

    def __init__(self, cfg: CodecCfg, sd: Dict[str, torch.Tensor], device="cuda:0"):
        _require_cuda(device)
        self.cfg, self.dev, self.lib = cfg, torch.device(device), L.lib()
        self._keep = []
        c = L.CodecEncoder()
        c.n_codebooks, c.codebook_size, c.codebook_dim, c.latent_dim = (cfg.n_codebooks, cfg.codebook_size,
                                                                        cfg.codebook_dim, cfg.latent_dim)
        nb = len(cfg.encoder_rates)
        assert nb <= 4 and len(cfg.dilations) == 3
        c.n_blocks, c.n_units, c.enc_dim = nb, 3, cfg.encoder_dim
        for i, r in enumerate(cfg.encoder_rates):
            c.rates[i] = r
        K = cfg.n_codebooks
        f = lambda p: fold_weight_norm(sd[p + "weight_g"].float(), sd[p + "weight_v"].float())
        q = "quantizer.quantizers."
        c.in_proj_w = L.ptr(self._dev(torch.stack([f(f"{q}{k}.in_proj.")[:, :, 0] for k in range(K)])))
        c.in_proj_b = L.ptr(self._dev(torch.stack([sd[f"{q}{k}.in_proj.bias"].float() for k in range(K)])))
        c.codebooks = L.ptr(self._dev(torch.stack([sd[f"{q}{k}.codebook.weight"].float() for k in range(K)])))
        c.out_proj_w = L.ptr(self._dev(torch.stack([f(f"{q}{k}.out_proj.")[:, :, 0] for k in range(K)])))
        c.out_proj_b = L.ptr(self._dev(torch.stack([sd[f"{q}{k}.out_proj.bias"].float() for k in range(K)])))
        w0 = f("encoder.block.0.")
        c.conv_in_w = L.ptr(self._dev(w0[:, 0, :].t()))
        c.conv_in_b = L.ptr(self._dev(sd["encoder.block.0.bias"]))
        d = cfg.encoder_dim
        for b, r in enumerate(cfg.encoder_rates):
            p = f"encoder.block.{b + 1}.block."
            for u, dil in enumerate(cfg.dilations):
                qq = p + f"{u}.block."
                c.alpha_res[b][u][0] = L.ptr(self._dev(sd[qq + "0.alpha"].reshape(-1)))
                self._conv(c.res[b][u][0], f(qq + "1.").permute(2, 0, 1), sd[qq + "1.bias"], dil)
                c.alpha_res[b][u][1] = L.ptr(self._dev(sd[qq + "2.alpha"].reshape(-1)))
                self._conv(c.res[b][u][1], f(qq + "3.").permute(2, 0, 1), sd[qq + "3.bias"], 1)
            c.alpha_down[b] = L.ptr(self._dev(sd[p + "3.alpha"].reshape(-1)))
            self._conv(c.down[b], self.strided_as_three_taps(f(p + "4."), r), sd[p + "4.bias"], 1)
            d *= 2
        n = nb + 1
        c.alpha_out = L.ptr(self._dev(sd[f"encoder.block.{n}.alpha"].reshape(-1)))
        self._conv(c.conv_out, f(f"encoder.block.{n + 1}.").permute(2, 0, 1), sd[f"encoder.block.{n + 1}.bias"], 1)
        self.c = c
        self._ws_key = None

    @staticmethod
    def strided_as_three_taps(w: torch.Tensor, r: int) -> torch.Tensor:
        cout, cin, k = w.shape
        assert k == 2 * r and r % 2 == 0
        out = torch.zeros(3, cout, r * cin, dtype=w.dtype)
        for tau in (-1, 0, 1):
            for qi in range(r):
                t = tau * r + qi + r // 2
                if 0 <= t < k:
                    out[tau + 1, :, qi * cin:(qi + 1) * cin] = w[:, :, t]
        return out

    def _dev(self, t):
        d = t.detach().to(self.dev, torch.float32).contiguous()
        self._keep.append(d)
        return d

    def _conv(self, cv: L.Conv, wl: torch.Tensor, bias: torch.Tensor, dilation: int):
        wl = wl.contiguous().float()
        taps, cout, cin = wl.shape
        hi = wl.half()
        lo = (wl - hi.float()).half()
        pr = torch.stack([hi.reshape(taps, cout, cin // 8, 8), lo.reshape(taps, cout, cin // 8, 8)], dim=-2)
        keep = pr.contiguous().to(self.dev)
        self._keep.append(keep)
        cv.w = L.ptr(keep)
        cv.bias = L.ptr(self._dev(bias))
        cv.cin, cv.cout, cv.taps, cv.dilation, cv.stride = cin, cout, taps, dilation, 1

    @torch.no_grad()
    def encode(self, wav: torch.Tensor) -> torch.Tensor:
        if wav.dim() == 1:
            wav = wav[None]
        if wav.dim() == 3:
            wav = wav[:, 0]
        hop = int(math.prod(self.cfg.encoder_rates))
        B, N = wav.shape
        T = (N + hop - 1) // hop
        with off_null_stream(self.dev) as caller:
            x = torch.zeros(B, T * hop, dtype=torch.float32, device=self.dev)
            x[:, :N] = wav.to(self.dev, torch.float32)
# ... 137 lines not shown
```

vaura_amd/variants.py:

```python
from __future__ import annotations

import contextlib
import enum
import os


class Variant(enum.IntFlag):
    ROWSPLIT_OFF = 1 << 0
    QKV_OWN_LAUNCH = 1 << 1
    MLP_TWO_LAUNCHES = 1 << 2
    PREFILL_ATTN_PER_POSITION = 1 << 4
    PREFILL_GEMM_64_ROWS = 1 << 5
    VIT_SPACE_THREAD_PER_QUERY = 1 << 7
    VIT_CLS_UNSPLIT = 1 << 9
    VIT_TIME_THREAD_PER_HEAD_FRAME = 1 << 10
    VIT_SPACE_FP32_MFMA = 1 << 11
    CODEC_LAST_CONV_UNTILED = 1 << 13
    GEMM3_ROUND2_TILE_RULE = 1 << 14
    PREFILL_GEMM_LAUNCH_ORDER = 1 << 15
    GEMM3_ONE_KGROUP = 1 << 16
    PREFILL_GEMM_REGISTER_STAGED = 1 << 17
    GEMM4_NO_DMA = 1 << 18
    ATTN_MERGE_OWN_LAUNCH = 1 << 19
    CODEC_128_ROWS = 1 << 20
    CODEC_UNIT_TWO_LAUNCHES = 1 << 21
    PREFILL_GEMM_NO_CUT = 1 << 22
    PREFILL_GEMM_64x256 = 1 << 23


class Variant2(enum.IntFlag):
    ROW_BLOCKS_WALK = 1 << 0
    ENGINE_MAX_16_ROWS = 1 << 1
    FP8_ROWSPLIT_OFF = 1 << 3
    FP8_NO_ENGINE = 1 << 4
    LINEAR_REGISTER_STAGED = 1 << 5
    LINEAR_DMA_LATE_FRAGMENTS = 1 << 6


FIELDS = {"GRAPH_STEPS": (1, 24, 4), "ENGINE_ABL": (1, 28, 4), "LINEAR_PANEL": (2, 12, 4)}


def _field(name: str, n: int) -> int:
    _, shift, width = FIELDS[name]
    if not 0 <= n < (1 << width):
        raise ValueError(f"{name} takes 0..{(1 << width) - 1}, not {n}")
    return n << shift


def graph_steps(n: int) -> int:
    return _field("GRAPH_STEPS", n)


def engine_abl(n: int) -> int:
    return _field("ENGINE_ABL", n)


def linear_panel(n: int) -> int:
    return _field("LINEAR_PANEL", n)


_open = False


@contextlib.contextmanager
def variants(word1: int = 0, word2: int = 0, lib=None):
    global _open
    if _open:
        raise RuntimeError("variants() does not nest: the words are process-global (pass every switch to one call)")
    if lib is None:
        from . import _lib
        lib = _lib.lib()
    _open = True
    try:
        lib.vaura_set_debug_flags(int(word1))
        lib.vaura_set_debug_flags2(int(word2))
        yield
    finally:
        lib.vaura_set_debug_flags(0)
        lib.vaura_set_debug_flags2(0)
        _open = False


def parse(text: str, names=Variant) -> int:
    word = 0
    for part in text.replace(",", "|").split("|"):
        part = part.strip()
        if part:
            word |= int(names[part]) if part in names.__members__ else int(part, 0)
    return word


def from_env(environ=None):
    e = os.environ if environ is None else environ
    return parse(e.get("VAURA_DEBUG_FLAGS", "0"), Variant), parse(e.get("VAURA_DEBUG_FLAGS2", "0"), Variant2)
```

Baseline: 74940.

## Fuse input Snake into codec residual-unit kernels, passing raw fp32 stream between units

Residual units in the codec decoder now read the raw fp32 residual stream and apply Snake plus the f16 hi/lo split while staging the input tile into LDS. The producer therefore no longer writes a separate activated pair tensor. This removes one activated-tensor write and read per unit and lets the residual come from the same input buffer. In exchange each unit reads fp32 input, which is twice the bytes of the f16 pairs, and recomputes Snake for the halo rows. It also adds LDS alpha tables, an extra barrier, and a third variant word to switch back to the old handover.

```diff
diff --git a/include/vaura_hip.h b/include/vaura_hip.h
--- a/include/vaura_hip.h
+++ b/include/vaura_hip.h
@@ -311,6 +311,8 @@
 int vaura_dac_unit(const vaura_conv* c7, const vaura_conv* c1, int precision, const float* in, const float* res,
                    const float* alpha_mid, const float* alpha_next, float* out_raw, void* out_act, float* scratch, float* mid, int B,
                    int L, vaura_stream_t s);
+int vaura_dac_unit_raw(const vaura_conv* c7, const vaura_conv* c1, int precision, const float* in, const float* alpha_in,
+                       const float* alpha_mid, const float* alpha_next, float* out_raw, void* out_act, int B, int L, vaura_stream_t s);
 int vaura_dac_from_codes(const int32_t* codes, const float* codebooks, const float* out_proj_w, const float* out_proj_b, void* z,
                          int B, int K, int T, int size, int dim, int latent, int pairs, vaura_stream_t s);
 int vaura_dac_conv_out(const vaura_conv* cv, int precision, const float* in, float* wav, float* scratch, int B, int L,
@@ -462,6 +464,7 @@
 
 void vaura_set_debug_flags(unsigned flags);
 void vaura_set_debug_flags2(unsigned flags);
+void vaura_set_debug_flags3(unsigned flags);
 long long vaura_debug_counter(int which);
 
 const char* vaura_version(void);
diff --git a/vaura_amd/_lib.py b/vaura_amd/_lib.py
--- a/vaura_amd/_lib.py
+++ b/vaura_amd/_lib.py
@@ -181,6 +181,7 @@
     "vaura_version": (C.c_char_p, []),
     "vaura_set_debug_flags": (None, [C.c_uint]),
     "vaura_set_debug_flags2": (None, [C.c_uint]),
+    "vaura_set_debug_flags3": (None, [C.c_uint]),
     "vaura_debug_counter": (C.c_longlong, [C.c_int]),
     "vaura_struct_size": (C.c_size_t, [C.c_int]),
     "vaura_packed_weight_bytes": (C.c_size_t, [C.c_int64, C.c_int64, C.c_int]),
@@ -271,6 +272,8 @@
                                     C.c_int, C.c_int, C.c_void_p]),
     "vaura_dac_unit": (C.c_int, [C.POINTER(Conv), C.POINTER(Conv), C.c_int, C.c_void_p, C.c_void_p, C.c_void_p, C.c_void_p, C.c_void_p,
                                  C.c_void_p, C.c_void_p, C.c_void_p, C.c_int, C.c_int, C.c_void_p]),
+    "vaura_dac_unit_raw": (C.c_int, [C.POINTER(Conv), C.POINTER(Conv), C.c_int, C.c_void_p, C.c_void_p, C.c_void_p, C.c_void_p, C.c_void_p,
+                                     C.c_void_p, C.c_int, C.c_int, C.c_void_p]),
     "vaura_dac_from_codes": (C.c_int, [C.c_void_p, C.c_void_p, C.c_void_p, C.c_void_p, C.c_void_p, C.c_int, C.c_int, C.c_int, C.c_int,
                                        C.c_int, C.c_int, C.c_int, C.c_void_p]),
     "vaura_dac_conv_out": (C.c_int, [C.POINTER(Conv), C.c_int, C.c_void_p, C.c_void_p, C.c_void_p, C.c_int, C.c_int, C.c_void_p]),
diff --git a/vaura_amd/csrc/dac.hip b/vaura_amd/csrc/dac.hip
--- a/vaura_amd/csrc/dac.hip
+++ b/vaura_amd/csrc/dac.hip
@@ -100,8 +100,8 @@
 
 #define XHALO 56
 #define XROWS (BM + XHALO)
-template <int NI, bool WS, bool XS = false, int MJ = 4, bool FUSE = false>
-__global__ __launch_bounds__(256, 2) void conv_pair_kernel(ConvPArgs a) {
+template <int NI, bool WS, bool XS, int MJ, bool FUSE, bool RAWIN>
+__device__ __forceinline__ void conv_pair_body(ConvPArgs a, const float* alpha_in) {
   constexpr int BN_ = 32 * NI;
   constexpr int BMT = 32 * MJ;
   constexpr int XROWS_T = BMT + XHALO;
@@ -116,7 +116,8 @@
   constexpr int W1_ELEMS = FUSE ? 3 * (BK / 4) * W1STR : 0, Y_ELEMS = FUSE ? 3 * (BK / 4) * YSTR : 0;
   static_assert(!FUSE || Y_ELEMS * 16 >= 64 * SP * 4, "the 64-row output tile is staged over the activated tile");
   constexpr int SMEM_ELEMS = (WS_ELEMS + XS_ELEMS) > (W1_ELEMS + Y_ELEMS) ? (WS_ELEMS + XS_ELEMS) : (W1_ELEMS + Y_ELEMS);
-  constexpr int TAB_ELEMS = FUSE ? 2 * BN_ / 4 : 0;
+  static_assert(!RAWIN || FUSE, "raw input: the one-launch unit only (Cin = BN_)");
+  constexpr int TAB_ELEMS = FUSE ? (RAWIN ? 4 : 2) * BN_ / 4 : 0;
   __shared__ u32x4 smem[SMEM_ELEMS + TAB_ELEMS];
   auto coff = [](int kq) { return (kq & 1) + ((kq >> 2) << 1); };
   auto Ws = [&](int buf, int kq, int row) -> u32x4& { return smem[(buf * (BK / 4) + kq) * WSTR + row + coff(kq)]; };
@@ -138,6 +139,8 @@
   const int xrows = BMT + span;
   constexpr int XL = (XROWS_T * (BK / 4) + 255) / 256;
 
+  static_assert(!RAWIN || XL % 2 == 0, "raw input: a thread stages whole octets (two fp32 quads)");
+
   u32x4 wreg[NI], xreg[XL];
   auto load_w = [&](int kt) {
     const int c = kt / NT, t = kt - c * NT;
@@ -155,6 +158,17 @@
   };
   auto load_x = [&](int c) {
     const int q0 = c * (BK / 4);
+    if constexpr (RAWIN) {
+#pragma unroll
+      for (int i = 0; i < XL / 2; ++i) {
+        const int od = tid + 256 * i, row = od >> 2, o = od & 3;
+        const int jr = j0 + lo_off + row;
+        const bool ok = row < xrows && jr >= 0 && jr < a.Lin;
+        xreg[2 * i] = ok ? in[(size_t)jr * cq + q0 + 2 * o] : u32x4{0u, 0u, 0u, 0u};
+        xreg[2 * i + 1] = ok ? in[(size_t)jr * cq + q0 + 2 * o + 1] : u32x4{0u, 0u, 0u, 0u};
+      }
+      return;
+    }
 #pragma unroll
     for (int i = 0; i < XL; ++i) {
       const int qd = tid + 256 * i, row = qd >> 3, kq = qd & 7;
@@ -162,7 +176,30 @@
       xreg[i] = (row < xrows && jr >= 0 && jr < a.Lin) ? in[(size_t)jr * cq + q0 + kq] : u32x4{0u, 0u, 0u, 0u};
     }
   };
-  auto store_x = [&](int buf) {
+  auto store_x = [&](int buf, int c) {
+    if constexpr (RAWIN) {
+      const float* tin = reinterpret_cast<const float*>(smem + SMEM_ELEMS) + 2 * BN_ + c * BK + 8 * (tid & 3);
+      const f32x4 al0 = *reinterpret_cast<const f32x4*>(tin), al1 = *reinterpret_cast<const f32x4*>(tin + 4);
+      const f32x4 iv0 = *reinterpret_cast<const f32x4*>(tin + BN_), iv1 = *reinterpret_cast<const f32x4*>(tin + BN_ + 4);
+#pragma unroll
+      for (int i = 0; i < XL / 2; ++i) {
+        const int od = tid + 256 * i, row = od >> 2, o = od & 3;
+        if (row >= XROWS_T) continue;
+        const int jr = j0 + lo_off + row;
+        const f32x4 v0 = __builtin_bit_cast(f32x4, xreg[2 * i]), v1 = __builtin_bit_cast(f32x4, xreg[2 * i + 1]);
+        f16x8 h, l;
+#pragma unroll
+        for (int e = 0; e < 4; ++e) {
+          const float s0 = snake_fi(v0[e], al0[e], iv0[e]), s1 = snake_fi(v1[e], al1[e], iv1[e]);
+          h[e] = (_Float16)s0; l[e] = (_Float16)(s0 - (float)h[e]);
+          h[e + 4] = (_Float16)s1; l[e + 4] = (_Float16)(s1 - (float)h[e + 4]);
+        }
+        if (!(row < xrows && jr >= 0 && jr < a.Lin)) h = l = f16x8{0, 0, 0, 0, 0, 0, 0, 0};
+        Xs(buf, 2 * o, row) = __builtin_bit_cast(u32x4, h);
+        Xs(buf, 2 * o + 1, row) = __builtin_bit_cast(u32x4, l);
+      }
+      return;
+    }
 #pragma unroll
     for (int i = 0; i < XL; ++i) {
       const int qd = tid + 256 * i;
@@ -181,14 +218,23 @@
   load_w(0);
   load_x(0);
   store_w(0);
-  store_x(0);
+  if constexpr (!RAWIN) store_x(0, 0);
   if constexpr (FUSE) {
     if (tid < BN_) {
       float* tab = reinterpret_cast<float*>(smem + SMEM_ELEMS);
       const float al = a.alpha_mid[tid];
       tab[tid] = al;
       tab[BN_ + tid] = 1.0f / (al + 1e-9f);
-    }
+      if constexpr (RAWIN) {
+        const float ai = alpha_in[tid];
+        tab[2 * BN_ + tid] = ai;
+        tab[3 * BN_ + tid] = 1.0f / (ai + 1e-9f);
+      }
+    }
+  }
+  if constexpr (RAWIN) {
+    __syncthreads();
+    store_x(0, 0);
   }
   __syncthreads();
   VA_STAMP(stamps, 1);
@@ -228,7 +274,7 @@
       if (kt + 1 < nk) store_w(buf ^ 1);
       if (t == NT - 1 && c + 1 < kc) {
         if constexpr (NXB == 1) __syncthreads();
-        store_x(NXB == 2 ? (xb ^ 1) : 0);
+        store_x(NXB == 2 ? (xb ^ 1) : 0, c + 1);
       }
       __syncthreads();
     }
@@ -348,6 +394,12 @@
   VA_STAMP(stamps, 6);
   VA_STAMP_FLUSH(stamps, 20);
 }
+template <int NI, bool WS, bool XS = false, int MJ = 4, bool FUSE = false>
+__global__ __launch_bounds__(256, 2) void conv_pair_kernel(ConvPArgs a) { conv_pair_body<NI, WS, XS, MJ, FUSE, false>(a, nullptr); }
+template <bool WS, bool XS>
+__global__ __launch_bounds__(256, 2) void conv_pair_raw_kernel(ConvPArgs a, const float* alpha_in) {
+  conv_pair_body<3, WS, XS, 8, true, true>(a, alpha_in);
+}
 
 template <int N, typename F>
 __device__ __forceinline__ void va_static_for(F&& f) {
@@ -357,8 +409,8 @@
   }
 }
 
-template <int NCT, int RB, bool WS, bool XS>
-__global__ __launch_bounds__(256, 2) void conv_unit_kernel(ConvPArgs a) {
+template <int NCT, int RB, bool WS, bool XS, bool RAWIN>
+__device__ __forceinline__ void conv_unit_body(ConvPArgs a, const float* alpha_in) {
   constexpr int C_ = 16 * NCT;
   constexpr int BMT = 64 * RB;
   constexpr int KC = C_ / BK;
@@ -368,7 +420,7 @@
   constexpr int SP = BN + 4;
   constexpr int W2_ELEMS = 2 * (BK / 4) * W2STR, ST_ELEMS = 64 * SP / 4;
   constexpr int MAIN_ELEMS = WS_ELEMS + XS_ELEMS > W2_ELEMS + ST_ELEMS ? WS_ELEMS + XS_ELEMS : W2_ELEMS + ST_ELEMS;
-  constexpr int TAB_ELEMS = 2 * C_ / 4;
+  constexpr int TAB_ELEMS = (RAWIN ? 4 : 2) * C_ / 4;
   static_assert(NCT % 6 == 0 && (RB == 2 || RB == 4) && NCT * RB == 24, "96 channels x 256 rows or 192 x 128: 96 accumulator registers");
   __shared__ u32x4 smem[MAIN_ELEMS + TAB_ELEMS];
   auto coff = [](int kq) { return (kq & 1) + ((kq >> 2) << 1); };
@@ -389,6 +441,7 @@
   const int xrows = BMT + span;
   constexpr int WL = C_ * (BK / 4) / 256;
   constexpr int XL = (XROWS_T * (BK / 4) + 255) / 256;
+  static_assert(!RAWIN || XL % 2 == 0, "raw input: a thread stages whole octets (two fp32 quads)");
 
   u32x4 wreg[WL], xreg[XL];
   auto load_w = [&](int kt) {
@@ -405,6 +458,17 @@
     }
   };
   auto load_x = [&](int c) {
+    if constexpr (RAWIN) {
+#pragma unroll
+      for (int i = 0; i < XL / 2; ++i) {
+        const int od = tid + 256 * i, row = od >> 2, o = od & 3;
+        const int jr = j0 + lo_off + row;
+        const bool ok = row < xrows && jr >= 0 && jr < a.Lin;
+        xreg[2 * i] = ok ? in[(size_t)jr * cq + c * (BK / 4) + 2 * o] : u32x4{0u, 0u, 0u, 0u};
+        xreg[2 * i + 1] = ok ? in[(size_t)jr * cq + c * (BK / 4) + 2 * o + 1] : u32x4{0u, 0u, 0u, 0u};
+      }
+      return;
+    }
 #pragma unroll
     for (int i = 0; i < XL; ++i) {
       const int qd = tid + 256 * i, row = qd >> 3, kq = qd & 7;
@@ -412,7 +476,30 @@
       xreg[i] = (row < xrows && jr >= 0 && jr < a.Lin) ? in[(size_t)jr * cq + c * (BK / 4) + kq] : u32x4{0u, 0u, 0u, 0u};
     }
   };
-  auto store_x = [&]() {
+  auto store_x = [&](int c) {
+    if constexpr (RAWIN) {
+      const float* tin = tab + 2 * C_ + c * BK + 8 * (tid & 3);
+      const f32x4 al0 = *reinterpret_cast<const f32x4*>(tin), al1 = *reinterpret_cast<const f32x4*>(tin + 4);
+      const f32x4 iv0 = *reinterpret_cast<const f32x4*>(tin + C_), iv1 = *reinterpret_cast<const f32x4*>(tin + C_ + 4);
+#pragma unroll
+      for (int i = 0; i < XL / 2; ++i) {
+        const int od = tid + 256 * i, row = od >> 2, o = od & 3;
+        if (row >= XROWS_T) continue;
+        const int jr = j0 + lo_off + row;
+        const f32x4 v0 = __builtin_bit_cast(f32x4, xreg[2 * i]), v1 = __builtin_bit_cast(f32x4, xreg[2 * i + 1]);
+        f16x8 h, l;
+#pragma unroll
+        for (int e = 0; e < 4; ++e) {
+          const float s0 = snake_fi(v0[e], al0[e], iv0[e]), s1 = snake_fi(v1[e], al1[e], iv1[e]);
+          h[e] = (_Float16)s0; l[e] = (_Float16)(s0 - (float)h[e]);
+          h[e + 4] = (_Float16)s1; l[e + 4] = (_Float16)(s1 - (float)h[e + 4]);
+        }
+        if (!(row < xrows && jr >= 0 && jr < a.Lin)) h = l = f16x8{0, 0, 0, 0, 0, 0, 0, 0};
+        Xs(2 * o, row) = __builtin_bit_cast(u32x4, h);
+        Xs(2 * o + 1, row) = __builtin_bit_cast(u32x4, l);
+      }
+      return;
+    }
 #pragma unroll
     for (int i = 0; i < XL; ++i) { const int qd = tid + 256 * i; if ((qd >> 3) < XROWS_T) Xs(qd & 7, qd >> 3) = xreg[i]; }
   };
@@ -428,11 +515,20 @@
   load_w(0);
   load_x(0);
   store_w(0);
-  store_x();
+  if constexpr (!RAWIN) store_x(0);
   for (int ch = tid; ch < C_; ch += 256) {
     const float al = a.alpha_mid[ch];
     tab[ch] = al;
     tab[C_ + ch] = 1.0f / (al + 1e-9f);
+    if constexpr (RAWIN) {
+      const float ai = alpha_in[ch];
+      tab[2 * C_ + ch] = ai;
+      tab[3 * C_ + ch] = 1.0f / (ai + 1e-9f);
+    }
+  }
+  if constexpr (RAWIN) {
+    __syncthreads();
+    store_x(0);
   }
   __syncthreads();
   VA_STAMP(stamps, 1);
@@ -469,7 +565,7 @@
       if (kt + 1 < nk) store_w(buf ^ 1);
       if (t == NT - 1 && c + 1 < KC) {
         __syncthreads();
-        store_x();
+        store_x(c + 1);
       }
       __syncthreads();
     }
@@ -569,6 +665,10 @@
   VA_STAMP(stamps, 6);
   VA_STAMP_FLUSH(stamps, 22);
 }
+template <int NCT, int RB, bool WS, bool XS>
+__global__ __launch_bounds__(256, 2) void conv_unit_kernel(ConvPArgs a) { conv_unit_body<NCT, RB, WS, XS, false>(a, nullptr); }
+template <int NCT, int RB, bool WS, bool XS>
+__global__ __launch_bounds__(256, 2) void conv_unit_raw_kernel(ConvPArgs a, const float* alpha_in) { conv_unit_body<NCT, RB, WS, XS, true>(a, alpha_in); }
 
 typedef int i32x8 __attribute__((ext_vector_type(8)));
 
@@ -948,17 +1048,26 @@
 
 #define VA_UNIT_NOT_ELIGIBLE (-0x7fffff00)
 static long long va_conv_units_fused = 0;
-static int launch_conv_unit(const vaura_conv& c7, const vaura_conv& c1, const float* in, const float* res, const float* alpha_mid,
-                            const float* alpha_next, float* out_raw, float* out_act, int B, int L, int pairs, hipStream_t s) {
-  if (pairs != 1 && pairs != 2 && pairs != 4) return VA_UNIT_NOT_ELIGIBLE;
-  if (va_variant(VV_CODEC_UNIT_TWO_LAUNCHES) || va_variant(VV_CODEC_128_ROWS)) return VA_UNIT_NOT_ELIGIBLE;
+static bool va_conv_unit_shape_ok(const vaura_conv& c7, const vaura_conv& c1, int B, int L, int pairs) {
+  if (pairs != 1 && pairs != 2 && pairs != 4) return false;
+  if (va_variant(VV_CODEC_UNIT_TWO_LAUNCHES) || va_variant(VV_CODEC_128_ROWS)) return false;
   const int C = c7.cin;
   if ((C != BN && C != 2 * BN) || c7.cout != C || c1.cin != C || c1.cout != C || c7.stride != 1 || c1.stride != 1 || c1.taps != 1 || c7.taps < 1 ||
-      (c7.taps - 1) * c7.dilation > XHALO || !c7.w || !c7.bias || !c1.w || !c1.bias || !alpha_mid || !alpha_next || !res || !out_act || (const float*)out_act == in)
+      (c7.taps - 1) * c7.dilation > XHALO || !c7.w || !c7.bias || !c1.w || !c1.bias)
+    return false;
+  const int rows = C == BN ? 256 : 128;
+  return (int64_t)((L + rows - 1) / rows) * B >= 384;
+}
+static int launch_conv_unit(const vaura_conv& c7, const vaura_conv& c1, const float* in, const float* res, const float* alpha_mid,
+                            const float* alpha_next, float* out_raw, float* out_act, int B, int L, int pairs, hipStream_t s,
+                            const float* alpha_in = nullptr) {
+  if (!va_conv_unit_shape_ok(c7, c1, B, L, pairs)) return VA_UNIT_NOT_ELIGIBLE;
+  if (!alpha_mid || !res || (const float*)out_act == in) return VA_UNIT_NOT_ELIGIBLE;
+  if (alpha_in ? (res != in || out_raw == in || (!out_raw && !out_act) || (out_act && !alpha_next)) : (!alpha_next || !out_act))
     return VA_UNIT_NOT_ELIGIBLE;
+  const int C = c7.cin;
   const int rows = C == BN ? 256 : 128;
   const int gx = (L + rows - 1) / rows;
-  if ((int64_t)gx * B < 384) return VA_UNIT_NOT_ELIGIBLE;
   ConvPArgs p;
   p.in = reinterpret_cast<const uint16_t*>(in); p.w = reinterpret_cast<const uint16_t*>(c7.w); p.bias = c7.bias; p.res = res;
   p.alpha = alpha_next; p.out_raw = out_raw; p.out_act = reinterpret_cast<uint16_t*>(out_act);
@@ -968,6 +1077,18 @@
   p.w2 = reinterpret_cast<const uint16_t*>(c1.w); p.bias2 = c1.bias; p.alpha_mid = alpha_mid;
   ++va_conv_units_fused;
   const dim3 grid(gx, 1, B);
+  if (alpha_in) {
+    if (C == BN) {
+      if (pairs == 4) VA_LAUNCH((conv_pair_raw_kernel<true, true>), grid, dim3(256), 0, s, p, alpha_in);
+      else if (pairs == 2) VA_LAUNCH((conv_pair_raw_kernel<true, false>), grid, dim3(256), 0, s, p, alpha_in);
+      else VA_LAUNCH((conv_pair_raw_kernel<false, false>), grid, dim3(256), 0, s, p, alpha_in);
+    } else {
+      if (pairs == 4) VA_LAUNCH((conv_unit_raw_kernel<12, 2, true, true>), grid, dim3(256), 0, s, p, alpha_in);
+      else if (pairs == 2) VA_LAUNCH((conv_unit_raw_kernel<12, 2, true, false>), grid, dim3(256), 0, s, p, alpha_in);
+      else VA_LAUNCH((conv_unit_raw_kernel<12, 2, false, false>), grid, dim3(256), 0, s, p, alpha_in);
+    }
+    return 0;
+  }
   if (C == BN) {
     if (pairs == 4) VA_LAUNCH((conv_pair_kernel<3, true, true, 8, true>), grid, dim3(256), 0, s, p);
     else if (pairs == 2) VA_LAUNCH((conv_pair_kernel<3, true, false, 8, true>), grid, dim3(256), 0, s, p);
@@ -1184,9 +1305,26 @@
   if (lay && (rc = va_clips_zero(*lay, A, 1, c->conv_in.cout * act_b, s))) return rc;
   int L = T;
   for (int b = 0; b < c->n_blocks; ++b) {
-    rc = launch_conv(c->up[b], A, nullptr, c->alpha_res[b][0][0], Y, Z, B, L, pr, s);
+    bool raw_level = !va_variant(VV_CODEC_PAIR_HANDOVER);
+    for (int u = 0; u < 3; ++u)
+      raw_level = raw_level && va_conv_unit_shape_ok(c->res[b][u][0], c->res[b][u][1], B, L * c->rates[b], pr) && c->alpha_res[b][u][0] && c->alpha_res[b][u][1];
+    rc = launch_conv(c->up[b], A, nullptr, c->alpha_res[b][0][0], Y, raw_level ? nullptr : Z, B, L, pr, s);
     if (rc) return rc;
     L *= c->rates[b];
+    if (raw_level) {
+      float* X = Y; float* O = R;
+      if (lay && (rc = va_clips_zero(*lay, X, L / T, c->up[b].cout * sizeof(float), s))) return rc;
+      for (int u = 0; u < 3; ++u) {
+        const float* next_alpha = (u < 2) ? c->alpha_res[b][u + 1][0] : (b + 1 < c->n_blocks ? c->alpha_up[b + 1] : c->alpha_out);
+        rc = launch_conv_unit(c->res[b][u][0], c->res[b][u][1], X, X, c->alpha_res[b][u][1], next_alpha, (u < 2) ? O : nullptr,
+                              (u < 2) ? nullptr : Z, B, L, pr, s, c->alpha_res[b][u][0]);
+        if (rc) return rc == VA_UNIT_NOT_ELIGIBLE ? VAURA_ERR_STATE : rc;
+        if (lay && (rc = va_clips_zero(*lay, (u < 2) ? O : Z, L / T, c->up[b].cout * act_b, s))) return rc;
+        { float* t = X; X = O; O = t; }
+      }
+      { float* t = A; A = Z; Z = t; }
+      continue;
+    }
     if (lay && (rc = va_clips_zero(*lay, Z, L / T, c->up[b].cout * act_b, s))) return rc;
     { float* t = R; R = Y; Y = t; t = A; A = Z; Z = t; }
     for (int u = 0; u < 3; ++u) {
@@ -1401,6 +1539,17 @@
   return rc ? rc : VAURA_DAC_UNIT_TWO_LAUNCHES;
 }
 
+int vaura_dac_unit_raw(const vaura_conv* c7, const vaura_conv* c1, int precision, const float* in, const float* alpha_in,
+                       const float* alpha_mid, const float* alpha_next, float* out_raw, void* out_act, int B, int L, vaura_stream_t s_) {
+  if (!c7 || !c1 || !in || !alpha_in || !alpha_mid || (!out_raw && !out_act) || (out_act && !alpha_next) || out_raw == in ||
+      (const float*)out_act == in || B <= 0 || L <= 0 || precision < 0 || precision > 4)
+    return VAURA_ERR_ARG;
+  if (c7->cin % 32) return VAURA_ERR_SHAPE;
+  const int rc = launch_conv_unit(*c7, *c1, in, in, alpha_mid, alpha_next, out_raw, reinterpret_cast<float*>(out_act), B, L, precision,
+                                  as_stream(s_), alpha_in);
+  return rc == VA_UNIT_NOT_ELIGIBLE ? VAURA_DAC_UNIT_TWO_LAUNCHES : rc;
+}
+
 int vaura_dac_from_codes(const int32_t* codes, const float* codebooks, const float* out_proj_w, const float* out_proj_b, void* z,
                          int B, int K, int T, int size, int dim, int latent, int pairs, vaura_stream_t s_) {
   if (!codes || !codebooks || !out_proj_w || !out_proj_b || !z || B <= 0 || T <= 0) return VAURA_ERR_ARG;
diff --git a/vaura_amd/csrc/gemv3.hip b/vaura_amd/csrc/gemv3.hip
--- a/vaura_amd/csrc/gemv3.hip
+++ b/vaura_amd/csrc/gemv3.hip
@@ -6,8 +6,11 @@
 unsigned va_debug_flags2 = 0;
 unsigned va_debug_flags_get() { return va_debug_flags; }
 unsigned va_debug_flags2_get() { return va_debug_flags2; }
+unsigned va_debug_flags3 = 0;
+unsigned va_debug_flags3_get() { return va_debug_flags3; }
 extern "C" void vaura_set_debug_flags(unsigned flags) { va_debug_flags = flags; }
 extern "C" void vaura_set_debug_flags2(unsigned flags) { va_debug_flags2 = flags; }
+extern "C" void vaura_set_debug_flags3(unsigned flags) { va_debug_flags3 = flags; }
 VA_STAMP_SETTER(vaura_stamps_set_gemv3)
 
 static bool rb2(const Gemv3Args& a) { return a.R >= 2 && !va_variant(VV_ROW_BLOCKS_WALK); }
diff --git a/vaura_amd/csrc/variants.h b/vaura_amd/csrc/variants.h
--- a/vaura_amd/csrc/variants.h
+++ b/vaura_amd/csrc/variants.h
@@ -27,7 +27,8 @@
   X(FP8_ROWSPLIT_OFF, 2, 3, "fp8 weights, 17..32 rows: wo / w2 on one workgroup per tile instead of the fp8 row-split pair instances") \
   X(FP8_NO_ENGINE, 2, 4, "fp8 weights never take the one-launch MLP")                                                                  \
   X(LINEAR_REGISTER_STAGED, 2, 5, "extractor linear layers on the register-staged linear_pair_kernel, not linear_dma_kernel (bit-identical)") \
-  X(LINEAR_DMA_LATE_FRAGMENTS, 2, 6, "extractor linear layers: LDS-DMA kernel with the fragments read beside their matrix instructions")
+  X(LINEAR_DMA_LATE_FRAGMENTS, 2, 6, "extractor linear layers: LDS-DMA kernel with the fragments read beside their matrix instructions") \
+  X(CODEC_PAIR_HANDOVER, 3, 0, "codec one-launch units take the producer's activated pairs, not the raw stream with Snake on load")
 
 #define VA_VARIANT_FIELDS(X)                                                                                                           \
   X(GRAPH_STEPS, 1, 24, 4, "decode steps per graph launch (1..15; 0 = the default VA_GRAPH_STEPS), read by vaura_step_graph_build")    \
@@ -46,13 +47,13 @@
 };
 
 constexpr bool va_variants_disjoint() {
-  unsigned seen[2] = {0u, 0u};
+  unsigned seen[3] = {0u, 0u, 0u};
   bool ok = true;
-#define X(name, word, bit, effect) ok = ok && (word) >= 1 && (word) <= 2 && (bit) < 32 && !(seen[(word) - 1] >> (bit) & 1u), seen[(word) - 1] |= 1u << (bit);
+#define X(name, word, bit, effect) ok = ok && (word) >= 1 && (word) <= 3 && (bit) < 32 && !(seen[(word) - 1] >> (bit) & 1u), seen[(word) - 1] |= 1u << (bit);
   VA_VARIANTS(X)
 #undef X
 #define X(name, word, shift, width, effect)                                                                                  \
-  ok = ok && (word) >= 1 && (word) <= 2 && (width) >= 1 && (shift) + (width) <= 32 &&                                        \
+  ok = ok && (word) >= 1 && (word) <= 3 && (width) >= 1 && (shift) + (width) <= 32 &&                                        \
        !(seen[(word) - 1] & (unsigned)(((1ull << (width)) - 1) << (shift))),                                                 \
   seen[(word) - 1] |= (unsigned)(((1ull << (width)) - 1) << (shift));
   VA_VARIANT_FIELDS(X)
@@ -63,16 +64,18 @@
 
 unsigned va_debug_flags_get();
 unsigned va_debug_flags2_get();
+unsigned va_debug_flags3_get();
+inline unsigned va_variant_word(unsigned i) { return i == 0 ? va_debug_flags_get() : (i == 1 ? va_debug_flags2_get() : va_debug_flags3_get()); }
 
-inline bool va_variant(VaVariant v) { return ((v < 32 ? va_debug_flags_get() : va_debug_flags2_get()) >> (v & 31u)) & 1u; }
+inline bool va_variant(VaVariant v) { return (va_variant_word(v >> 5) >> (v & 31u)) & 1u; }
 inline unsigned va_variant_field(VaVariantField f) {
-  return (((f & 255u) < 32 ? va_debug_flags_get() : va_debug_flags2_get()) >> (f & 31u)) & ((1u << (f >> 8)) - 1u);
+  return (va_variant_word((f & 255u) >> 5) >> (f & 31u)) & ((1u << (f >> 8)) - 1u);
 }
 
 struct VaVariantWords {
-  unsigned w1 = 0, w2 = 0;
-  static VaVariantWords current() { return {va_debug_flags_get(), va_debug_flags2_get()}; }
-  void set() const { vaura_set_debug_flags(w1); vaura_set_debug_flags2(w2); }
+  unsigned w1 = 0, w2 = 0, w3 = 0;
+  static VaVariantWords current() { return {va_debug_flags_get(), va_debug_flags2_get(), va_debug_flags3_get()}; }
+  void set() const { vaura_set_debug_flags(w1); vaura_set_debug_flags2(w2); vaura_set_debug_flags3(w3); }
 };
 class VaVariantScope {
   const VaVariantWords saved = VaVariantWords::current();
diff --git a/vaura_amd/engine.py b/vaura_amd/engine.py
--- a/vaura_amd/engine.py
+++ b/vaura_amd/engine.py
@@ -1409,6 +1409,20 @@
         L.check(rc, "vaura_dac_unit")
         return True
 
+    @torch.no_grad()
+    def raw(self, x: torch.Tensor, alpha_in: torch.Tensor, alpha_mid: torch.Tensor, alpha_next: Optional[torch.Tensor],
+            out_raw: Optional[torch.Tensor], out_act: Optional[torch.Tensor]) -> bool:
+        B, Ln, cin = x.shape
+        assert cin == self.c7.cin and x.dtype == torch.float32
+        _cuda_contiguous(x, alpha_in, alpha_mid, alpha_next, out_raw, out_act)
+        with off_null_stream(self.dev):
+            rc = self.lib.vaura_dac_unit_raw(C.byref(self.c7), C.byref(self.c1), self.pairs, L.ptr(x), L.ptr(alpha_in), L.ptr(alpha_mid),
+                                             L.ptr(alpha_next), L.ptr(out_raw), L.ptr(out_act), B, Ln, L.current_stream(self.dev))
+        if rc == L.DAC_UNIT_TWO_LAUNCHES:
+            return False
+        L.check(rc, "vaura_dac_unit_raw")
+        return True
+
 
 @torch.no_grad()
 def codec_from_codes(codes: torch.Tensor, codebooks: torch.Tensor, out_proj_w: torch.Tensor, out_proj_b: torch.Tensor,
diff --git a/vaura_amd/variants.py b/vaura_amd/variants.py
--- a/vaura_amd/variants.py
+++ b/vaura_amd/variants.py
@@ -37,6 +37,10 @@
     LINEAR_DMA_LATE_FRAGMENTS = 1 << 6
 
 
+class Variant3(enum.IntFlag):
+    CODEC_PAIR_HANDOVER = 1 << 0
+
+
 FIELDS = {"GRAPH_STEPS": (1, 24, 4), "ENGINE_ABL": (1, 28, 4), "LINEAR_PANEL": (2, 12, 4)}
 
 
@@ -63,21 +67,28 @@
 
 
 @contextlib.contextmanager
-def variants(word1: int = 0, word2: int = 0, lib=None):
+def variants(word1: int = 0, word2: int = 0, lib=None, word3: int = 0):
     global _open
     if _open:
         raise RuntimeError("variants() does not nest: the words are process-global (pass every switch to one call)")
     if lib is None:
         from . import _lib
         lib = _lib.lib()
+    set3 = getattr(lib, "vaura_set_debug_flags3", None)
+    if word3 and set3 is None:
+        raise RuntimeError("this library has no third variant word (vaura_set_debug_flags3)")
     _open = True
     try:
         lib.vaura_set_debug_flags(int(word1))
         lib.vaura_set_debug_flags2(int(word2))
+        if set3 is not None:
+            set3(int(word3))
         yield
     finally:
         lib.vaura_set_debug_flags(0)
         lib.vaura_set_debug_flags2(0)
+        if set3 is not None:
+            set3(0)
         _open = False
 
 
```

Measured after the change: 74520. About the same (-0.6%).
